# giech/usrp_nfc

Measured on NVIDIA B200. Metric: decoded_msamples_per_s, higher is better.
Workload: dtype f64

## Files before the change

usrp_nfc_b200/csrc/linecode.cu:

```cuda
#include "common.cuh"
#include "scan.cuh"

#include <algorithm>

namespace nfc {

#ifndef NFC_LC_CHUNK
#define NFC_LC_CHUNK 64
#endif
static const int CHUNK = NFC_LC_CHUNK;
static const int LOOKBACK_LIMIT = 4096;
static const int RSTATES = 32, GSTATES = 16;

struct __align__(16) ChunkMap {
    uint8_t r[RSTATES];
    uint8_t g[GSTATES];
};
struct ComposeMap {
    __device__ __forceinline__ ChunkMap operator()(const ChunkMap &a, const ChunkMap &b) const {
        ChunkMap c;
#pragma unroll
        for (int s = 0; s < RSTATES; s++) c.r[s] = b.r[a.r[s] & 31];
#pragma unroll
        for (int s = 0; s < GSTATES; s++) c.g[s] = b.g[a.g[s] & 15];
        return c;
    }
};

struct __align__(16) ChunkCnt {
    uint32_t nsym, nbit0, nbit1, nemit;
    uint32_t has0, tail0, has1, tail1;
};
struct CombineCnt {
    __device__ __forceinline__ ChunkCnt operator()(const ChunkCnt &a, const ChunkCnt &b) const {
        ChunkCnt c;
        c.nsym = a.nsym + b.nsym;
        c.nbit0 = a.nbit0 + b.nbit0;
        c.nbit1 = a.nbit1 + b.nbit1;
        c.nemit = a.nemit + b.nemit;
        if (a.has0 & 1) {
            if ((b.has0 & 2) && a.tail0 == 0) c.nemit--;
            c.has0 = a.has0;
        } else {
            c.has0 = (b.has0 & 1) | (((b.has0 & 2) && a.tail0 == 0) ? 2u : 0u);
        }
        if (a.has1 & 1) {
            if ((b.has1 & 2) && a.tail1 == 0) c.nemit--;
            c.has1 = a.has1;
        } else {
            c.has1 = (b.has1 & 1) | (((b.has1 & 2) && a.tail1 == 0) ? 2u : 0u);
        }
        c.tail0 = (b.has0 & 1) ? b.tail0 : a.tail0 + b.tail0;
        c.tail1 = (b.has1 & 1) ? b.tail1 : a.tail1 + b.tail1;
        return c;
    }
};
__device__ __forceinline__ uint32_t resolved_records(const ChunkCnt &pc, const uint32_t *pending) {
    return pc.nemit - (((pc.has0 & 2) && pending[0] == 0) ? 1u : 0u) - (((pc.has1 & 2) && pending[1] == 0) ? 1u : 0u);
}

struct EvCount {
    const uint32_t *d_M;
    uint32_t cap;
    __device__ __forceinline__ uint32_t n() const { return min(*d_M, cap); }
};

struct TabView {
    const uint8_t *dcm, *dcg;
    const TabEntry *tab;
    int goff;
    int use_reader, use_tag;
    uint32_t pitch, skip, len;
};

static const uint32_t NO_CAPTURE = 0xffffffffu;
__device__ __forceinline__ uint32_t batch_capture(const TabView &tv, uint32_t rel_pos, bool &inside) {
    const uint32_t cap = rel_pos / tv.pitch, off = rel_pos - cap * tv.pitch;
    inside = off >= tv.skip && off < tv.len;
    return cap;
}
__device__ __forceinline__ uint32_t batch_capture_before(const TabView &tv, const EventRec *__restrict__ ev, int64_t i) {
    return i > 0 ? ev[i - 1].rel_pos / tv.pitch : NO_CAPTURE;
}

template <class Sink>
__device__ __forceinline__ void framer_put(int &started, int o, int type, uint32_t pos, Sink &sink) {
    const int start_bit = type == 0 ? 1 : 0;
    sink.symbol(pos, type, o);
    if (o >= 2) {
        if (started) {
            sink.emission(pos, type);
            started = 0;
        }
    } else if (!started && o == start_bit) {
        started = 1;
    } else {
        sink.bit(type, o);
    }
}

template <class Sink>
__device__ __forceinline__ void step_event(const EventRec &ev, const TabView &tv, int &rs, int &gs, Sink &sink) {
    const bool is_r = ev.type == 1;
    if (!(is_r ? tv.use_reader != 0 : (ev.type == 0 && tv.use_tag != 0))) return;
    const uint8_t *dc = is_r ? tv.dcm : tv.dcg;
    const int nst = is_r ? MILLER_STATES : MANCH_STATES, sh = is_r ? 4 : 3;
    const int st = is_r ? rs : gs;
    const TabEntry e = tv.tab[(is_r ? 0 : tv.goff) + ((int)dc[ev.d] * 4 + (ev.v + 1)) * nst + (st & (nst - 1))];
    int started = st >> sh;
    const int n = tab_nout(e), type = is_r ? 1 : 0;
    if (n > 0) framer_put(started, tab_out0(e), type, ev.rel_pos, sink);
    if (n > 1 && is_r) framer_put(started, tab_out1(e), type, ev.rel_pos, sink);
    const int nx = (tab_next(e) & (nst - 1)) | (started << sh);
    rs = is_r ? nx : rs;
    gs = is_r ? gs : nx;
}

template <class Sink>
__device__ __forceinline__ void step_event_batch(const EventRec &ev, const TabView &tv, int &rs, int &gs, Sink &sink, uint32_t &cap_prev) {
    if (tv.pitch) {
        bool inside;
        const uint32_t cap = batch_capture(tv, ev.rel_pos, inside);
        if (cap != cap_prev) {
            cap_prev = cap;
            rs = 0;
            gs = 0;
            sink.new_capture();
        }
        if (!inside) return;
    }
    step_event(ev, tv, rs, gs, sink);
}

__device__ __forceinline__ void load8(const EventRec *__restrict__ ev, int64_t base, EventRec (&e)[8]) {
    const uint4 *p = reinterpret_cast<const uint4 *>(ev + base);
    const uint4 q[4] = {__ldg(p), __ldg(p + 1), __ldg(p + 2), __ldg(p + 3)};
#pragma unroll
    for (int k = 0; k < 4; k++) {
        const unsigned w[4] = {q[k].x, q[k].y, q[k].z, q[k].w};
#pragma unroll
        for (int h = 0; h < 2; h++) {
            EventRec r;
            r.rel_pos = w[2 * h];
            r.d = (uint16_t)(w[2 * h + 1] & 0xffffu);
            r.v = (int8_t)((w[2 * h + 1] >> 16) & 0xffu);
            r.type = (int8_t)(w[2 * h + 1] >> 24);
            e[2 * k + h] = r;
        }
    }
}

struct NullSink {
    __device__ __forceinline__ void symbol(uint32_t, int, int) {}
    __device__ __forceinline__ void emission(uint32_t, int) {}
    __device__ __forceinline__ void bit(int, int) {}
    __device__ __forceinline__ void new_capture() {}
};

__device__ __forceinline__ void load_tables(const LineTables &lt, TabEntry *sm, TabEntry *sg) {
    for (int i = threadIdx.x; i < lt.n_dclass_miller * 4 * MILLER_STATES; i += blockDim.x) sm[i] = lt.miller[i];
    for (int i = threadIdx.x; i < lt.n_dclass_manch * 4 * MANCH_STATES; i += blockDim.x) sg[i] = lt.manch[i];
    __syncthreads();
}

#define NFC_TABLE_SMEM                                              \
    __shared__ TabEntry s_tab[MAX_DCLASS * 4 * (MILLER_STATES + MANCH_STATES)]; \
    load_tables(lt, s_tab, s_tab + MAX_DCLASS * 4 * MILLER_STATES); \
    TabView tv;                                                     \
    tv.dcm = lt.dclass_miller; tv.dcg = lt.dclass_manch;            \
    tv.tab = s_tab; tv.goff = MAX_DCLASS * 4 * MILLER_STATES;        \
    tv.use_reader = lt.decode_reader; tv.use_tag = lt.decode_tag;   \
    tv.pitch = lt.batch_pitch; tv.skip = lt.batch_skip; tv.len = lt.batch_len;

__global__ void chunk_map_kernel(const EventRec *__restrict__ ev, EvCount evc, LineTables lt,
                                 ChunkMap *__restrict__ maps, uint32_t cap_chunks) {
    NFC_TABLE_SMEM
    const uint32_t c = blockIdx.x * blockDim.x + threadIdx.x;
    const uint32_t n_ev = evc.n();
    if (c >= cap_chunks) return;
    const uint32_t i0 = min(n_ev, c * CHUNK), i1 = min(n_ev, i0 + CHUNK);
    uint8_t r[RSTATES], g[GSTATES];
    for (int s = 0; s < RSTATES; s++) r[s] = (uint8_t)s;
    for (int s = 0; s < GSTATES; s++) g[s] = (uint8_t)s;
    bool r_flat = false, g_flat = false;
    NullSink sink;
    uint32_t cap_prev = tv.pitch ? batch_capture_before(tv, ev, (int64_t)i0) : 0u;
    for (uint32_t i = i0; i < i1; i++) {
        const EventRec e = ev[i];
        if (tv.pitch) {
            bool inside;
            const uint32_t cap = batch_capture(tv, e.rel_pos, inside);
            if (cap != cap_prev) {
                cap_prev = cap;
                r[0] = 0; g[0] = 0;
                r_flat = g_flat = true;
            }
            if (!inside) continue;
        }
        if (e.type == 1 && tv.use_reader) {
            if (r_flat) {
                int rs = r[0], gs = 0;
                step_event(e, tv, rs, gs, sink);
                r[0] = (uint8_t)rs;
            } else {
                bool same = true;
                int first = 0;
                for (int s = 0; s < RSTATES; s++) {
                    int rs = r[s], gs = 0;
                    step_event(e, tv, rs, gs, sink);
                    r[s] = (uint8_t)rs;
                    if (s == 0) first = rs;
                    same = same && (rs == first);
                }
                r_flat = same;
            }
        } else if (e.type == 0 && tv.use_tag) {
            if (g_flat) {
                int rs = 0, gs = g[0];
                step_event(e, tv, rs, gs, sink);
                g[0] = (uint8_t)gs;
            } else {
                bool same = true;
                int first = 0;
                for (int s = 0; s < GSTATES; s++) {
                    int rs = 0, gs = g[s];
                    step_event(e, tv, rs, gs, sink);
                    g[s] = (uint8_t)gs;
                    if (s == 0) first = gs;
                    same = same && (gs == first);
                }
                g_flat = same;
            }
        }
    }
    ChunkMap m;
    for (int s = 0; s < RSTATES; s++) m.r[s] = r_flat ? r[0] : r[s];
    for (int s = 0; s < GSTATES; s++) m.g[s] = g_flat ? g[0] : g[s];
    maps[c] = m;
}

struct CountSink {
    ChunkCnt c;
    __device__ __forceinline__ void symbol(uint32_t, int, int) { c.nsym++; }
    __device__ __forceinline__ void emission(uint32_t, int type) {
        uint32_t &has = type == 0 ? c.has0 : c.has1;
        uint32_t &tail = type == 0 ? c.tail0 : c.tail1;
        if (tail != 0) c.nemit++;
        else if (!(has & 1)) { c.nemit++; has |= 2; }
        has |= 1;
        tail = 0;
    }
    __device__ __forceinline__ void bit(int type, int) {
        if (type == 0) { c.nbit0++; c.tail0++; } else { c.nbit1++; c.tail1++; }
    }
    __device__ __forceinline__ void new_capture() {
        c.has0 |= 1; c.tail0 = 0;
        c.has1 |= 1; c.tail1 = 0;
    }
};

__global__ void chunk_summary_kernel(const EventRec *__restrict__ ev, EvCount evc, LineTables lt,
                                     uint16_t *__restrict__ summary) {
    NFC_TABLE_SMEM
    const uint32_t c = blockIdx.x * blockDim.x + threadIdx.x;
    const uint32_t n_ev = evc.n(), n_chunks = (n_ev + CHUNK - 1) / CHUNK;
    if (c >= n_chunks) return;
    int rs = 0, gs = 0;
    bool kR = false, kG = false;
    NullSink sink;
    const uint32_t i0 = c * CHUNK, i1 = min(n_ev, i0 + CHUNK);
    uint32_t cap_prev = tv.pitch ? batch_capture_before(tv, ev, (int64_t)i0) : 0u;
    for (uint32_t i = i0; i < i1; i += 8) {
        EventRec e8[8];
        load8(ev, i, e8);
#pragma unroll
        for (int k = 0; k < 8; k++) {
            if (i + k >= i1) continue;
            const EventRec e = e8[k];
            int dummy = 0;
            if (tv.pitch) {
                bool inside;
                const uint32_t cap = batch_capture(tv, e.rel_pos, inside);
                if (cap != cap_prev) {
                    cap_prev = cap;
                    rs = 0; kR = true;
                    gs = 0; kG = true;
                }
                if (!inside) continue;
            }
            if (e.type == 1 && tv.use_reader) {
                const uint8_t r = lt.reset_miller[(int)tv.dcm[e.d] * 4 + (e.v + 1)];
                if (r != 0xFF) { rs = r; kR = true; }
                else if (kR) step_event(e, tv, rs, dummy, sink);
            } else if (e.type == 0 && tv.use_tag) {
                const uint8_t r = lt.reset_manch[(int)tv.dcg[e.d] * 4 + (e.v + 1)];
                if (r != 0xFF) { gs = r; kG = true; }
                else if (kG) step_event(e, tv, dummy, gs, sink);
            }
        }
    }
    summary[c] = (uint16_t)((rs & 31) | (kR ? 32 : 0) | ((gs & 15) << 8) | (kG ? 4096 : 0));
}

__global__ void chunk_start_kernel(const EventRec *__restrict__ ev, EvCount evc, LineTables lt,
                                   const DecCarry *__restrict__ carry_in, const uint16_t *__restrict__ summary,
                                   uint16_t *__restrict__ start, uint32_t *__restrict__ flags) {
    NFC_TABLE_SMEM
    const uint32_t c = blockIdx.x * blockDim.x + threadIdx.x;
    const uint32_t n_ev = evc.n(), n_chunks = (n_ev + CHUNK - 1) / CHUNK;
    if (c >= n_chunks) return;
    const DecCarry carry = *carry_in;
    int rs = (carry.miller_state & 15) | ((carry.started[1] & 1) << 4);
    int gs = (carry.manch_state & 7) | ((carry.started[0] & 1) << 3);
    const int64_t i0 = (int64_t)c * CHUNK;
    bool foundR = !tv.use_reader, foundG = !tv.use_tag;
    int64_t iR = -1, iG = -1;
    int64_t cc = (int64_t)c - 1;
    const int64_t cmin = max((int64_t)0, (int64_t)c - LOOKBACK_LIMIT / CHUNK);
    for (; cc >= cmin && !(foundR && foundG); cc--) {
        const unsigned sm = summary[cc];
        if (!foundR && (sm & 32u)) { foundR = true; iR = (cc + 1) * CHUNK - 1; rs = (int)(sm & 31u); }
        if (!foundG && (sm & 4096u)) { foundG = true; iG = (cc + 1) * CHUNK - 1; gs = (int)((sm >> 8) & 15u); }
    }
    if (cc >= 0 && !(foundR && foundG)) {
        atomicOr(flags, (uint32_t)POST_UNRESOLVED);
        start[c] = 0;
        return;
    }
    NullSink sink;
    const int64_t fromR = tv.use_reader ? iR + 1 : i0, fromG = tv.use_tag ? iG + 1 : i0;
    const int64_t from = fromR < fromG ? fromR : fromG;
    uint32_t cap_prev = (tv.pitch && from < i0) ? batch_capture_before(tv, ev, from) : 0u;
    for (int64_t base = from & ~(int64_t)7; base < i0; base += 8) {
        EventRec e8[8];
        load8(ev, base, e8);
#pragma unroll
        for (int k = 0; k < 8; k++) {
            const int64_t kk = base + k;
            if (kk < from || kk >= i0) continue;
            const EventRec e = e8[k];
            int dummy_r = 0, dummy_g = 0;
            if (tv.pitch) {
                bool inside;
                const uint32_t cap = batch_capture(tv, e.rel_pos, inside);
                if (cap != cap_prev) {
                    cap_prev = cap;
                    if (kk > iR) rs = 0;
                    if (kk > iG) gs = 0;
                }
                if (!inside) continue;
            }
            if (e.type == 1) {
                if (kk > iR) step_event(e, tv, rs, dummy_g, sink);
            } else if (e.type == 0) {
                if (kk > iG) step_event(e, tv, dummy_r, gs, sink);
            }
        }
    }
    start[c] = (uint16_t)(rs | (gs << 8));
}

__global__ void chunk_start_from_maps_kernel(const ChunkMap *__restrict__ prefix, const DecCarry *__restrict__ carry_in,
                                             uint16_t *__restrict__ start, uint32_t n_chunks) {
    const uint32_t c = blockIdx.x * blockDim.x + threadIdx.x;
    if (c >= n_chunks) return;
    const DecCarry carry = *carry_in;
    const int rs0 = (carry.miller_state & 15) | ((carry.started[1] & 1) << 4);
    const int gs0 = (carry.manch_state & 7) | ((carry.started[0] & 1) << 3);
    start[c] = (uint16_t)(prefix[c].r[rs0] | (prefix[c].g[gs0] << 8));
}

__global__ void chunk_count_kernel(const EventRec *__restrict__ ev, EvCount evc, LineTables lt,
                                   const uint16_t *__restrict__ start, ChunkCnt *__restrict__ cnts, uint32_t cap_chunks) {
    NFC_TABLE_SMEM
    const uint32_t c = blockIdx.x * blockDim.x + threadIdx.x;
    const uint32_t n_ev = evc.n(), n_chunks = (n_ev + CHUNK - 1) / CHUNK;
    if (c >= cap_chunks) return;
    CountSink sink;
    sink.c = ChunkCnt{0, 0, 0, 0, 0, 0, 0, 0};
    if (c >= n_chunks) {
        cnts[c] = sink.c;
        return;
    }
    int rs = start[c] & 31, gs = (start[c] >> 8) & 15;
    const uint32_t i0 = c * CHUNK, i1 = min(n_ev, i0 + CHUNK);
    uint32_t cap_prev = tv.pitch ? batch_capture_before(tv, ev, (int64_t)i0) : 0u;
    for (uint32_t i = i0; i < i1; i += 8) {
        EventRec e[8];
        load8(ev, i, e);
#pragma unroll
        for (int k = 0; k < 8; k++)
            if (i + k < i1) step_event_batch(e[k], tv, rs, gs, sink, cap_prev);
    }
    cnts[c] = sink.c;
}

struct WriteSink {
    SymbolRec *sym;
    uint8_t *bits0, *bits1;
    FrameRec *fr;
    unsigned long long *fx;
    uint32_t *n_empty;
    int64_t a;
    unsigned long long base0, base1;
    uint32_t isym, ib0, ib1, iem;
    uint32_t pend0, pend1;
    uint32_t cap_sym, cap_b0, cap_b1, cap_em;
    __device__ __forceinline__ void symbol(uint32_t pos, int type, int o) {
        if (sym && isym < cap_sym) {
            SymbolRec s;
            s.rel_pos = pos; s.type = (int8_t)type; s.val = (int8_t)o; s.pad = 0;
            sym[isym] = s;
        }
        isym++;
    }
    __device__ __forceinline__ void emission(uint32_t pos, int type) {
        const uint32_t nbits = type == 0 ? pend0 : pend1;
        if (nbits == 0) {
            atomicAdd(n_empty, 1u);
            return;
        }
        if (iem < cap_em) {
            FrameRec f;
            f.pos = a + (int64_t)pos;
            f.bit_off = (int64_t)((type == 0 ? base0 + ib0 : base1 + ib1) - nbits);
            f.nbits = (int32_t)nbits;
            f.type = type;
            fr[iem] = f;
            fx[iem] = ((unsigned long long)f.pos << 24) | ((unsigned long long)nbits << 8) | (unsigned long long)type;
        }
        if ((((unsigned long long)(a + (int64_t)pos)) >> 40) || nbits >= 65536u) atomicOr(n_empty, 0x80000000u);
        iem++;
        if (type == 0) pend0 = 0; else pend1 = 0;
    }
    __device__ __forceinline__ void bit(int type, int o) {
        if (type == 0) { if (ib0 < cap_b0) bits0[ib0] = (uint8_t)o; ib0++; pend0++; }
        else { if (ib1 < cap_b1) bits1[ib1] = (uint8_t)o; ib1++; pend1++; }
    }
    __device__ __forceinline__ void new_capture() { pend0 = 0; pend1 = 0; }
};

struct LineOut {
    SymbolRec *sym;
    uint8_t *bits0, *bits1;
    FrameRec *fr;
    unsigned long long *fx;
    uint32_t cap_sym, cap_b0, cap_b1, cap_em;
    const uint32_t *pending_in;
    int64_t a;
    const unsigned long long *bits_in;
    unsigned long long *bits_out;
    uint32_t *n_empty;
    uint32_t *n_frames;
};

__global__ void chunk_write_kernel(const EventRec *__restrict__ ev, EvCount evc, LineTables lt,
                                   const uint16_t *__restrict__ start,
                                   const ChunkCnt *__restrict__ cnt_prefix, LineOut out, const DecCarry *__restrict__ carry_in,
                                   DecCarry *__restrict__ carry_out, uint32_t *__restrict__ pending_out) {
    NFC_TABLE_SMEM
    const uint32_t c = blockIdx.x * blockDim.x + threadIdx.x;
    const uint32_t n_ev = evc.n(), n_chunks = (n_ev + CHUNK - 1) / CHUNK;
    if (n_chunks == 0 && c == 0) {
        *carry_out = *carry_in;
        pending_out[0] = out.pending_in[0];
        pending_out[1] = out.pending_in[1];
        out.bits_out[0] = out.bits_in[0];
        out.bits_out[1] = out.bits_in[1];
    }
    if (c >= n_chunks) return;
    int rs = start[c] & 31, gs = (start[c] >> 8) & 15;
    const ChunkCnt pc = cnt_prefix[c];
    WriteSink sink;
    sink.sym = out.sym; sink.bits0 = out.bits0; sink.bits1 = out.bits1; sink.fr = out.fr; sink.fx = out.fx;
    sink.n_empty = out.n_empty; sink.a = out.a; sink.base0 = out.bits_in[0]; sink.base1 = out.bits_in[1];
    sink.cap_sym = out.cap_sym; sink.cap_b0 = out.cap_b0; sink.cap_b1 = out.cap_b1; sink.cap_em = out.cap_em;
    sink.isym = pc.nsym; sink.ib0 = pc.nbit0; sink.ib1 = pc.nbit1; sink.iem = resolved_records(pc, out.pending_in);
    sink.pend0 = (pc.has0 & 1) ? pc.tail0 : out.pending_in[0] + pc.tail0;
    sink.pend1 = (pc.has1 & 1) ? pc.tail1 : out.pending_in[1] + pc.tail1;
    const uint32_t i0 = c * CHUNK, i1 = min(n_ev, i0 + CHUNK);
    uint32_t cap_prev = tv.pitch ? batch_capture_before(tv, ev, (int64_t)i0) : 0u;
    for (uint32_t i = i0; i < i1; i += 8) {
        EventRec e[8];
        load8(ev, i, e);
#pragma unroll
        for (int k = 0; k < 8; k++)
            if (i + k < i1) step_event_batch(e[k], tv, rs, gs, sink, cap_prev);
    }
    if (c == n_chunks - 1) {
        DecCarry co;
        co.miller_state = rs & 15; co.started[1] = rs >> 4;
        co.manch_state = gs & 7; co.started[0] = gs >> 3;
        *carry_out = co;
        pending_out[0] = sink.pend0;
        pending_out[1] = sink.pend1;
        out.bits_out[0] = sink.base0 + sink.ib0;
        out.bits_out[1] = sink.base1 + sink.ib1;
        *out.n_frames = sink.iem;
    }
}

uint32_t linecode_chunks(uint32_t n_ev) { return (n_ev + CHUNK - 1) / CHUNK; }
size_t linecode_map_bytes() { return sizeof(ChunkMap); }
size_t linecode_cnt_bytes() { return sizeof(ChunkCnt); }
size_t linecode_emission_bytes() { return sizeof(FrameRec); }
size_t linecode_scratch_bytes(uint32_t n_chunks) {
    return scan_scratch_elems(n_chunks) * sizeof(ChunkMap) + scan_scratch_elems(n_chunks) * sizeof(ChunkCnt);
}

int launch_linecode_start(const EventRec *d_ev, const uint32_t *d_M, uint32_t cap_ev, const LineTables &lt, const DecCarry *d_carry_in,
                          uint16_t *d_summary, uint16_t *d_start, uint32_t *d_flags, cudaStream_t stream) {
    const uint32_t nc = std::max(1u, linecode_chunks(cap_ev));
    const EvCount evc{d_M, cap_ev};
    chunk_summary_kernel<<<(nc + 127) / 128, 128, 0, stream>>>(d_ev, evc, lt, d_summary);
    NFC_CUDA_CHECK(cudaGetLastError());
    chunk_start_kernel<<<(nc + 127) / 128, 128, 0, stream>>>(d_ev, evc, lt, d_carry_in, d_summary, d_start, d_flags);
    NFC_CUDA_CHECK(cudaGetLastError());
    return 0;
}

int launch_linecode_start_scan(const EventRec *d_ev, const uint32_t *d_M, uint32_t cap_ev, const LineTables &lt,
                               const DecCarry *d_carry_in, void *d_maps, void *d_prefix, void *d_scratch, uint16_t *d_start,
                               cudaStream_t stream) {
    const uint32_t nc = std::max(1u, linecode_chunks(cap_ev));
    ChunkMap *maps = (ChunkMap *)d_maps, *prefix = (ChunkMap *)d_prefix;
    const unsigned nb = (nc + 127) / 128;
    const EvCount evc{d_M, cap_ev};
    chunk_map_kernel<<<nb, 128, 0, stream>>>(d_ev, evc, lt, maps, nc);
    NFC_CUDA_CHECK(cudaGetLastError());
    ChunkMap ident;
    for (int s = 0; s < RSTATES; s++) ident.r[s] = (uint8_t)s;
    for (int s = 0; s < GSTATES; s++) ident.g[s] = (uint8_t)s;
    if (device_exclusive_scan<ChunkMap, ComposeMap>(maps, prefix, nc, ident, ComposeMap(), (ChunkMap *)d_scratch, nullptr, stream))
        return -1;
    chunk_start_from_maps_kernel<<<nb, 128, 0, stream>>>(prefix, d_carry_in, d_start, nc);
    NFC_CUDA_CHECK(cudaGetLastError());
    return 0;
}

int launch_linecode_count(const EventRec *d_ev, const uint32_t *d_M, uint32_t cap_ev, const LineTables &lt, const uint16_t *d_start,
                          void *d_cnts, void *d_cnt_prefix, void *d_scratch, void *d_total, cudaStream_t stream) {
    const uint32_t nc = std::max(1u, linecode_chunks(cap_ev));
    ChunkCnt *cnts = (ChunkCnt *)d_cnts, *cprefix = (ChunkCnt *)d_cnt_prefix;
    const EvCount evc{d_M, cap_ev};
    chunk_count_kernel<<<(nc + 127) / 128, 128, 0, stream>>>(d_ev, evc, lt, d_start, cnts, nc);
    NFC_CUDA_CHECK(cudaGetLastError());
    ChunkCnt zero = {0, 0, 0, 0, 0, 0, 0, 0};
    return device_exclusive_scan<ChunkCnt, CombineCnt>(cnts, cprefix, nc, zero, CombineCnt(), (ChunkCnt *)d_scratch,
                                                       (ChunkCnt *)d_total, stream);
}

int launch_linecode_write(const EventRec *d_ev, const uint32_t *d_M, uint32_t cap_ev, const LineTables &lt, const uint16_t *d_start,
                          const void *d_cnt_prefix, SymbolRec *d_sym, uint32_t cap_sym, uint8_t *d_bits0, uint32_t cap_b0,
                          uint8_t *d_bits1, uint32_t cap_b1, void *d_frames, void *d_findex, uint32_t cap_em, int64_t a,
                          const void *d_bits_in, void *d_bits_out, uint32_t *d_n_empty, uint32_t *d_n_frames, const uint32_t *d_pending_in,
                          const DecCarry *d_carry_in, DecCarry *d_carry_out, uint32_t *d_pending_out, cudaStream_t stream) {
    const uint32_t nc = std::max(1u, linecode_chunks(cap_ev));
    LineOut out;
    out.sym = d_sym; out.bits0 = d_bits0; out.bits1 = d_bits1; out.fr = (FrameRec *)d_frames; out.fx = (unsigned long long *)d_findex;
    out.cap_sym = cap_sym; out.cap_b0 = cap_b0; out.cap_b1 = cap_b1; out.cap_em = cap_em;
    out.pending_in = d_pending_in;
    out.a = a;
    out.bits_in = (const unsigned long long *)d_bits_in;
    out.bits_out = (unsigned long long *)d_bits_out;
    out.n_empty = d_n_empty;
    out.n_frames = d_n_frames;
    const EvCount evc{d_M, cap_ev};
    chunk_write_kernel<<<(nc + 127) / 128, 128, 0, stream>>>(d_ev, evc, lt, d_start, (const ChunkCnt *)d_cnt_prefix, out,
                                                             d_carry_in, d_carry_out, d_pending_out);
    NFC_CUDA_CHECK(cudaGetLastError());
    return 0;
}

}
```

usrp_nfc_b200/csrc/slicer.cu:

```cuda
#include <atomic>
#include <map>
#include <mutex>
#include <utility>
#include "common.cuh"
#include <cstdio>
#include <stdlib.h>

namespace nfc {

static const unsigned FULL = 0xffffffffu;
__device__ unsigned long long g_tile_stats[16];
#ifdef NFC_CYCLES
__device__ unsigned long long g_cyc[12];
#endif
__device__ int g_pipe_tune[4] = {6, 3, 2, 18};
enum { CLS_LOW = -1, CLS_MID = 0, CLS_HIGH = 1 };

template <int NT>
__device__ __forceinline__ void cta_sync() {
    asm volatile("bar.sync 1, %0;" ::"n"(NT) : "memory");
}
template <int NT>
__device__ __forceinline__ int cta_sync_or(int pred) {
    int r;
    asm volatile(
        "{\n\t"
        ".reg .pred p, q;\n\t"
        "setp.ne.s32 p, %1, 0;\n\t"
        "bar.red.or.pred q, 1, %2, p;\n\t"
        "selp.s32 %0, 1, 0, q;\n\t"
        "}"
        : "=r"(r)
        : "r"(pred), "n"(NT)
        : "memory");
    return r;
}

__device__ __forceinline__ float env_real(float s) { return __fmul_rn(s, s); }
__device__ __forceinline__ float env_iq(float re, float im) { return __fadd_rn(__fmul_rn(re, re), __fmul_rn(im, im)); }
__device__ __forceinline__ float env_sc16(short2 s, float scale) {
    return env_iq(__fdiv_rn((float)s.x, scale), __fdiv_rn((float)s.y, scale));
}
__device__ __forceinline__ float env_sc16_word(unsigned u, float scale) {
    return env_sc16(make_short2((short)(u & 0xffffu), (short)(u >> 16)), scale);
}
__device__ __forceinline__ float4 env_sc16x4(float4 v, float scale) {
    return make_float4(env_sc16_word(__float_as_uint(v.x), scale), env_sc16_word(__float_as_uint(v.y), scale),
                       env_sc16_word(__float_as_uint(v.z), scale), env_sc16_word(__float_as_uint(v.w), scale));
}

template <bool SC16 = true>
__device__ __forceinline__ float load_one(const void *in, int64_t idx, const SlicerParams &p) {
    if (SC16 && p.input_kind == IN_SC16) return env_sc16(__ldg(reinterpret_cast<const short2 *>(in) + idx), p.pcm_scale);
    switch (p.input_kind) {
        case IN_ENVELOPE_F32: return __ldg(reinterpret_cast<const float *>(in) + idx);
        case IN_REAL_F32: return env_real(__ldg(reinterpret_cast<const float *>(in) + idx));
        case IN_IQ_F32: {
            float2 c = __ldg(reinterpret_cast<const float2 *>(in) + idx);
            return env_iq(c.x, c.y);
        }
        default: {
            float s = __fdiv_rn((float)__ldg(reinterpret_cast<const short *>(in) + idx), p.pcm_scale);
            return env_real(s);
        }
    }
}

__device__ __forceinline__ float4 ldg_stream4(const float4 *ptr) {
    float4 r;
    asm volatile("ld.global.nc.L1::no_allocate.v4.f32 {%0,%1,%2,%3}, [%4];"
                 : "=f"(r.x), "=f"(r.y), "=f"(r.z), "=f"(r.w)
                 : "l"(ptr));
    return r;
}

template <int K, bool SC16 = true>
__device__ __forceinline__ void load_samples(const SegWork &w, const SlicerParams &p, int64_t p0, float (&x)[K]) {
    const int64_t i0 = p0 - w.in_pos0;
    if (K == 4 && p0 >= w.in_begin && p0 + 4 <= w.in_end) {
        if (p.input_kind == IN_ENVELOPE_F32 || p.input_kind == IN_REAL_F32) {
            float4 v = ldg_stream4(reinterpret_cast<const float4 *>(reinterpret_cast<const float *>(w.in) + i0));
            x[0] = v.x; x[1] = v.y; x[2] = v.z; x[3] = v.w;
            if (p.input_kind == IN_REAL_F32) {
#pragma unroll
                for (int j = 0; j < K; j++) x[j] = env_real(x[j]);
            }
            return;
        }
        if (p.input_kind == IN_IQ_F32) {
            const float4 *q = reinterpret_cast<const float4 *>(reinterpret_cast<const float2 *>(w.in) + i0);
            float4 a = ldg_stream4(q), b = ldg_stream4(q + 1);
            x[0] = env_iq(a.x, a.y); x[1] = env_iq(a.z, a.w); x[2] = env_iq(b.x, b.y); x[3] = env_iq(b.z, b.w);
            return;
        }
        if (p.input_kind == IN_PCM_S16) {
            short4 s = __ldg(reinterpret_cast<const short4 *>(reinterpret_cast<const short *>(w.in) + i0));
            x[0] = env_real(__fdiv_rn((float)s.x, p.pcm_scale));
            x[1] = env_real(__fdiv_rn((float)s.y, p.pcm_scale));
            x[2] = env_real(__fdiv_rn((float)s.z, p.pcm_scale));
            x[3] = env_real(__fdiv_rn((float)s.w, p.pcm_scale));
            return;
        }
        if (SC16 && p.input_kind == IN_SC16) {
            const float4 v = env_sc16x4(ldg_stream4(reinterpret_cast<const float4 *>(reinterpret_cast<const short2 *>(w.in) + i0)),
                                        p.pcm_scale);
            x[0] = v.x; x[1] = v.y; x[2] = v.z; x[3] = v.w;
            return;
        }
    }
#pragma unroll
    for (int j = 0; j < K; j++) {
        int64_t q = p0 + j;
        x[j] = (q >= w.in_begin && q < w.in_end) ? load_one<SC16>(w.in, q - w.in_pos0, p) : 0.0f;
    }
}

__device__ __noinline__ int classify_div(double pr, double ss, double lo, double hi) {
    double ratio = __ddiv_rn(pr, ss);
    if (lo > ratio) return CLS_LOW;
    if (ratio > hi) return CLS_HIGH;
    return CLS_MID;
}

__device__ __forceinline__ int classify(float x, double ss, const SlicerParams &p) {
    if (ss == 0.0) return x == 0.0f ? p.cls_ss0_x0 : p.cls_ss0_xn;
    const double pr = (double)x * p.Ld;
    if (!(ss > 0.0) || !(p.lo > 0.0) || !(p.hi > 0.0)) return classify_div(pr, ss, p.lo, p.hi);
    const double r = fma(-p.lo, ss, pr);
    if (r < 0.0) {
        if (r > -(p.lo * ss) * 0x1p-50) return classify_div(pr, ss, p.lo, p.hi);
        return CLS_LOW;
    }
    const double r2 = fma(-p.hi, ss, pr);
    if (r2 > 0.0) {
        if (r2 < (p.hi * ss) * 0x1p-50) return classify_div(pr, ss, p.lo, p.hi);
        return CLS_HIGH;
    }
    return CLS_MID;
}

__device__ __forceinline__ bool st2_forced(int64_t i, int64_t b, int64_t a, int mx) {
    if (b == NO_POS || i - b > (int64_t)mx + 1) return false;
    const int64_t j = b - a;
    const bool tmo = j >= mx && (j % mx) == 0;
    return !tmo;
}

template <int NT>
struct BlockShared {
    static const int NW = NT / 32;
    double wsum[2][NW];
    int wcnt[2][NW];
    int wlastcls[NW];
    int wmaxL[NW];
    int wmaxS[NW];
    unsigned flags[3];
    int emin, emax;
    double red[NW];
};

struct SegCarry {
    double ss0;
    int64_t lastL, lrun_start;
    int last_val;
    uint32_t seg_count;
    unsigned round_no;
    int scan_buf, cnt_buf;
};

template <int NT>
__device__ __forceinline__ double block_excl_scan(double v, double &total, double (*wsum)[NT / 32], int buf) {
    const int lane = threadIdx.x & 31, warp = threadIdx.x >> 5;
    double inc = v;
#pragma unroll
    for (int o = 1; o < 32; o <<= 1) {
        double n = __shfl_up_sync(FULL, inc, o);
        if (lane >= o) inc += n;
    }
    if (lane == 31) wsum[buf][warp] = inc;
    cta_sync<NT>();
    double wbase = 0.0, tot = 0.0;
#pragma unroll
    for (int w = 0; w < NT / 32; w++) {
        double s = wsum[buf][w];
        if (w < warp) wbase += s;
        tot += s;
    }
    total = tot;
    return wbase + (inc - v);
}

template <int NT>
__device__ __forceinline__ int block_excl_scan_int(int v, int &total, int (*wcnt)[NT / 32], int buf) {
    const int lane = threadIdx.x & 31, warp = threadIdx.x >> 5;
    int inc = v;
#pragma unroll
    for (int o = 1; o < 32; o <<= 1) {
        int n = __shfl_up_sync(FULL, inc, o);
        if (lane >= o) inc += n;
    }
    if (lane == 31) wcnt[buf][warp] = inc;
    cta_sync<NT>();
    int wbase = 0, tot = 0;
#pragma unroll
    for (int w = 0; w < NT / 32; w++) {
        int s = wcnt[buf][w];
        if (w < warp) wbase += s;
        tot += s;
    }
    total = tot;
    return wbase + (inc - v);
}

__device__ __forceinline__ void exp_track(float x, int &emin, int &emax) {
    const unsigned ub = __float_as_uint(x);
    if (ub != 0u) {
        const int e = (int)(ub >> 23);
        emin = min(emin, max(e, 1));
        emax = max(emax, e);
    }
}

template <int NT, int K, bool BM = false, bool SC16 = true>
__device__ __noinline__ void exact_tile(const SegWork *wp, const SlicerParams *pp, float *ring, BlockShared<NT> *shp,
                                        const int64_t P0, const int slot0, SegCarry *cs) {
    constexpr int NW = NT / 32;
    const SegWork &w = *wp;
    const SlicerParams &p = *pp;
    BlockShared<NT> &sh = *shp;
    const int L = p.L, mx = p.mx;
    const int tid = threadIdx.x, lane = tid & 31, warp = tid >> 5;
    const int64_t p0 = P0 + (int64_t)tid * K;
    SegCarry c = *cs;
    int emin = 1 << 30, emax = 0;
    const double ss0 = c.ss0;
    const int64_t lastL = c.lastL, lrun_start = c.lrun_start;
    const int last_val = c.last_val;

    float x[K], prev[K];
    bool act[K];
    load_samples<K, SC16>(w, p, p0, x);
#pragma unroll
    for (int j = 0; j < K; j++) act[j] = (p0 + j >= w.warm_begin) && (p0 + j < w.end);

    int slot[K];
#pragma unroll
    for (int j = 0; j < K; j++) {
        int s = slot0 + j;
        slot[j] = s >= L ? s - L : s;
    }
    if (K == 4 && (L & 3) == 0) {
        float4 v = *reinterpret_cast<const float4 *>(ring + slot0);
        prev[0] = v.x; prev[1] = v.y; prev[2] = v.z; prev[3] = v.w;
    } else {
#pragma unroll
        for (int j = 0; j < K; j++) prev[j] = ring[slot[j]];
    }

    int cls[K];
    bool forced[K];
#pragma unroll
    for (int j = 0; j < K; j++) {
        cls[j] = act[j] ? classify(x[j], ss0, p) : CLS_MID;
        forced[j] = false;
    }
    const bool carry_recent = lastL != NO_POS && (P0 - lastL) <= (int64_t)mx + 1;

    double total = 0.0;
    bool had_slow = false, anyL = false;
    for (;;) {
        const unsigned fb = c.round_no % 3u;
        if (tid == 0) sh.flags[(c.round_no + 1u) % 3u] = 0u;
        double pre[K];
        double run = 0.0;
#pragma unroll
        for (int j = 0; j < K; j++) {
            pre[j] = run;
            const bool admit = act[j] && (cls[j] == CLS_MID || (cls[j] == CLS_HIGH && forced[j]));
            if (admit) run += (double)x[j] - (double)prev[j];
        }
        const double base = block_excl_scan<NT>(run, total, sh.wsum, c.scan_buf);
        c.scan_buf ^= 1;

        unsigned f = 0u;
#pragma unroll
        for (int j = 0; j < K; j++) {
            if (act[j]) {
                const int cc = classify(x[j], ss0 + (base + pre[j]), p);
                if (cc != cls[j]) { f |= 1u; cls[j] = cc; }
                if (cc == CLS_HIGH) f |= 2u;
                if (cc == CLS_LOW) f |= 4u;
            }
        }
        f = __reduce_or_sync(FULL, f);
        if (lane == 0 && f) atomicOr(&sh.flags[fb], f);
        if (lane == 31) sh.wlastcls[warp] = act[K - 1] ? cls[K - 1] : 2;
        cta_sync<NT>();
        unsigned flags = sh.flags[fb];
        c.round_no++;

        if ((flags & 2u) && ((flags & 4u) || carry_recent)) {
            int pc = __shfl_up_sync(FULL, cls[K - 1], 1);
            const bool pact = __shfl_up_sync(FULL, (int)act[K - 1], 1) != 0;
            if (lane == 0) {
                pc = CLS_MID;
                bool found = false;
                for (int ww = warp - 1; ww >= 0 && !found; ww--) {
                    int cc = sh.wlastcls[ww];
                    if (cc != 2) { pc = cc; found = true; }
                }
                if (!found) pc = (last_val == -1) ? CLS_LOW : CLS_MID;
            } else if (!pact) {
                pc = (last_val == -1) ? CLS_LOW : CLS_MID;
            }
            int myL = -1, myS = -1;
            int preL[K], preS[K];
            {
                int c_prev = pc;
#pragma unroll
                for (int j = 0; j < K; j++) {
                    preL[j] = myL;
                    preS[j] = myS;
                    if (act[j]) {
                        if (cls[j] == CLS_LOW) {
                            if (c_prev != CLS_LOW) myS = tid * K + j;
                            myL = tid * K + j;
                        }
                        c_prev = cls[j];
                    }
                }
            }
            int incL = myL, incS = myS;
#pragma unroll
            for (int o = 1; o < 32; o <<= 1) {
                int a = __shfl_up_sync(FULL, incL, o), b = __shfl_up_sync(FULL, incS, o);
                if (lane >= o) { incL = max(incL, a); incS = max(incS, b); }
            }
            int exL = __shfl_up_sync(FULL, incL, 1), exS = __shfl_up_sync(FULL, incS, 1);
            if (lane == 0) { exL = -1; exS = -1; }
            if (lane == 31) { sh.wmaxL[warp] = incL; sh.wmaxS[warp] = incS; }
            cta_sync<NT>();
            for (int ww = 0; ww < warp; ww++) {
                exL = max(exL, sh.wmaxL[ww]);
                exS = max(exS, sh.wmaxS[ww]);
            }
            unsigned f2 = 0u;
#pragma unroll
            for (int j = 0; j < K; j++) {
                bool fo = false;
                if (act[j] && cls[j] == CLS_HIGH) {
                    const int bl = max(exL, preL[j]);
                    const int sl = max(exS, preS[j]);
                    const int64_t b = bl >= 0 ? P0 + bl : lastL;
                    const int64_t a = sl >= 0 ? P0 + sl : lrun_start;
                    fo = st2_forced(p0 + j, b, a, mx);
                }
                if (fo != forced[j]) { f2 = 1u; forced[j] = fo; }
            }
            const unsigned fb2 = c.round_no % 3u;
            if (tid == 0) sh.flags[(c.round_no + 1u) % 3u] = 0u;
            f2 = __reduce_or_sync(FULL, f2);
            if (lane == 0 && f2) atomicOr(&sh.flags[fb2], f2);
            cta_sync<NT>();
            flags |= sh.flags[fb2] & 1u;
            c.round_no++;
            had_slow = true;
        } else if (had_slow) {
            unsigned f2 = 0u;
#pragma unroll
            for (int j = 0; j < K; j++) {
                if (forced[j]) { f2 = 1u; forced[j] = false; }
            }
            if (cta_sync_or<NT>((int)f2)) flags |= 1u;
            had_slow = false;
        }
        if (!(flags & 1u)) {
            anyL = (flags & 4u) != 0u;
            break;
        }
    }

    float nv[K];
#pragma unroll
    for (int j = 0; j < K; j++) {
        const bool admit = act[j] && (cls[j] == CLS_MID || (cls[j] == CLS_HIGH && forced[j]));
        nv[j] = admit ? x[j] : prev[j];
        if (admit) exp_track(x[j], emin, emax);
    }
    if (K == 4 && (L & 3) == 0 && act[0] && act[K - 1]) {
        *reinterpret_cast<float4 *>(ring + slot0) = make_float4(nv[0], nv[1], nv[2], nv[3]);
    } else {
#pragma unroll
        for (int j = 0; j < K; j++)
            if (act[j]) ring[slot[j]] = nv[j];
    }

    int val[K];
#pragma unroll
    for (int j = 0; j < K; j++)
        val[j] = act[j] ? (cls[j] == CLS_LOW ? -1 : ((cls[j] == CLS_HIGH && !forced[j]) ? 1 : 0)) : 3;
    int mylast = 3;
#pragma unroll
    for (int j = 0; j < K; j++)
        if (val[j] != 3) mylast = val[j];
    int pv;
    {
        const unsigned has = __ballot_sync(FULL, mylast != 3);
        const unsigned lower = has & ((1u << lane) - 1u);
        const int src = lower ? 31 - __clz(lower) : 0;
        const int got = __shfl_sync(FULL, mylast, src);
        pv = lower ? got : 3;
        int wl = __shfl_sync(FULL, mylast, has ? 31 - __clz(has) : 0);
        if (!has) wl = 3;
        if (lane == 0) sh.wlastcls[warp] = wl;
    }
    cta_sync<NT>();
    if (pv == 3) {
        pv = last_val;
        for (int ww = warp - 1; ww >= 0; ww--) {
            const int cc = sh.wlastcls[ww];
            if (cc != 3) { pv = cc; break; }
        }
    }
    int ntr = 0;
    unsigned trmask = 0u;
    int maxS = -1, maxL = -1;
    {
        int c_prev = pv;
#pragma unroll
        for (int j = 0; j < K; j++) {
            if (val[j] != 3) {
                if (val[j] != c_prev) {
                    if (p0 + j >= w.begin) { trmask |= 1u << j; ntr++; }
                    if (val[j] == -1) maxS = tid * K + j;
                }
                if (val[j] == -1) maxL = tid * K + j;
                c_prev = val[j];
            }
        }
    }
    if (anyL) {
        int mL = __reduce_max_sync(FULL, maxL), mS = __reduce_max_sync(FULL, maxS);
        if (lane == 0) { sh.wmaxL[warp] = mL; sh.wmaxS[warp] = mS; }
    }
    int tot_tr = 0;
    const int tr_base = block_excl_scan_int<NT>(ntr, tot_tr, sh.wcnt, c.cnt_buf);
    c.cnt_buf ^= 1;
    if (BM) {
        if (K == 4 && w.bitmap) {
            unsigned wv = 0u;
#pragma unroll
            for (int j = 0; j < K; j++) {
                const bool on = val[j] != 3 && (p0 + j >= w.begin);
                const unsigned bn = __ballot_sync(FULL, !on || val[j] != -1), bh = __ballot_sync(FULL, on && val[j] == 1);
                if (lane == j) wv = bn;
                if (lane == 4 + j) wv = bh;
            }
            const int64_t cfirst = P0 + (int64_t)warp * 128;
            if (lane < 8 && cfirst + 127 >= w.begin && cfirst < w.end) w.bitmap[((cfirst - w.bm_pos0) >> 7) * 8 + lane] = wv;
        }
    } else if (tot_tr) {
        uint32_t idx = c.seg_count + (uint32_t)tr_base;
#pragma unroll
        for (int j = 0; j < K; j++) {
            if (trmask & (1u << j)) {
                if (idx < w.trans_cap) w.trans[idx] = pack_trans((uint32_t)(p0 + j - w.slab_pos0), val[j]);
                idx++;
            }
        }
        c.seg_count += (uint32_t)tot_tr;
    }
    c.ss0 = ss0 + total;
    if (anyL) {
        int mL = -1, mS = -1;
#pragma unroll
        for (int ww = 0; ww < NW; ww++) {
            mL = max(mL, sh.wmaxL[ww]);
            mS = max(mS, sh.wmaxS[ww]);
        }
        if (mL >= 0) {
            c.lastL = P0 + mL;
            if (mS >= 0) c.lrun_start = P0 + mS;
        }
    }
    {
        int lv = 3;
        for (int ww = NW - 1; ww >= 0; ww--) {
            const int cc = sh.wlastcls[ww];
            if (cc != 3) { lv = cc; break; }
        }
        if (lv != 3) c.last_val = lv;
    }
    emin = __reduce_min_sync(FULL, emin);
    emax = __reduce_max_sync(FULL, emax);
    if (lane == 0) {
        atomicMin(&sh.emin, emin);
        atomicMax(&sh.emax, emax);
    }
    if (tid == 0) *cs = c;
    cta_sync<NT>();
}

constexpr int SLICER_NT = 256;
__global__ void __launch_bounds__(SLICER_NT, 2) slicer_kernel(const SegWork *__restrict__ works,
                                                             const SlicerParams *__restrict__ params) {
    constexpr int NT = SLICER_NT, T = SLICER_NT;
    constexpr int NW = NT / 32;
    extern __shared__ __align__(16) float ring[];
    __shared__ BlockShared<NT> sh;

    __shared__ SegWork w_s;
    __shared__ SlicerParams p_s;
    __shared__ SegCarry c_s;
    if (threadIdx.x == 0) {
        w_s = works[blockIdx.x];
        p_s = params[w_s.param_idx];
    }
    __syncthreads();
    const SegWork &w = w_s;
    const SlicerParams &p = p_s;
    const int L = p.L;
    const int tid = threadIdx.x, lane = tid & 31, warp = tid >> 5;

    SegCarry c;
    int status = SEG_OK;
    int emin = 1 << 30, emax = 0;

    if (w.state_in) {
        const float *src = state_ring(w.state_in);
        for (int i = tid; i < L; i += NT) {
            float v = src[i];
            ring[i] = v;
            exp_track(v, emin, emax);
        }
        c.ss0 = w.state_in->ss;
        c.lastL = w.state_in->lastL;
        c.lrun_start = w.state_in->lrun_start;
        c.last_val = w.state_in->last_val;
    } else {
        double part = 0.0;
        for (int i = tid; i < L; i += NT) {
            const int64_t q = w.warm_begin - L + i;
            float v = load_one(w.in, q - w.in_pos0, p);
            ring[(int)(q % L)] = v;
            part += (double)v;
            exp_track(v, emin, emax);
        }
#pragma unroll
        for (int o = 16; o > 0; o >>= 1) part += __shfl_xor_sync(FULL, part, o);
        if (lane == 0) sh.red[warp] = part;
        __syncthreads();
        double s0 = 0.0;
        for (int i = 0; i < NW; i++) s0 += sh.red[i];
        c.ss0 = s0;
        c.lastL = NO_POS;
        c.lrun_start = NO_POS;
        c.last_val = 0;
    }
    if (tid == 0) {
        sh.flags[0] = sh.flags[1] = sh.flags[2] = 0u;
        sh.emin = 1 << 30;
        sh.emax = 0;
    }
    __syncthreads();
    c.seg_count = 0;
    c.scan_buf = 0;
    c.cnt_buf = 0;
    c.round_no = 0;
    unsigned n_exact = 0;

    const int64_t tile_first = w.warm_begin / T;
    const int64_t tile_last = (w.end > w.warm_begin) ? (w.end - 1) / T : tile_first - 1;
    int slot0 = (int)((tile_first * T + (int64_t)tid) % L);

    for (int64_t tile = tile_first; tile <= tile_last; tile++) {
        const int64_t P0 = tile * T;

        if (w.seam_in && P0 == w.begin && w.begin > w.warm_begin) {
            float *dst = state_ring(w.seam_in);
            for (int i = tid; i < L; i += NT) dst[i] = ring[i];
            if (tid == 0) {
                SlicerHdr h;
                h.ss = c.ss0; h.pos = w.begin; h.lastL = c.lastL; h.lrun_start = c.lrun_start;
                h.last_val = c.last_val; h.emin = 0; h.emax = 0; h.status = 0; h.count = 0; h.pad = 0;
                *w.seam_in = h;
            }
        }

#pragma unroll
        for (int j = 0; j < 3; j++) {
            if (w.ckpt_state[j] && P0 == w.ckpt_pos[j]) {
                float *dst = state_ring(w.ckpt_state[j]);
                for (int i = tid; i < L; i += NT) dst[i] = ring[i];
                if (tid == 0) {
                    SlicerHdr h;
                    h.ss = c.ss0; h.pos = P0; h.lastL = c.lastL; h.lrun_start = c.lrun_start;
                    h.last_val = c.last_val; h.emin = 0; h.emax = 0; h.status = 0; h.count = c.seg_count; h.pad = 0;
                    *w.ckpt_state[j] = h;
                }
            }
        }

        if (tid == 0) c_s = c;
        __syncthreads();
        exact_tile<NT, 1>(&w_s, &p_s, ring, &sh, P0, slot0, &c_s);
        c = c_s;
        n_exact++;
        slot0 += T % L;
        if (slot0 >= L) slot0 -= L;
    }

#pragma unroll
    for (int o = 16; o > 0; o >>= 1) {
        emin = min(emin, __shfl_xor_sync(FULL, emin, o));
        emax = max(emax, __shfl_xor_sync(FULL, emax, o));
    }
    __syncthreads();
    if (lane == 0) { atomicMin(&sh.emin, emin); atomicMax(&sh.emax, emax); }
    __syncthreads();
    emin = sh.emin; emax = sh.emax;
    if (emax >= 255) status |= SEG_NOT_SANE;
    if (emax > 0 && emax - emin > p.span_limit) status |= SEG_INEXACT;
    if (c.seg_count > w.trans_cap) status |= SEG_OVERFLOW;

    if (w.state_out) {
        float *dst = state_ring(w.state_out);
        for (int i = tid; i < L; i += NT) dst[i] = ring[i];
        if (tid == 0) {
            SlicerHdr h;
            h.ss = c.ss0; h.pos = w.end; h.lastL = c.lastL; h.lrun_start = c.lrun_start;
            h.last_val = c.last_val; h.emin = emin; h.emax = emax; h.status = status; h.count = c.seg_count; h.pad = 0;
            *w.state_out = h;
        }
    }
    if (tid == 0 && w.trans_count) *w.trans_count = c.seg_count;
    if (tid == 0 && w.status) *w.status = status;
    if (tid == 0) {
        atomicAdd(&g_tile_stats[1], (unsigned long long)n_exact);
        atomicAdd(&g_tile_stats[8], (unsigned long long)c.round_no);
    }
}

}
#include "slicer_fast.cuh"
namespace nfc {

__global__ void slicer_serial_kernel(const SegWork *__restrict__ works, const SlicerParams *__restrict__ params,
                                     float *__restrict__ ring_scratch, size_t ring_stride) {
    if (threadIdx.x != 0) return;
    const SegWork w = works[blockIdx.x];
    const SlicerParams p = params[w.param_idx];
    const int L = p.L, mx = p.mx;
    float *ring = ring_scratch + (size_t)blockIdx.x * ring_stride;

    double ss;
    int64_t lastL, lrun_start;
    int last_val;
    if (w.state_in) {
        const float *src = state_ring(w.state_in);
        for (int i = 0; i < L; i++) ring[i] = src[i];
        ss = w.state_in->ss;
        lastL = w.state_in->lastL;
        lrun_start = w.state_in->lrun_start;
        last_val = w.state_in->last_val;
    } else {
        ss = 0.0;
        for (int i = 0; i < L; i++) {
            const int64_t q = w.warm_begin - L + i;
            float v = load_one(w.in, q - w.in_pos0, p);
            ring[(int)(q % L)] = v;
            ss += (double)v;
        }
        lastL = NO_POS;
        lrun_start = NO_POS;
        last_val = 0;
    }
    uint32_t count = 0;
    int slot = (int)(w.warm_begin % L);
    for (int64_t q = w.warm_begin; q < w.end; q++) {
        if (w.seam_in && q == w.begin && w.begin > w.warm_begin) {
            float *dst = state_ring(w.seam_in);
            for (int i = 0; i < L; i++) dst[i] = ring[i];
            SlicerHdr h;
            h.ss = ss; h.pos = q; h.lastL = lastL; h.lrun_start = lrun_start;
            h.last_val = last_val; h.emin = 0; h.emax = 0; h.status = 0; h.count = 0; h.pad = 0;
            *w.seam_in = h;
        }
        const float x = load_one(w.in, q - w.in_pos0, p);
        const float prev = ring[slot];
        int c;
        if (ss == 0.0) c = x == 0.0f ? p.cls_ss0_x0 : p.cls_ss0_xn;
        else c = classify_div((double)x * p.Ld, ss, p.lo, p.hi);
        int val;
        if (c == CLS_LOW) {
            val = -1;
            if (last_val != -1) lrun_start = q;
            lastL = q;
        } else if (c == CLS_HIGH && !st2_forced(q, lastL, lrun_start, mx)) {
            val = 1;
        } else {
            val = 0;
            ring[slot] = x;
            ss += ((double)x - (double)prev);
        }
        if (val != last_val) {
            if (q >= w.begin) {
                if (count < w.trans_cap) w.trans[count] = pack_trans((uint32_t)(q - w.slab_pos0), val);
                count++;
            }
            last_val = val;
        }
        slot++;
        if (slot == L) slot = 0;
    }
    if (w.state_out) {
        float *dst = state_ring(w.state_out);
        for (int i = 0; i < L; i++) dst[i] = ring[i];
        SlicerHdr h;
        h.ss = ss; h.pos = w.end; h.lastL = lastL; h.lrun_start = lrun_start;
        h.last_val = last_val; h.emin = 0; h.emax = 0;
        h.status = count > w.trans_cap ? SEG_OVERFLOW : SEG_OK;
        h.count = count; h.pad = 0;
        *w.state_out = h;
    }
    if (w.trans_count) *w.trans_count = count;
    if (w.status) *w.status = count > w.trans_cap ? SEG_OVERFLOW : SEG_OK;
}

__device__ __forceinline__ void canon_st2(const SlicerHdr &h, int mx, int &kind, int64_t &val) {
    if (h.last_val == -1) { kind = 1; val = h.lrun_start; return; }
    if (h.lastL == NO_POS) { kind = 0; val = 0; return; }
    const int64_t j = h.lastL - h.lrun_start;
    const bool tmo = j >= mx && (j % mx) == 0;
    const int64_t until = tmo ? h.lastL : h.lastL + mx + 1;
    if (until < h.pos) { kind = 0; val = 0; } else { kind = 2; val = until; }
}

__global__ void seam_compare_kernel(const SlicerHdr *const *__restrict__ truth, const SlicerHdr *const *__restrict__ assumed,
                                    const int *__restrict__ param_idx, const SlicerParams *__restrict__ params,
                                    int *__restrict__ mismatch) {
    const SlicerHdr *a = truth[blockIdx.x], *b = assumed[blockIdx.x];
    if (!a || !b) return;
    const SlicerParams p = params[param_idx[blockIdx.x]];
    int bad = 0;
    const uint32_t *ra = reinterpret_cast<const uint32_t *>(state_ring(a));
    const uint32_t *rb = reinterpret_cast<const uint32_t *>(state_ring(b));
    if ((((uintptr_t)ra | (uintptr_t)rb) & 15) == 0 && (p.L & 3) == 0) {
        const uint4 *va = reinterpret_cast<const uint4 *>(ra), *vb = reinterpret_cast<const uint4 *>(rb);
        const int n4 = p.L >> 2;
        for (int i = threadIdx.x; i < n4; i += 2 * blockDim.x) {
            const int j = i + blockDim.x;
            const uint4 x0 = __ldg(va + i), y0 = __ldg(vb + i);
            uint4 x1 = x0, y1 = y0;
            if (j < n4) { x1 = __ldg(va + j); y1 = __ldg(vb + j); }
            bad |= (x0.x != y0.x) | (x0.y != y0.y) | (x0.z != y0.z) | (x0.w != y0.w) | (x1.x != y1.x) | (x1.y != y1.y) |
                   (x1.z != y1.z) | (x1.w != y1.w);
        }
    } else {
        for (int i = threadIdx.x; i < p.L; i += blockDim.x) bad |= (ra[i] != rb[i]);
    }
    if (threadIdx.x == 0) {
        if (__double_as_longlong(a->ss) != __double_as_longlong(b->ss)) bad = 1;
        if (a->last_val != b->last_val || a->pos != b->pos) bad = 1;
        int ka, kb;
        int64_t va, vb;
        canon_st2(*a, p.mx, ka, va);
        canon_st2(*b, p.mx, kb, vb);
        if (ka != kb || va != vb) bad = 1;
    }
    if (__syncthreads_or(bad) && threadIdx.x == 0) mismatch[blockIdx.x] = 1;
}

bool slicer_streaming_ok(int L, int kind);
int slicer_streaming_tile(int L, int kind);
int slicer_tile(int L, int kind) {
    if (slicer_streaming_ok(L, kind)) return slicer_streaming_tile(L, kind);
    return SLICER_NT;
}

static int raise_dynamic_smem(const void *fn, size_t smem);

struct FastVariant {
    const void *fn;
    int threads;
    size_t smem;
    int tile;
};
static int env_int(const char *name, int dflt) {
    const char *v = getenv(name);
    return (v && v[0]) ? atoi(v) : dflt;
}
static size_t smem_optin_limit() {
    int dev = 0, lim = 0;
    cudaGetDevice(&dev);
    cudaDeviceGetAttribute(&lim, cudaDevAttrMaxSharedMemoryPerBlockOptin, dev);
    return (size_t)lim;
}
static const size_t FAST_STATIC_SMEM = 10 * 1024;

static const int FAST_SMALL_MIN_L = 1024, FAST_BIG_MIN_L = 8192;
template <int KIND>
static FastVariant fast_variant(int L) {
    static const int pipe = env_int("NFC_SLICER_PIPE", 1), stages = env_int("NFC_SLICER_STAGES", 3);
    const size_t ring = ((size_t)L * 4 + 15) / 16 * 16;
    const size_t item = KIND == IN_IQ_F32 ? 8 : (KIND == IN_PCM_S16 ? 2 : 4);
    const size_t T = L >= FAST_BIG_MIN_L ? 4096 : 512;
    const size_t one = KIND == IN_IQ_F32 ? 0 : T * item;
    const size_t stg = KIND == IN_PCM_S16 ? T * 6 : T * 4;
    const size_t half = smem_optin_limit() / 2;
    FastVariant v;
    v.tile = (int)T;
    if (L < FAST_BIG_MIN_L) {
        if (pipe && KIND != IN_IQ_F32) {
            v.fn = (const void *)slicer_fast_kernel<128, 1, 5, KIND, 3>;
            v.threads = 192;
            v.smem = ring + 3 * stg;
        } else {
            v.fn = (const void *)slicer_fast_kernel<128, 1, 6, KIND, 0>;
            v.threads = 128;
            v.smem = ring + one;
        }
        return v;
    }
    if (pipe && KIND != IN_IQ_F32) {
        if (stages >= 3 && ring + 3 * stg + FAST_STATIC_SMEM <= half) {
            v.fn = (const void *)slicer_fast_kernel<256, 4, 2, KIND, 3>;
            v.threads = 320;
            v.smem = ring + 3 * stg;
        } else if (ring + 2 * stg + FAST_STATIC_SMEM <= half) {
            v.fn = (const void *)slicer_fast_kernel<256, 4, 2, KIND, 2>;
            v.threads = 320;
            v.smem = ring + 2 * stg;
        } else if (env_int("NFC_SLICER_HALF_TILE", 1) && ring + 3 * (stg / 2) + FAST_STATIC_SMEM <= half) {
            v.fn = (const void *)slicer_fast_kernel<256, 2, 2, KIND, 3>;
            v.threads = 320;
            v.smem = ring + 3 * (stg / 2);
            v.tile = 2048;
        } else if (ring + 3 * stg + FAST_STATIC_SMEM <= smem_optin_limit()) {
            v.fn = (const void *)slicer_fast_kernel<512, 2, 1, KIND, 3>;
            v.threads = 576;
            v.smem = ring + 3 * stg;
        } else {
            v.fn = (const void *)slicer_fast_kernel<256, 4, 3, KIND, 0>;
            v.threads = 256;
            v.smem = ring + one;
        }
    } else {
        v.fn = (const void *)slicer_fast_kernel<256, 4, 3, KIND, 0>;
        v.threads = 256;
        v.smem = ring + one;
    }
    return v;
}
static FastVariant fast_variant_of(int L, int kind) {
    switch (kind) {
        case IN_ENVELOPE_F32: return fast_variant<IN_ENVELOPE_F32>(L);
        case IN_REAL_F32: return fast_variant<IN_REAL_F32>(L);
        case IN_IQ_F32: return fast_variant<IN_IQ_F32>(L);
        case IN_SC16: return fast_variant<IN_SC16>(L);
        default: return fast_variant<IN_PCM_S16>(L);
    }
}

int slicer_streaming_tile(int L, int kind) { return fast_variant_of(L, kind).tile; }

static int raise_dynamic_smem(const void *fn, size_t smem) {
    static std::mutex mu;
    static std::map<std::pair<const void *, int>, size_t> have;
    int dev = 0;
    NFC_CUDA_CHECK(cudaGetDevice(&dev));
    std::lock_guard<std::mutex> lock(mu);
    size_t &cur = have[std::make_pair(fn, dev)];
    if (cur < smem) {
        NFC_CUDA_CHECK(cudaFuncSetAttribute(fn, cudaFuncAttributeMaxDynamicSharedMemorySize, (int)smem));
        cur = smem;
    }
    return 0;
}

bool slicer_streaming_ok(int L, int kind) {
    if (L % 4 != 0 || L < FAST_SMALL_MIN_L) return false;
    const FastVariant v = fast_variant_of(L, kind);
    cudaFuncAttributes fa;
    if (cudaFuncGetAttributes(&fa, v.fn) != cudaSuccess) return false;
    return v.smem + fa.sharedSizeBytes <= smem_optin_limit();
}

static int apply_pipe_tuning() {
    static std::mutex mu;
    static bool done[64] = {false};
    int dev = 0;
    NFC_CUDA_CHECK(cudaGetDevice(&dev));
    std::lock_guard<std::mutex> lock(mu);
    if (done[dev & 63]) return 0;
    done[dev & 63] = true;
    if (getenv("NFC_PIPE_MIN") || getenv("NFC_PIPE_COOL") || getenv("NFC_MEAS_MAX") || getenv("NFC_RESUM_BITS")) {
        int t[4] = {env_int("NFC_PIPE_MIN", 6), env_int("NFC_PIPE_COOL", 3), env_int("NFC_MEAS_MAX", 2), env_int("NFC_RESUM_BITS", 18)};
        if (t[0] < 3) t[0] = 3;
        if (t[1] < 0) t[1] = 0;
        if (t[2] < 1) t[2] = 1;
        NFC_CUDA_CHECK(cudaMemcpyToSymbol(g_pipe_tune, t, sizeof(t)));
    }
    return 0;
}

int launch_slicer_streaming(const SegWork *d_works, int n_works, const SlicerParams *d_params, int L, int kind, cudaStream_t stream) {
    if (n_works <= 0) return 0;
    if (apply_pipe_tuning()) return -1;
    const FastVariant v = fast_variant_of(L, kind);
    if (raise_dynamic_smem(v.fn, v.smem)) return -1;
    void *args[2] = {(void *)&d_works, (void *)&d_params};
    NFC_CUDA_CHECK(cudaLaunchKernel(v.fn, dim3((unsigned)n_works), dim3((unsigned)v.threads), args, v.smem, stream));
    return 0;
}

int launch_slicer(const SegWork *d_works, int n_works, const SlicerParams *d_params, int L, cudaStream_t stream) {
    if (n_works <= 0) return 0;
    const size_t smem = ((size_t)L * 4 + 15) / 16 * 16;
    if (raise_dynamic_smem((const void *)slicer_kernel, smem)) return -1;
    slicer_kernel<<<n_works, SLICER_NT, smem, stream>>>(d_works, d_params);
    NFC_CUDA_CHECK(cudaGetLastError());
    return 0;
}

int slicer_tile_stats(unsigned long long *out4, bool reset) {
    NFC_CUDA_CHECK(cudaMemcpyFromSymbol(out4, g_tile_stats, sizeof(unsigned long long) * 16));
#ifdef NFC_CYCLES
    {
        unsigned long long c[12];
        NFC_CUDA_CHECK(cudaMemcpyFromSymbol(c, g_cyc, sizeof(c)));
        fprintf(stderr, "cycles: tile passes %llu in %llu calls (%llu repeats), ring sums after refused tiles %llu, fix-point path %llu, exact path %llu, segment set-up %llu, snapshots %llu, after pipelined runs %llu (its last barrier %llu), loop top %llu, commits %llu\n",
                c[0], c[1], c[5], c[2], c[3], c[4], c[6], c[7], c[8], c[11], c[9], c[10]);
        if (reset) {
            unsigned long long z[12] = {0};
            NFC_CUDA_CHECK(cudaMemcpyToSymbol(g_cyc, z, sizeof(z)));
        }
    }
#endif
    if (reset) {
        unsigned long long z[16] = {0};
        NFC_CUDA_CHECK(cudaMemcpyToSymbol(g_tile_stats, z, sizeof(z)));
    }
    return 0;
}

int slicer_resident_ctas(int L, int kind) {
    int dev = 0, sms = 0, per = 0;
    cudaGetDevice(&dev);
    cudaDeviceGetAttribute(&sms, cudaDevAttrMultiProcessorCount, dev);
    cudaError_t e = cudaSuccess;
    const void *fn = (const void *)slicer_kernel;
    int threads = SLICER_NT;
    size_t dyn = ((size_t)L * 4 + 15) / 16 * 16;
    if (slicer_streaming_ok(L, kind)) {
        const FastVariant v = fast_variant_of(L, kind);
        fn = v.fn;
        threads = v.threads;
        dyn = v.smem;
    }
    if (raise_dynamic_smem(fn, dyn) == 0) e = cudaOccupancyMaxActiveBlocksPerMultiprocessor(&per, fn, threads, dyn);
    if (e != cudaSuccess || per < 1) per = 1;
    return sms * per;
}

__global__ void __launch_bounds__(256) batch_warm_kernel(const char *__restrict__ items, int64_t stride_bytes, int64_t pitch,
                                                         const SlicerParams *__restrict__ params, char *__restrict__ states,
                                                         size_t state_bytes) {
    extern __shared__ float warm_s[];
    const int64_t c = blockIdx.x;
    const SlicerParams p = params[c];
    const int L = p.L;
    SlicerHdr *h = reinterpret_cast<SlicerHdr *>(states + (size_t)c * state_bytes);
    float *ring = state_ring(h);
    const int64_t B = c * pitch;
    const void *in = items + c * stride_bytes;
    for (int i = threadIdx.x; i < L; i += blockDim.x) {
        const float v = load_one(in, i, p);
        warm_s[i] = v;
        ring[(int)((B + i) % L)] = v;
    }
    __syncthreads();
    if (threadIdx.x == 0) {
        double s = 0.0;
        for (int i = 0; i < L; i++) s += (double)warm_s[i];
        SlicerHdr hh;
        hh.ss = s;
        hh.pos = B + L;
        hh.lastL = NO_POS;
        hh.lrun_start = NO_POS;
        hh.last_val = 0;
        hh.emin = 0; hh.emax = 0; hh.status = 0; hh.count = 0; hh.pad = 0;
        *h = hh;
    }
}

__global__ void bitmap_fill_kernel(uint4 *__restrict__ bm, size_t n_chunks) {
    const size_t i = (size_t)blockIdx.x * blockDim.x + threadIdx.x;
    if (i >= n_chunks) return;
    bm[2 * i] = make_uint4(FULL, FULL, FULL, FULL);
    bm[2 * i + 1] = make_uint4(0u, 0u, 0u, 0u);
}

int launch_batch_warm(const void *d_items, int64_t stride_bytes, int64_t pitch, int n_cap, int L, const SlicerParams *d_params,
                      void *d_states, size_t state_bytes, cudaStream_t stream) {
    if (n_cap <= 0) return 0;
    const size_t smem = (size_t)L * 4;
    if (raise_dynamic_smem((const void *)batch_warm_kernel, smem)) return -1;
    batch_warm_kernel<<<n_cap, 256, smem, stream>>>((const char *)d_items, stride_bytes, pitch, d_params, (char *)d_states, state_bytes);
    NFC_CUDA_CHECK(cudaGetLastError());
    return 0;
}

int launch_bitmap_fill(uint32_t *d_bm, size_t n_chunks, cudaStream_t stream) {
    if (!n_chunks) return 0;
    bitmap_fill_kernel<<<(unsigned)((n_chunks + 255) / 256), 256, 0, stream>>>(reinterpret_cast<uint4 *>(d_bm), n_chunks);
    NFC_CUDA_CHECK(cudaGetLastError());
    return 0;
}

int launch_slicer_serial(const SegWork *d_works, int n_works, const SlicerParams *d_params, float *d_ring_scratch,
                         size_t ring_stride, cudaStream_t stream) {
    if (n_works <= 0) return 0;
    slicer_serial_kernel<<<n_works, 32, 0, stream>>>(d_works, d_params, d_ring_scratch, ring_stride);
    NFC_CUDA_CHECK(cudaGetLastError());
    return 0;
}

int launch_seam_compare(const SlicerHdr *const *d_truth, const SlicerHdr *const *d_assumed, const int *d_param_idx,
                        const SlicerParams *d_params, int *d_mismatch, int n, cudaStream_t stream) {
    if (n <= 0) return 0;
    seam_compare_kernel<<<n, 256, 0, stream>>>(d_truth, d_assumed, d_param_idx, d_params, d_mismatch);
    NFC_CUDA_CHECK(cudaGetLastError());
    return 0;
}

}
```

usrp_nfc_b200/csrc/stream.cu:

```cuda
#include <algorithm>
#include <atomic>
#include <chrono>
#include <cstdarg>
#include <cstdio>
#include <cstdlib>
#include <cstring>
#include <memory>
#include <string>
#include <thread>
#include <deque>
#include <vector>

#include "../../include/usrp_nfc_b200.h"
#include "common.cuh"
#include "tables.h"

namespace nfc {

int launch_slicer(const SegWork *d_works, int n_works, const SlicerParams *d_params, int L, cudaStream_t);
bool slicer_streaming_ok(int L, int kind);
int launch_slicer_streaming(const SegWork *d_works, int n_works, const SlicerParams *d_params, int L, int kind, cudaStream_t);
int launch_extract_count(const uint32_t *d_bm, int64_t bm_pos0, int64_t a, int64_t b, const RunCarry *d_rc_in, int carry_from_bm,
                         uint32_t *d_block_counts, uint32_t *d_block_offsets, uint32_t *d_scan_scratch, uint32_t *d_total,
                         cudaStream_t stream);
int launch_extract_write(const uint32_t *d_bm, int64_t bm_pos0, int64_t a, int64_t b, const RunCarry *d_rc_in, int carry_from_bm,
                         const uint32_t *d_block_offsets, TransRec *d_out, uint32_t out_cap, cudaStream_t stream);
size_t extract_blocks(int64_t bm_pos0, int64_t a, int64_t b);
int launch_slicer_serial(const SegWork *d_works, int n_works, const SlicerParams *d_params, float *d_ring_scratch,
                         size_t ring_stride, cudaStream_t);
int launch_seam_compare(const SlicerHdr *const *d_truth, const SlicerHdr *const *d_assumed, const int *d_param_idx,
                        const SlicerParams *d_params, int *d_mismatch, int n, cudaStream_t);
int launch_gather_transitions(const SegWork *d_works, const uint32_t *d_counts, uint32_t *d_offsets, int n_segs,
                              TransRec *d_dense, cudaStream_t);
int launch_gather_pieces(const TransRec *const *d_src, const uint32_t *d_n, const uint32_t *d_off, int n_pieces,
                         TransRec *d_dense, cudaStream_t);
int launch_run_count(const TransRec *d_tr, const uint32_t *d_R, uint32_t cap_R, int64_t w0, int64_t w1, const RunCarry *d_rc_in,
                     int mx, int keep_dropped, uint32_t *d_counts, uint32_t *d_offsets, uint32_t *d_scratch, uint32_t *d_total,
                     uint32_t *d_flags, cudaStream_t stream);
int launch_run_write(const TransRec *d_tr, const uint32_t *d_R, uint32_t cap_R, int64_t w0, int64_t w1, const RunCarry *d_rc_in,
                     int mx, int keep_dropped, const uint32_t *d_offsets, EventRec *d_events, uint32_t cap, const uint32_t *d_M,
                     RunCarry *d_carry_out, uint32_t *d_flags, cudaStream_t stream);
uint32_t linecode_chunks(uint32_t n_ev);
size_t linecode_map_bytes();
size_t linecode_cnt_bytes();
size_t linecode_emission_bytes();
size_t linecode_scratch_bytes(uint32_t n_chunks);
int launch_linecode_start(const EventRec *d_ev, const uint32_t *d_M, uint32_t cap_ev, const LineTables &lt, const DecCarry *d_carry_in,
                          uint16_t *d_summary, uint16_t *d_start, uint32_t *d_flags, cudaStream_t stream);
int launch_linecode_start_scan(const EventRec *d_ev, const uint32_t *d_M, uint32_t cap_ev, const LineTables &lt,
                               const DecCarry *d_carry_in, void *d_maps, void *d_prefix, void *d_scratch, uint16_t *d_start,
                               cudaStream_t stream);
int launch_linecode_count(const EventRec *d_ev, const uint32_t *d_M, uint32_t cap_ev, const LineTables &lt, const uint16_t *d_start,
                          void *d_cnts, void *d_cnt_prefix, void *d_scratch, void *d_total, cudaStream_t stream);
int launch_linecode_write(const EventRec *d_ev, const uint32_t *d_M, uint32_t cap_ev, const LineTables &lt, const uint16_t *d_start,
                          const void *d_cnt_prefix, SymbolRec *d_sym, uint32_t cap_sym, uint8_t *d_bits0, uint32_t cap_b0,
                          uint8_t *d_bits1, uint32_t cap_b1, void *d_frames, void *d_findex, uint32_t cap_em, int64_t a,
                          const void *d_bits_in, void *d_bits_out, uint32_t *d_n_empty, uint32_t *d_n_frames, const uint32_t *d_pending_in,
                          const DecCarry *d_carry_in, DecCarry *d_carry_out, uint32_t *d_pending_out, cudaStream_t stream);
int slicer_tile(int L, int kind);
int slicer_resident_ctas(int L, int kind);
int slicer_tile_stats(unsigned long long *out4, bool reset);
int launch_batch_warm(const void *d_items, int64_t stride_bytes, int64_t pitch, int n_cap, int L, const SlicerParams *d_params,
                      void *d_states, size_t state_bytes, cudaStream_t stream);
int launch_bitmap_fill(uint32_t *d_bm, size_t n_chunks, cudaStream_t stream);
int synth_render(void *dev_out, int64_t n, int64_t first_index, const int8_t *codes, const int64_t *lens, int64_t n_runs,
                 float carrier, float pause, float tag_high, float noise, float fade, double fade_period, uint64_t seed,
                 int as_envelope, cudaStream_t);

static thread_local char g_err[512] = "";
void set_error(const char *fmt, ...) {
    va_list ap;
    va_start(ap, fmt);
    vsnprintf(g_err, sizeof(g_err), fmt, ap);
    va_end(ap);
}

struct DevBuf {
    void *p = nullptr;
    size_t cap = 0;
    int ensure(size_t bytes) {
        if (bytes <= cap) return 0;
        if (p) cudaFree(p);
        p = nullptr;
        cap = 0;
        size_t want = bytes + bytes / 4 + 256;
        NFC_CUDA_CHECK(cudaMalloc(&p, want));
        cap = want;
        return 0;
    }
    void release() {
        if (p) cudaFree(p);
        p = nullptr;
        cap = 0;
    }
    template <class T>
    T *as() const { return reinterpret_cast<T *>(p); }
};

static size_t item_bytes(int kind) {
    switch (kind) {
        case IN_IQ_F32: return 8;
        case IN_PCM_S16: return 2;
        case IN_SC16: return 4;
        default: return 4;
    }
}

static int ceil_log2(int v) {
    int l = 0;
    while ((1LL << l) < v) l++;
    return l;
}

static int classify_ratio_host(double ratio, double lo, double hi) {
    if (lo > ratio) return -1;
    if (ratio > hi) return 1;
    return 0;
}

struct FrameArena {
    nfc_frame *p = nullptr;
    size_t n = 0, cap = 0;
    size_t size() const { return n; }
    bool empty() const { return n == 0; }
    nfc_frame *data() { return p; }
    const nfc_frame &operator[](size_t i) const { return p[i]; }
    void clear() { n = 0; }
    int reserve(size_t need) {
        if (need <= cap) return 0;
        const size_t ncap = std::max(need + need / 2 + 4096, cap * 2);
        nfc_frame *q = nullptr;
        if (cudaMallocHost((void **)&q, ncap * sizeof(nfc_frame)) != cudaSuccess) return -1;
        if (n) memcpy(q, p, n * sizeof(nfc_frame));
        if (p) cudaFreeHost(p);
        p = q;
        cap = ncap;
        return 0;
    }
    void release() {
        if (p) cudaFreeHost(p);
        p = nullptr;
        n = cap = 0;
    }
};
static_assert(sizeof(nfc_frame) == sizeof(FrameRec), "the device writes nfc_frame records");

struct BitArena {
    uint8_t *p = nullptr;
    size_t cap = 0, len = 0, closed = 0;
    int reserve(size_t need) {
        if (need <= cap) return 0;
        const size_t ncap = std::max(need + need / 2 + 65536, cap * 2);
        uint8_t *q = nullptr;
        if (cudaMallocHost((void **)&q, ncap) != cudaSuccess) return -1;
        if (len) memcpy(q, p, len);
        if (p) cudaFreeHost(p);
        p = q;
        cap = ncap;
        return 0;
    }
    void consume() {
        const size_t open = len - closed;
        if (open && closed) memmove(p, p + closed, open);
        len = open;
        closed = 0;
    }
    void clear() { len = closed = 0; }
    void release() {
        if (p) cudaFreeHost(p);
        p = nullptr;
        cap = len = closed = 0;
    }
};

struct Stream {
    nfc_params prm;
    SlicerParams sp;
    HostTables ht;
    LineTables lt;
    double factor;
    cudaStream_t cs = nullptr;
    cudaStream_t cs2 = nullptr;
    cudaStream_t cs3 = nullptr;
    cudaEvent_t ev_h[2] = {nullptr, nullptr};
    cudaEvent_t ev_k0 = nullptr, ev_k1 = nullptr;
    DevBuf staging2[2];
    static const int NCTX = 4;
    cudaEvent_t ev_a[NCTX] = {}, ev_b[NCTX] = {}, ev_c[NCTX] = {};
    cudaStream_t csR = nullptr, csL = nullptr;
    cudaEvent_t evE[NCTX] = {}, evR[NCTX] = {}, evL[NCTX] = {};
    long long chain_first_seq = 0;
    long long last_final_seq = -1;
    cudaEvent_t ev_ctx[NCTX] = {};
    cudaEvent_t ev_out[2] = {};
    bool ev_out_set[2] = {false, false};
    DevBuf ctx_d;
    char *ctx_h = nullptr;
    long long slab_seq = 0;
    struct Rates {
        bool have = false;
        double R = 0, M = 0, sym = 0, b0 = 0, b1 = 0, em = 0;
    } rates;

    int64_t pos = 0;
    bool stable = false;
    bool serial_mode = false;
    std::vector<float> warm;
    DevBuf state;
    RunCarry run_carry{0, 0, 0, 0};
    DecCarry dec_carry{0, 0, {0, 0}};
    uint32_t pending[2] = {0, 0};

    int64_t seg_len = 0, halo = 0, slab_len = 0;
    int force_serial = 0;

    DevBuf params_d, tab_d, staging, works_d, states_d, trans_seg, seg_counts, seg_status,
        seam_ptrs, mismatch_d, run_counts, run_offsets, scan_scr, maps_d, prefix_d, cnts_d, cprefix_d,
        line_scr, serial_ring, start_d, ckpt_d, redo_states, redo_trans,
        redo_counts, pieces_d, bitmap_d, ex_counts, ex_offsets, ex_scr, summ_d;
    DevBuf events_d[2], sym_d[2], bits0_d[2], bits1_d[2], em_d[2], fx_d[2];
    DevBuf trans_dense[2];
    std::vector<DevBuf> kept_bufs;
    static const int NPIN = 3;
    void *pinned[NPIN] = {nullptr, nullptr, nullptr};
    size_t pinned_cap[NPIN] = {0, 0, 0};
    long long slabs_enqueued = 0;
    std::atomic<long long> slabs_marshalled{0};
    std::thread marshal_thr;
    bool blocking_wait = false;
    cudaEvent_t ev_blk = nullptr;
    cudaError_t sync_cs() {
        if (!blocking_wait) return cudaStreamSynchronize(cs);
        const cudaError_t e = cudaEventRecord(ev_blk, cs);
        return e != cudaSuccess ? e : cudaEventSynchronize(ev_blk);
    }
    int set_wait_mode(bool blocking);
    std::atomic<int> marshal_err{0};
    struct SlabJob {
        long long seq = 0;
        int64_t a = 0, b = 0;
        uint32_t cap_R = 0, cap_M = 0, cap_sym = 0, cap_b0 = 0, cap_b1 = 0, cap_em = 0;
        bool exact = false;
        bool events_only = false;
        bool from_bitmap = false;
        bool want_ev = false, want_sym = false, want_fr = false, have_line = false;
        double t0 = 0, t1 = 0, t2 = 0;
    };
    std::deque<SlabJob> jobs;
    cudaEvent_t ev_d[NPIN] = {nullptr, nullptr, nullptr};
    int post_chain(int64_t a, int64_t b, bool from_bitmap, uint32_t R_host, bool force_exact, double t0, double t1,
                   const EventRec *host_events = nullptr, uint32_t n_host_events = 0);
    int64_t push_events(const nfc_event *ev, int64_t n);
    int finalize_front();
    int finalize_all() {
        while (!jobs.empty())
            if (finalize_front()) return -1;
        return 0;
    }
    int marshal(const SlabJob &j, int pi, char *hp, size_t off_ev, size_t off_sym, uint32_t M, uint32_t nsym);

    std::vector<nfc_event> out_events;
    std::vector<nfc_symbol> out_symbols;
    FrameArena out_frames;
    cudaEvent_t ev_last_records = nullptr;
    bool have_last_records = false;
    int settle_frames();
    uint64_t *findex = nullptr;
    size_t findex_n = 0, findex_cap = 0;
    bool findex_bad = false;
    bool findex_ext = false;
    bool findex_ext_locked = false;
    void findex_drop() {
        if (findex && findex_ext && findex_ext_locked) cudaHostUnregister(findex);
        if (findex && !findex_ext) cudaFreeHost(findex);
        findex = nullptr;
        findex_ext = findex_ext_locked = false;
        findex_cap = findex_n = 0;
    }
    int findex_reserve(size_t n) {
        if (n <= findex_cap) return 0;
        if (findex_ext) return -1;
        const size_t cap = std::max(n, findex_cap * 2 + 4096);
        uint64_t *p = nullptr;
        if (cudaMallocHost((void **)&p, cap * sizeof(uint64_t)) != cudaSuccess) return -1;
        if (findex_n) memcpy(p, findex, findex_n * sizeof(uint64_t));
        if (findex) cudaFreeHost(findex);
        findex = p;
        findex_cap = cap;
        return 0;
    }
    BitArena fb[2];
    int resident_ctas = 0;
    size_t ev_head = 0, sym_head = 0, fr_head = 0;

    nfc_stats stats;

    int tile() const { return slicer_tile(sp.L, sp.input_kind); }
    bool parallel_ok() const { return sp.L >= 256 && sp.L <= 52000 && !force_serial && !serial_mode; }

    int init(const nfc_params *p);
    void destroy();
    int ensure_pinned(int idx, size_t bytes);
    int join_marshal();
    int finish_pending() { return finalize_all(); }
    int settle() { return finalize_all() || join_marshal() || settle_frames() ? -1 : 0; }
    int64_t push(const void *items, int64_t n, int mem, int *called_back);
    int64_t push_batch(const void *items, int mem, int64_t n_cap, int64_t cap_len, int64_t stride_items, const double *lo_vals,
                       const double *hi_vals, int64_t *pitch_out);
    int64_t batch_fill_pitch = 0, batch_fill_caps = 0, batch_fill_len = 0;
    DevBuf batch_states, batch_stage;
    int finish_warmup();
    int process_slab(const void *d_in, int64_t in_pos0, int64_t in_begin, int64_t in_end, int64_t a, int64_t b, int64_t slicer_end);
    enum class Slicer { streaming, first_gen, sequential };
    int run_slicer(Slicer kind, const void *d_in, int64_t in_pos0, int64_t in_begin, int64_t in_end, int64_t a, int64_t b,
                   uint32_t *R_out, bool *fell_back);
    int launch_streaming(const SegWork *d_works, int n_works);
    void add_kernel_time();
    int compare_states(const std::vector<const SlicerHdr *> &truth, const std::vector<const SlicerHdr *> &assumed, int n,
                       std::vector<int> &mism);
    int64_t bm_lo = 0, bm_hi = 0, bm_origin = 0;
    int64_t super_slab = 5;
    bool super_balance = true;
    bool streaming_ok() const { return parallel_ok() && slicer_streaming_ok(sp.L, sp.input_kind); }
};

int Stream::ensure_pinned(int idx, size_t bytes) {
    if (bytes <= pinned_cap[idx]) return 0;
    if (pinned[idx]) cudaFreeHost(pinned[idx]);
    pinned[idx] = nullptr;
    pinned_cap[idx] = 0;
    NFC_CUDA_CHECK(cudaMallocHost(&pinned[idx], bytes + bytes / 4 + 4096));
    pinned_cap[idx] = bytes + bytes / 4 + 4096;
    return 0;
}

int Stream::join_marshal() {
    if (marshal_thr.joinable()) marshal_thr.join();
    if (const int err = marshal_err.exchange(0)) {
        set_error(err == 3 ? "more frames than the caller's frame index buffer holds (nfc_stream_set_frame_index_buffer)"
                           : (err == 2 ? "copying a slab's records to the host failed" : "internal: frame longer than the retained bits"));
        return -1;
    }
    return 0;
}

int Stream::init(const nfc_params *p) {
    prm = *p;
    memset(&stats, 0, sizeof(stats));
    if (!(p->samp_rate > 0) || p->av_window < 1 || p->max_len < 1 || p->max_len > 65535) {
        set_error("bad parameters: samp_rate=%g av_window=%d max_len=%d", p->samp_rate, p->av_window, p->max_len);
        return -1;
    }
    if (p->av_window >= (1 << 28)) {
        set_error("av_window too large");
        return -1;
    }
    NFC_CUDA_CHECK(cudaSetDevice(p->device));
    NFC_CUDA_CHECK(cudaStreamCreateWithFlags(&cs, cudaStreamNonBlocking));
    NFC_CUDA_CHECK(cudaStreamCreateWithFlags(&cs2, cudaStreamNonBlocking));
    NFC_CUDA_CHECK(cudaStreamCreateWithFlags(&cs3, cudaStreamNonBlocking));
    NFC_CUDA_CHECK(cudaStreamCreateWithFlags(&csR, cudaStreamNonBlocking));
    NFC_CUDA_CHECK(cudaStreamCreateWithFlags(&csL, cudaStreamNonBlocking));
    for (int i = 0; i < 2; i++) NFC_CUDA_CHECK(cudaEventCreateWithFlags(&ev_h[i], cudaEventDisableTiming));
    NFC_CUDA_CHECK(cudaEventCreate(&ev_k0));
    NFC_CUDA_CHECK(cudaEventCreate(&ev_k1));
    for (int i = 0; i < NCTX; i++) {
        NFC_CUDA_CHECK(cudaEventCreate(&ev_a[i]));
        NFC_CUDA_CHECK(cudaEventCreate(&ev_b[i]));
        NFC_CUDA_CHECK(cudaEventCreate(&ev_c[i]));
        NFC_CUDA_CHECK(cudaEventCreateWithFlags(&ev_ctx[i], cudaEventDisableTiming));
        NFC_CUDA_CHECK(cudaEventCreateWithFlags(&evE[i], cudaEventDisableTiming));
        NFC_CUDA_CHECK(cudaEventCreateWithFlags(&evR[i], cudaEventDisableTiming));
        NFC_CUDA_CHECK(cudaEventCreateWithFlags(&evL[i], cudaEventDisableTiming));
    }
    for (int i = 0; i < 2; i++) NFC_CUDA_CHECK(cudaEventCreateWithFlags(&ev_out[i], cudaEventDisableTiming));
    for (int i = 0; i < NPIN; i++) NFC_CUDA_CHECK(cudaEventCreateWithFlags(&ev_d[i], cudaEventDisableTiming | cudaEventBlockingSync));
    NFC_CUDA_CHECK(cudaMallocHost((void **)&ctx_h, (size_t)NCTX * 256));
    if (ctx_d.ensure((size_t)NCTX * 256)) return -1;
    NFC_CUDA_CHECK(cudaMemset(ctx_d.p, 0, (size_t)NCTX * 256));
    factor = 1e6 / p->samp_rate;
    sp.lo = p->lo_val;
    sp.hi = p->hi_val;
    sp.L = p->av_window;
    sp.Ld = (double)p->av_window;
    sp.mx = p->max_len;
    sp.loL = sp.lo / sp.Ld;
    sp.hiL = sp.hi / sp.Ld;
    sp.cls_ss0_x0 = classify_ratio_host(1.0, sp.lo, sp.hi);
    sp.cls_ss0_xn = classify_ratio_host(sp.hi + 0.1, sp.lo, sp.hi);
    sp.span_limit = std::max(0, 28 - ceil_log2(sp.L) - 1);
    sp.input_kind = p->input_kind;
    sp.pcm_scale = p->pcm_scale > 0 ? p->pcm_scale : 32767.0f;
    if (params_d.ensure(sizeof(SlicerParams))) return -1;
    NFC_CUDA_CHECK(cudaMemcpy(params_d.p, &sp, sizeof(sp), cudaMemcpyHostToDevice));

    if (!build_tables(sp.mx, factor, ht)) {
        set_error("line-code tables need more than %d duration classes", MAX_DCLASS);
        return -1;
    }
    const size_t dcm = ht.dclass_miller.size(), dcg = ht.dclass_manch.size();
    const size_t tm = ht.miller.size() * sizeof(TabEntry), tg = ht.manch.size() * sizeof(TabEntry);
    auto up = [](size_t v) { return (v + 255) / 256 * 256; };
    const size_t o1 = up(dcm), o2 = o1 + up(dcg), o3 = o2 + up(tm), o4 = o3 + up(tg), o5 = o4 + up(ht.reset_miller.size());
    if (tab_d.ensure(o5 + up(ht.reset_manch.size()))) return -1;
    char *base = tab_d.as<char>();
    NFC_CUDA_CHECK(cudaMemcpy(base, ht.dclass_miller.data(), dcm, cudaMemcpyHostToDevice));
    NFC_CUDA_CHECK(cudaMemcpy(base + o1, ht.dclass_manch.data(), dcg, cudaMemcpyHostToDevice));
    NFC_CUDA_CHECK(cudaMemcpy(base + o2, ht.miller.data(), tm, cudaMemcpyHostToDevice));
    NFC_CUDA_CHECK(cudaMemcpy(base + o3, ht.manch.data(), tg, cudaMemcpyHostToDevice));
    NFC_CUDA_CHECK(cudaMemcpy(base + o4, ht.reset_miller.data(), ht.reset_miller.size(), cudaMemcpyHostToDevice));
    NFC_CUDA_CHECK(cudaMemcpy(base + o5, ht.reset_manch.data(), ht.reset_manch.size(), cudaMemcpyHostToDevice));
    lt.dclass_miller = (const uint8_t *)base;
    lt.dclass_manch = (const uint8_t *)(base + o1);
    lt.miller = (const TabEntry *)(base + o2);
    lt.manch = (const TabEntry *)(base + o3);
    lt.reset_miller = (const uint8_t *)(base + o4);
    lt.reset_manch = (const uint8_t *)(base + o5);
    lt.n_dclass_miller = ht.n_dclass_miller;
    lt.n_dclass_manch = ht.n_dclass_manch;
    lt.decode_reader = p->decode_reader;
    lt.decode_tag = p->decode_tag;
    lt.batch_pitch = 0;
    lt.batch_skip = 0;
    lt.batch_len = 0;

    warm.reserve((size_t)sp.L);
    if (state.ensure(state_block_bytes(sp.L))) return -1;
    resident_ctas = parallel_ok() ? slicer_resident_ctas(sp.L, sp.input_kind) : 1;
    if (const char *e = getenv("NFC_SUPER_SLAB")) super_slab = std::max(1, std::min(8, atoi(e)));
    if (const char *e = getenv("NFC_SUPER_BALANCE")) super_balance = atoi(e) != 0;
    return 0;
}

void Stream::destroy() {
    DevBuf *all[] = {&batch_states, &batch_stage, &params_d, &tab_d, &staging, &works_d, &states_d, &trans_seg, &trans_dense[0], &trans_dense[1], &seg_counts,
                     &seg_status, &seam_ptrs, &mismatch_d, &run_counts, &run_offsets, &scan_scr, &maps_d,
                     &prefix_d, &cnts_d, &cprefix_d, &line_scr, &ctx_d, &events_d[0], &events_d[1], &sym_d[0], &sym_d[1], &bits0_d[0],
                     &bits0_d[1], &bits1_d[0], &bits1_d[1], &em_d[0], &em_d[1], &fx_d[0], &fx_d[1],
                     &serial_ring, &start_d, &ckpt_d, &redo_states, &redo_trans, &redo_counts, &pieces_d, &state, &bitmap_d,
                     &ex_counts, &ex_offsets, &ex_scr, &summ_d};
    finalize_all();
    if (marshal_thr.joinable()) marshal_thr.join();
    if (cs) cudaStreamSynchronize(cs);
    if (csR) cudaStreamSynchronize(csR);
    if (csL) cudaStreamSynchronize(csL);
    if (cs2) cudaStreamSynchronize(cs2);
    for (DevBuf *b : all) b->release();
    if (ctx_h) cudaFreeHost(ctx_h);
    ctx_h = nullptr;
    fb[0].release();
    fb[1].release();
    out_frames.release();
    findex_drop();
    for (int i = 0; i < NPIN; i++)
        if (pinned[i]) cudaFreeHost(pinned[i]);
    for (int i = 0; i < NCTX; i++) {
        if (ev_a[i]) cudaEventDestroy(ev_a[i]);
        if (ev_b[i]) cudaEventDestroy(ev_b[i]);
        if (ev_c[i]) cudaEventDestroy(ev_c[i]);
        if (ev_ctx[i]) cudaEventDestroy(ev_ctx[i]);
        if (evE[i]) cudaEventDestroy(evE[i]);
        if (evR[i]) cudaEventDestroy(evR[i]);
        if (evL[i]) cudaEventDestroy(evL[i]);
    }
    for (int i = 0; i < 2; i++)
        if (ev_out[i]) cudaEventDestroy(ev_out[i]);
    if (csR) cudaStreamDestroy(csR);
    if (csL) cudaStreamDestroy(csL);
    if (cs2) cudaStreamDestroy(cs2);
    if (cs3) cudaStreamDestroy(cs3);
    if (ev_k0) cudaEventDestroy(ev_k0);
    if (ev_k1) cudaEventDestroy(ev_k1);
    for (int i = 0; i < 2; i++) {
        if (ev_h[i]) cudaEventDestroy(ev_h[i]);
        staging2[i].release();
    }
    for (int i = 0; i < NPIN; i++)
        if (ev_d[i]) cudaEventDestroy(ev_d[i]);
    if (ev_blk) cudaEventDestroy(ev_blk);
    if (cs) cudaStreamDestroy(cs);
}

static float host_env(const void *items, int64_t i, int kind, float pcm_scale) {
    switch (kind) {
        case IN_ENVELOPE_F32: return ((const float *)items)[i];
        case IN_REAL_F32: {
            volatile float s = ((const float *)items)[i];
            volatile float r = s * s;
            return r;
        }
        case IN_IQ_F32: {
            volatile float re = ((const float *)items)[2 * i], im = ((const float *)items)[2 * i + 1];
            volatile float a = re * re, b = im * im;
            volatile float r = a + b;
            return r;
        }
        case IN_SC16: {
            const int16_t *iq = (const int16_t *)items + 2 * i;
            volatile float re = (float)iq[0] / pcm_scale, im = (float)iq[1] / pcm_scale;
            volatile float a = re * re, b = im * im;
            volatile float r = a + b;
            return r;
        }
        default: {
            volatile float s = (float)((const int16_t *)items)[i] / pcm_scale;
            volatile float r = s * s;
            return r;
        }
    }
}

int Stream::set_wait_mode(bool blocking) {
    if (settle()) return -1;
    NFC_CUDA_CHECK(cudaSetDevice(prm.device));
    const unsigned flags = cudaEventDisableTiming | (blocking ? cudaEventBlockingSync : 0);
    for (int i = 0; i < NCTX; i++) {
        if (ev_ctx[i]) cudaEventDestroy(ev_ctx[i]);
        ev_ctx[i] = nullptr;
        NFC_CUDA_CHECK(cudaEventCreateWithFlags(&ev_ctx[i], flags));
    }
    if (blocking && !ev_blk) NFC_CUDA_CHECK(cudaEventCreateWithFlags(&ev_blk, cudaEventDisableTiming | cudaEventBlockingSync));
    blocking_wait = blocking;
    return 0;
}

int Stream::finish_warmup() {
    double s = 0;
    for (int i = 0; i < sp.L; i++) s += (double)warm[(size_t)i];
    std::vector<char> blk(state_block_bytes(sp.L), 0);
    SlicerHdr *h = reinterpret_cast<SlicerHdr *>(blk.data());
    h->ss = s;
    h->pos = sp.L;
    h->lastL = NO_POS;
    h->lrun_start = NO_POS;
    h->last_val = 0;
    memcpy(state_ring(h), warm.data(), (size_t)sp.L * 4);
    NFC_CUDA_CHECK(cudaMemcpyAsync(state.p, blk.data(), blk.size(), cudaMemcpyHostToDevice, cs));
    NFC_CUDA_CHECK(sync_cs());
    run_carry.st = 0;
    run_carry.last_bit = 0;
    run_carry.dur = sp.L % sp.mx;
    stable = true;
    return 0;
}

int64_t Stream::push(const void *items, int64_t n, int mem, int *called_back) {
    if (called_back) *called_back = 0;
    if (n < 0) {
        set_error("negative item count");
        return -1;
    }
    NFC_CUDA_CHECK(cudaSetDevice(prm.device));
    const size_t ib = item_bytes(sp.input_kind);
    if (!stable) {
        const int64_t need = sp.L - (int64_t)warm.size();
        const int64_t can = std::min(n, need);
        if (can > 0) {
            std::vector<char> tmp;
            const void *src = items;
            if (mem == NFC_MEM_DEVICE) {
                tmp.resize((size_t)can * ib);
                NFC_CUDA_CHECK(cudaMemcpyAsync(tmp.data(), items, (size_t)can * ib, cudaMemcpyDeviceToHost, cs));
                NFC_CUDA_CHECK(sync_cs());
                src = tmp.data();
            }
            for (int64_t i = 0; i < can; i++) warm.push_back(host_env(src, i, sp.input_kind, sp.pcm_scale));
        }
        pos += can;
        if (can == need && finish_warmup()) return -1;
        return can;
    }
    if (called_back) *called_back = 1;
    int64_t done = 0;
    const int64_t slab = slab_len > 0 ? std::min<int64_t>(slab_len, (int64_t)1 << 30) : (int64_t)1 << 28;
    const bool host_in = mem == NFC_MEM_HOST;
    auto stage_host = [&](int64_t off, int64_t m, int64_t a, int buf) -> int {
        const size_t padb = (size_t)(a - (a - (a & 3))) * ib;
        if (staging2[buf].ensure(padb + (size_t)m * ib + 64)) return -1;
        NFC_CUDA_CHECK(cudaMemcpyAsync(staging2[buf].as<char>() + padb, (const char *)items + (size_t)off * ib, (size_t)m * ib,
                                       cudaMemcpyHostToDevice, cs3));
        NFC_CUDA_CHECK(cudaEventRecord(ev_h[buf], cs3));
        stats.h2d_bytes += (int64_t)((size_t)m * ib);
        return 0;
    };
    int hbuf = 0;
    if (host_in && n > 0) {
        NFC_CUDA_CHECK(sync_cs());
        if (stage_host(0, std::min(slab, n), pos, hbuf)) return -1;
    }
    while (done < n) {
        const int64_t m = std::min(slab, n - done);
        const int64_t a = pos, b = pos + m;
        const int64_t in_pos0 = a - (a & 3);
        const void *d_in = nullptr;
        int64_t in_begin = in_pos0;
        int64_t slicer_end = b;
        const char *src = (const char *)items + (size_t)done * ib;
        const size_t padb = (size_t)(a - in_pos0) * ib;
        if (host_in) {
            const int64_t m_next = std::min(slab, n - (done + m));
            if (m_next > 0 && stage_host(done + m, m_next, b, hbuf ^ 1)) return -1;
            NFC_CUDA_CHECK(cudaStreamWaitEvent(cs, ev_h[hbuf], 0));
            d_in = staging2[hbuf].p;
            hbuf ^= 1;
        } else if ((((uintptr_t)src - padb) & 15) == 0) {
            d_in = src - padb;
            in_begin = a;
            int64_t take = super_slab;
            if (super_balance) {
                const int64_t left = (n - done + slab - 1) / slab, launches = (left + super_slab - 1) / super_slab;
                take = (left + launches - 1) / launches;
            }
            slicer_end = std::min(pos + (n - done), a + take * slab);
        } else {
            if (staging.ensure(padb + (size_t)m * ib + 64)) return -1;
            NFC_CUDA_CHECK(cudaMemcpyAsync(staging.as<char>() + padb, src, (size_t)m * ib, cudaMemcpyDeviceToDevice, cs));
            d_in = staging.p;
        }
        if (process_slab(d_in, in_pos0, in_begin, std::max(b, slicer_end), a, b, slicer_end)) return -1;
        pos = b;
        done += m;
        stats.samples += m;
    }
    return n;
}

int64_t Stream::push_batch(const void *items, int mem, int64_t n_cap, int64_t cap_len, int64_t stride_items, const double *lo_vals,
                           const double *hi_vals, int64_t *pitch_out) {
    NFC_CUDA_CHECK(cudaSetDevice(prm.device));
    const int L = sp.L;
    const int T = tile();
    const size_t ib = item_bytes(sp.input_kind);
    if (pos != 0 || stable || !warm.empty()) {
        set_error("push_batch: the stream has consumed samples; reset it first");
        return -1;
    }
    if (!streaming_ok()) {
        set_error("push_batch: needs the streaming slicer (av_window in [1024, 52000], a multiple of 4)");
        return -1;
    }
    if (n_cap <= 0 || cap_len <= (int64_t)L + 2 * sp.mx || stride_items < cap_len || L <= sp.mx + 1) {
        set_error("push_batch: bad shape (captures %lld, items %lld, stride %lld, av_window %d)", (long long)n_cap, (long long)cap_len,
                  (long long)stride_items, L);
        return -1;
    }
    if (prm.outputs & NFC_OUT_DROPPED_EVENTS) {
        set_error("push_batch: type -1 events are not reproduced across capture boundaries (NFC_OUT_DROPPED_EVENTS)");
        return -1;
    }
    if (((size_t)stride_items * ib) % 16 != 0 || ((uintptr_t)items % 16) != 0) {
        set_error("push_batch: captures must start 16-byte aligned");
        return -1;
    }
    const int64_t pitch = (cap_len + T - 1) / T * T;
    if (pitch >= ((int64_t)1 << 30)) {
        set_error("push_batch: capture too long for one slab");
        return -1;
    }
    if (pitch_out) *pitch_out = pitch;
    const void *d_items = items;
    if (mem == NFC_MEM_HOST) {
        const size_t bytes = ((size_t)(n_cap - 1) * (size_t)stride_items + (size_t)cap_len) * ib;
        if (batch_stage.ensure(bytes + 64)) return -1;
        NFC_CUDA_CHECK(cudaMemcpyAsync(batch_stage.p, items, bytes, cudaMemcpyHostToDevice, cs));
        stats.h2d_bytes += (int64_t)bytes;
        d_items = batch_stage.p;
    }
    std::vector<SlicerParams> ps((size_t)n_cap, sp);
    for (int64_t c = 0; c < n_cap; c++) {
        SlicerParams &q = ps[(size_t)c];
        if (lo_vals) q.lo = lo_vals[c];
        if (hi_vals) q.hi = hi_vals[c];
        q.loL = q.lo / q.Ld;
        q.hiL = q.hi / q.Ld;
        q.cls_ss0_x0 = classify_ratio_host(1.0, q.lo, q.hi);
        q.cls_ss0_xn = classify_ratio_host(q.hi + 0.1, q.lo, q.hi);
        if (!(q.lo > 0.0) || !(q.hi > q.lo)) {
            set_error("push_batch: capture %lld: thresholds must satisfy 0 < lo_val < hi_val", (long long)c);
            return -1;
        }
    }
    if (params_d.ensure(sizeof(SlicerParams) * (size_t)n_cap)) return -1;
    NFC_CUDA_CHECK(cudaMemcpyAsync(params_d.p, ps.data(), sizeof(SlicerParams) * (size_t)n_cap, cudaMemcpyHostToDevice, cs));
    const size_t sblk = state_block_bytes(L);
    if (batch_states.ensure(sblk * (size_t)n_cap) || seg_status.ensure(sizeof(int32_t) * (size_t)n_cap) ||
        works_d.ensure(sizeof(SegWork) * (size_t)n_cap))
        return -1;
    const int64_t total = n_cap * pitch;
    const size_t n_chunks = (size_t)(total / 128);
    const size_t bm_cap_before = bitmap_d.cap;
    if (bitmap_d.ensure((n_chunks + 64) * 32)) return -1;
    if (bitmap_d.cap != bm_cap_before || batch_fill_pitch != pitch || batch_fill_caps < n_cap || batch_fill_len != cap_len) {
        if (launch_bitmap_fill(bitmap_d.as<uint32_t>(), n_chunks, cs)) return -1;
        batch_fill_pitch = pitch;
        batch_fill_caps = n_cap;
        batch_fill_len = cap_len;
        stats.launches++;
    }
    if (launch_batch_warm(d_items, (int64_t)((size_t)stride_items * ib), pitch, (int)n_cap, L, params_d.as<SlicerParams>(), batch_states.p,
                          sblk, cs))
        return -1;
    stats.launches++;
    std::vector<int64_t> order((size_t)n_cap);
    for (int64_t c = 0; c < n_cap; c++) order[(size_t)c] = c;
    if (hi_vals) std::stable_sort(order.begin(), order.end(), [&](int64_t a, int64_t b) { return hi_vals[a] > hi_vals[b]; });
    std::vector<SegWork> works((size_t)n_cap);
    for (int64_t k = 0; k < n_cap; k++) {
        const int64_t c = order[(size_t)k];
        SegWork &w = works[(size_t)k];
        memset(&w, 0, sizeof(w));
        const int64_t B = c * pitch;
        w.in = (const char *)d_items + (size_t)c * (size_t)stride_items * ib;
        w.in_pos0 = B;
        w.in_begin = B;
        w.in_end = B + cap_len;
        w.warm_begin = B + L;
        w.begin = B + L;
        w.end = B + cap_len;
        w.slab_pos0 = 0;
        w.state_in = reinterpret_cast<const SlicerHdr *>(batch_states.as<char>() + sblk * (size_t)c);
        for (int j = 0; j < 3; j++) w.ckpt_pos[j] = INT64_MAX;
        w.status = seg_status.as<int32_t>() + c;
        w.param_idx = (int32_t)c;
        w.bitmap = bitmap_d.as<uint32_t>();
        w.bm_pos0 = 0;
    }
    NFC_CUDA_CHECK(cudaMemcpyAsync(works_d.p, works.data(), sizeof(SegWork) * (size_t)n_cap, cudaMemcpyHostToDevice, cs));
    if (launch_streaming(works_d.as<SegWork>(), (int)n_cap)) return -1;
    stats.launches++;
    stats.slicer_launches++;
    stats.segments += n_cap;
    std::vector<int32_t> status((size_t)n_cap);
    NFC_CUDA_CHECK(cudaMemcpyAsync(status.data(), seg_status.p, sizeof(int32_t) * (size_t)n_cap, cudaMemcpyDeviceToHost, cs));
    NFC_CUDA_CHECK(sync_cs());
    add_kernel_time();
    for (int64_t c = 0; c < n_cap; c++)
        if (status[(size_t)c] & (SEG_INEXACT | SEG_NOT_SANE)) {
            set_error("push_batch: capture %lld is outside the exactly-summable regime: decode the captures one by one", (long long)c);
            return -3;
        }
    stable = true;
    bm_lo = 0;
    bm_hi = total;
    bm_origin = 0;
    lt.batch_pitch = (uint32_t)pitch;
    lt.batch_skip = (uint32_t)L;
    lt.batch_len = (uint32_t)cap_len;
    const int64_t slab_max = slab_len > 0 ? std::min<int64_t>(slab_len, (int64_t)1 << 30) : (int64_t)1 << 30;
    const int64_t per_slab = std::max<int64_t>(1, slab_max / pitch);
    int rc = 0;
    if (finish_pending()) return -1;
    run_carry = RunCarry{0, 0, L % sp.mx, 0};
    for (int64_t c0 = 0; c0 < n_cap && !rc; c0 += per_slab) {
        const int64_t c1 = std::min(n_cap, c0 + per_slab);
        if (process_slab(nullptr, c0 * pitch, c0 * pitch, c1 * pitch, c0 * pitch, c1 * pitch, c1 * pitch)) rc = -1;
        pos = c1 * pitch;
        stats.samples += (c1 - c0) * cap_len;
    }
    if (!rc && finish_pending()) rc = -1;
    lt.batch_pitch = 0;
    bm_lo = bm_hi = 0;
    cudaMemcpyAsync(params_d.p, &sp, sizeof(sp), cudaMemcpyHostToDevice, cs);
    if (sync_cs() != cudaSuccess && !rc) rc = -1;
    return rc ? rc : n_cap;
}

int Stream::launch_streaming(const SegWork *d_works, int n_works) {
    NFC_CUDA_CHECK(cudaEventRecord(ev_k0, cs));
    if (launch_slicer_streaming(d_works, n_works, params_d.as<SlicerParams>(), sp.L, sp.input_kind, cs)) return -1;
    NFC_CUDA_CHECK(cudaEventRecord(ev_k1, cs));
    return 0;
}

void Stream::add_kernel_time() {
    float ms = 0;
    if (cudaEventElapsedTime(&ms, ev_k0, ev_k1) == cudaSuccess) {
        stats.slicer_kernel_ms += ms;
        stats.slicer_kernel_launches++;
    }
}

int Stream::compare_states(const std::vector<const SlicerHdr *> &truth, const std::vector<const SlicerHdr *> &assumed, int n,
                           std::vector<int> &mism) {
    const size_t room = truth.size();
    char *base = seam_ptrs.as<char>();
    NFC_CUDA_CHECK(cudaMemcpyAsync(base, truth.data(), sizeof(void *) * (size_t)n, cudaMemcpyHostToDevice, cs));
    NFC_CUDA_CHECK(cudaMemcpyAsync(base + sizeof(void *) * room, assumed.data(), sizeof(void *) * (size_t)n, cudaMemcpyHostToDevice, cs));
    NFC_CUDA_CHECK(cudaMemsetAsync(base + 2 * sizeof(void *) * room, 0, sizeof(int) * (size_t)n, cs));
    NFC_CUDA_CHECK(cudaMemsetAsync(mismatch_d.p, 0, sizeof(int) * (size_t)n, cs));
    if (launch_seam_compare((const SlicerHdr *const *)base, (const SlicerHdr *const *)(base + sizeof(void *) * room),
                            (const int *)(base + 2 * sizeof(void *) * room), params_d.as<SlicerParams>(), mismatch_d.as<int>(), n, cs))
        return -1;
    stats.launches++;
    NFC_CUDA_CHECK(cudaMemcpyAsync(mism.data(), mismatch_d.p, sizeof(int) * (size_t)n, cudaMemcpyDeviceToHost, cs));
    return 0;
}

static int print_segment_cycles(const std::vector<SegWork> &works) {
    const int nseg = (int)works.size();
    double sum = 0;
    uint32_t mn = ~0u, mx = 0;
    std::vector<uint32_t> kc((size_t)nseg), rs((size_t)nseg);
    for (int k = 0; k < nseg; k++) {
        SlicerHdr h;
        NFC_CUDA_CHECK(cudaMemcpy(&h, works[(size_t)k].state_out, sizeof(SlicerHdr), cudaMemcpyDeviceToHost));
        kc[(size_t)k] = h.count; rs[(size_t)k] = h.pad;
        sum += h.count; mn = std::min(mn, h.count); mx = std::max(mx, h.count);
    }
    fprintf(stderr, "segments %d kcycles min %u avg %.0f max %u\n", nseg, mn, sum / nseg, mx);
    for (int k = 0; k < nseg; k += std::max(1, nseg / 24))
        fprintf(stderr, "  seg %d: %u kcyc, redo %u slow %u\n", k, kc[(size_t)k], rs[(size_t)k] >> 16, rs[(size_t)k] & 0xffff);
    for (int q = 0; q < 6; q++) {
        int best = 0;
        for (int k = 1; k < nseg; k++) if (kc[(size_t)k] > kc[(size_t)best]) best = k;
        fprintf(stderr, "  slowest seg %d: %u kcyc, redo %u slow %u\n", best, kc[(size_t)best], rs[(size_t)best] >> 16, rs[(size_t)best] & 0xffff);
        kc[(size_t)best] = 0;
    }
    return 0;
}

int Stream::run_slicer(Slicer kind, const void *d_in, int64_t in_pos0, int64_t in_begin, int64_t in_end, int64_t a, int64_t b,
                       uint32_t *R_out, bool *fell_back) {
    if (finalize_all()) return -1;
    bm_hi = bm_lo = 0;
    const bool bitmap = kind == Slicer::streaming;
    const int L = sp.L;
    const int T = tile();
    *fell_back = false;
    std::vector<int64_t> begins;
    begins.push_back(a);
    int64_t H = 0;
    if (kind != Slicer::sequential) {
        const int64_t Hs = halo > 0 ? halo : (int64_t)16 * L;
        H = (Hs + T - 1) / T * T;
        int64_t S = seg_len;
        if (S <= 0) {
            const int64_t n = b - a, res = std::max(1, resident_ctas);
            const int64_t s_min = 6 * H;
            int64_t s_max, k = 1;
            if (bitmap) {
                s_max = std::max<int64_t>((int64_t)4096 * L, s_min);
                k = std::max<int64_t>(1, (n + res * s_max - 1) / (res * s_max));
            } else {
                s_max = std::max<int64_t>((int64_t)256 * L, s_min);
                while (n / (res * (k + 1)) >= s_min) k++;
            }
            S = std::clamp(n / (res * k), s_min, s_max);
        }
        S = (S + T - 1) / T * T;
        int64_t b1 = a + std::max<int64_t>(S, (int64_t)L + H);
        b1 = (b1 + T - 1) / T * T;
        while (b1 + S / 2 <= b && b1 < b) {
            begins.push_back(b1);
            b1 += S;
        }
    }
    const int nseg = (int)begins.size();
    const size_t sblk = state_block_bytes(L);
    const int NCK = 3;
    const int64_t ck_off[NCK] = {H, 3 * H, 7 * H};
    if (states_d.ensure(sblk * 2 * (size_t)nseg) || (nseg > 1 && ckpt_d.ensure(sblk * NCK * (size_t)nseg))) return -1;
    if (seg_status.ensure(sizeof(int32_t) * (size_t)nseg) || works_d.ensure(sizeof(SegWork) * (size_t)nseg * 2) ||
        mismatch_d.ensure(sizeof(int) * (size_t)nseg) || seam_ptrs.ensure((sizeof(void *) * 2 + sizeof(int)) * (size_t)nseg))
        return -1;
    if (!bitmap && seg_counts.ensure(sizeof(uint32_t) * (size_t)nseg)) return -1;
    if (kind == Slicer::sequential && serial_ring.ensure((size_t)L * 4 + 64)) return -1;
    const int64_t bm_pos0 = a / T * T;
    if (bitmap && bitmap_d.ensure(((size_t)((b - bm_pos0 + 127) / 128) + 64) * 32)) return -1;
    auto seam_in = [&](int k) { return reinterpret_cast<SlicerHdr *>(states_d.as<char>() + sblk * (2 * (size_t)k)); };
    auto st_out = [&](int k) { return reinterpret_cast<SlicerHdr *>(states_d.as<char>() + sblk * (2 * (size_t)k + 1)); };
    auto ckpt = [&](int k, int j) { return reinterpret_cast<SlicerHdr *>(ckpt_d.as<char>() + sblk * ((size_t)k * NCK + (size_t)j)); };
    auto tmp_state = [&](int i) { return reinterpret_cast<SlicerHdr *>(redo_states.as<char>() + sblk * (size_t)i); };
    auto launch = [&](const SegWork *d_works, int n_works) -> int {
        if (kind == Slicer::streaming) {
            if (launch_streaming(d_works, n_works)) return -1;
        } else if (kind == Slicer::first_gen) {
            if (launch_slicer(d_works, n_works, params_d.as<SlicerParams>(), L, cs)) return -1;
        } else {
            if (launch_slicer_serial(d_works, n_works, params_d.as<SlicerParams>(), serial_ring.as<float>(), (size_t)L + 16, cs))
                return -1;
            stats.serial_segments += n_works;
        }
        stats.launches++;
        stats.slicer_launches++;
        return 0;
    };

    std::vector<uint32_t> caps((size_t)nseg);
    for (int k = 0; k < nseg; k++) {
        const int64_t e = k + 1 < nseg ? begins[(size_t)k + 1] : b;
        caps[(size_t)k] = (uint32_t)std::min<int64_t>((e - begins[(size_t)k]) / 8 + 1024, (e - begins[(size_t)k]) + 16);
    }
    std::vector<SegWork> works((size_t)nseg);
    std::vector<uint32_t> counts((size_t)nseg);
    std::vector<int32_t> status((size_t)nseg);
    struct Piece {
        const TransRec *src;
        uint32_t n;
    };

    for (int attempt = 0; attempt < 4; attempt++) {
        std::vector<size_t> toff((size_t)nseg);
        if (!bitmap) {
            size_t total_cap = 0;
            for (int k = 0; k < nseg; k++) {
                toff[(size_t)k] = total_cap;
                total_cap += caps[(size_t)k];
            }
            if (trans_seg.ensure(total_cap * sizeof(TransRec) + 16)) return -1;
        }
        for (int k = 0; k < nseg; k++) {
            SegWork &w = works[(size_t)k];
            memset(&w, 0, sizeof(w));
            w.in = d_in;
            w.in_pos0 = in_pos0;
            w.in_begin = in_begin;
            w.in_end = in_end;
            w.begin = begins[(size_t)k];
            w.end = k + 1 < nseg ? begins[(size_t)k + 1] : b;
            w.warm_begin = k == 0 ? a : w.begin - H;
            w.slab_pos0 = a;
            w.state_in = k == 0 ? state.as<SlicerHdr>() : nullptr;
            w.seam_in = k == 0 ? nullptr : seam_in(k);
            for (int j = 0; j < NCK; j++) {
                const bool use = k > 0 && w.begin + ck_off[j] < w.end;
                w.ckpt_pos[j] = use ? w.begin + ck_off[j] : INT64_MAX;
                w.ckpt_state[j] = use ? ckpt(k, j) : nullptr;
            }
            w.state_out = st_out(k);
            w.status = seg_status.as<int32_t>() + k;
            if (bitmap) {
                w.bitmap = bitmap_d.as<uint32_t>();
                w.bm_pos0 = bm_pos0;
            } else {
                w.trans = trans_seg.as<TransRec>() + toff[(size_t)k];
                w.trans_cap = caps[(size_t)k];
                w.trans_count = seg_counts.as<uint32_t>() + k;
            }
        }
        NFC_CUDA_CHECK(cudaMemcpyAsync(works_d.p, works.data(), sizeof(SegWork) * (size_t)nseg, cudaMemcpyHostToDevice, cs));
        if (launch(works_d.as<SegWork>(), nseg)) return -1;
        stats.segments += nseg;

        std::vector<int> mism((size_t)nseg, 0);
        std::vector<const SlicerHdr *> truth((size_t)nseg, nullptr), assumed((size_t)nseg, nullptr);
        if (nseg > 1) {
            for (int k = 1; k < nseg; k++) {
                truth[(size_t)k] = st_out(k - 1);
                assumed[(size_t)k] = seam_in(k);
            }
            if (compare_states(truth, assumed, nseg, mism)) return -1;
        }
        if (!bitmap)
            NFC_CUDA_CHECK(cudaMemcpyAsync(counts.data(), seg_counts.p, sizeof(uint32_t) * (size_t)nseg, cudaMemcpyDeviceToHost, cs));
        NFC_CUDA_CHECK(cudaMemcpyAsync(status.data(), seg_status.p, sizeof(int32_t) * (size_t)nseg, cudaMemcpyDeviceToHost, cs));
        NFC_CUDA_CHECK(sync_cs());
        if (bitmap) add_kernel_time();
        int st_all = 0;
        bool over = false;
        for (int k = 0; k < nseg; k++) {
            st_all |= status[(size_t)k];
            if (counts[(size_t)k] > caps[(size_t)k]) {
                over = true;
                caps[(size_t)k] = counts[(size_t)k] + 16;
            }
        }
        if (kind != Slicer::sequential && (st_all & (SEG_INEXACT | SEG_NOT_SANE))) {
            *fell_back = true;
            return 0;
        }
        if (over) {
            stats.overflow_retries++;
            continue;
        }

        std::vector<std::vector<Piece>> pieces((size_t)nseg);
        for (int k = 0; k < nseg && !bitmap; k++) pieces[(size_t)k].push_back(Piece{works[(size_t)k].trans, counts[(size_t)k]});
        std::vector<char> bad((size_t)nseg, 0);
        int nbad = 0;
        for (int k = 1; k < nseg; k++) {
            bad[(size_t)k] = mism[(size_t)k] ? 1 : 0;
            nbad += bad[(size_t)k];
        }
        for (int guard = 0; nbad > 0 && guard < nseg + 2; guard++) {
            std::vector<int> ks;
            for (int k = 1; k < nseg; k++)
                if (bad[(size_t)k] && !bad[(size_t)k - 1]) ks.push_back(k);
            const int nr = (int)ks.size();
            stats.seam_mismatches += nr;
            size_t rcap_total = 0;
            std::vector<size_t> roff((size_t)nr);
            for (int i = 0; i < nr; i++) {
                roff[(size_t)i] = rcap_total;
                rcap_total += caps[(size_t)ks[(size_t)i]];
            }
            if (redo_states.ensure(sblk * (size_t)nr) || redo_counts.ensure(sizeof(uint32_t) * 2 * (size_t)nr) ||
                (!bitmap && redo_trans.ensure(rcap_total * sizeof(TransRec) + 16)))
                return -1;
            std::vector<uint32_t> used((size_t)nr, 0);
            std::vector<int64_t> at((size_t)nr);
            std::vector<char> active((size_t)nr, 1);
            for (int i = 0; i < nr; i++) at[(size_t)i] = works[(size_t)ks[(size_t)i]].begin;
            for (int stage = 0; stage <= NCK; stage++) {
                std::vector<SegWork> redo;
                std::vector<int> who;
                for (int i = 0; i < nr; i++) {
                    if (!active[(size_t)i]) continue;
                    const int k = ks[(size_t)i];
                    const SegWork &ws = works[(size_t)k];
                    if (stage < NCK && !ws.ckpt_state[stage]) continue;
                    SegWork w = ws;
                    w.warm_begin = w.begin = at[(size_t)i];
                    w.end = stage < NCK ? ws.ckpt_pos[stage] : ws.end;
                    w.state_in = at[(size_t)i] == ws.begin ? st_out(k - 1) : tmp_state(i);
                    w.seam_in = nullptr;
                    for (int j = 0; j < NCK; j++) { w.ckpt_pos[j] = INT64_MAX; w.ckpt_state[j] = nullptr; }
                    w.state_out = tmp_state(i);
                    w.status = reinterpret_cast<int32_t *>(redo_counts.as<uint32_t>() + nr + i);
                    if (!bitmap) {
                        w.trans = redo_trans.as<TransRec>() + roff[(size_t)i] + used[(size_t)i];
                        w.trans_cap = caps[(size_t)k] - std::min(caps[(size_t)k], used[(size_t)i]);
                        w.trans_count = redo_counts.as<uint32_t>() + i;
                    }
                    redo.push_back(w);
                    who.push_back(i);
                }
                if (redo.empty()) continue;
                SegWork *d_redo = works_d.as<SegWork>() + nseg;
                NFC_CUDA_CHECK(cudaMemcpyAsync(d_redo, redo.data(), sizeof(SegWork) * redo.size(), cudaMemcpyHostToDevice, cs));
                if (launch(d_redo, (int)redo.size())) return -1;
                const int nw = (int)who.size();
                std::vector<SlicerHdr> ck_hdr((size_t)nw);
                for (int q = 0; q < nw; q++) {
                    const int i = who[(size_t)q], k = ks[(size_t)i];
                    truth[(size_t)q] = tmp_state(i);
                    assumed[(size_t)q] = stage < NCK ? works[(size_t)k].ckpt_state[stage] : tmp_state(i);
                    if (!bitmap && stage < NCK)
                        NFC_CUDA_CHECK(cudaMemcpyAsync(&ck_hdr[(size_t)q], works[(size_t)k].ckpt_state[stage], sizeof(SlicerHdr),
                                                       cudaMemcpyDeviceToHost, cs));
                }
                if (compare_states(truth, assumed, nw, mism)) return -1;
                std::vector<uint32_t> rc((size_t)nr * 2);
                NFC_CUDA_CHECK(cudaMemcpyAsync(rc.data(), redo_counts.p, sizeof(uint32_t) * 2 * (size_t)nr, cudaMemcpyDeviceToHost, cs));
                NFC_CUDA_CHECK(sync_cs());
                if (bitmap) add_kernel_time();
                for (int q = 0; q < nw; q++) {
                    const int i = who[(size_t)q], k = ks[(size_t)i];
                    if ((int32_t)rc[(size_t)nr + i] & (SEG_INEXACT | SEG_NOT_SANE)) {
                        *fell_back = true;
                        return 0;
                    }
                    if (!bitmap) {
                        const uint32_t got = rc[(size_t)i];
                        if (got > redo[(size_t)q].trans_cap) {
                            over = true;
                            caps[(size_t)k] = caps[(size_t)k] * 2 + got;
                        }
                        used[(size_t)i] += std::min(got, redo[(size_t)q].trans_cap);
                    }
                    at[(size_t)i] = redo[(size_t)q].end;
                    if (stage < NCK && !mism[(size_t)q]) {
                        const uint32_t cc = ck_hdr[(size_t)q].count;
                        if (!bitmap)
                            pieces[(size_t)k] = {Piece{redo_trans.as<TransRec>() + roff[(size_t)i], used[(size_t)i]},
                                                 Piece{works[(size_t)k].trans + cc, counts[(size_t)k] - std::min(counts[(size_t)k], cc)}};
                        active[(size_t)i] = 0;
                        bad[(size_t)k] = 0;
                    } else if (stage == NCK || at[(size_t)i] >= works[(size_t)k].end) {
                        if (!bitmap) pieces[(size_t)k] = {Piece{redo_trans.as<TransRec>() + roff[(size_t)i], used[(size_t)i]}};
                        NFC_CUDA_CHECK(cudaMemcpyAsync(st_out(k), tmp_state(i), sblk, cudaMemcpyDeviceToDevice, cs));
                        active[(size_t)i] = 0;
                        bad[(size_t)k] = 0;
                        if (k + 1 < nseg) bad[(size_t)k + 1] = 2;
                    }
                }
                if (over) break;
            }
            if (over) break;
            std::vector<int> unk;
            for (int k = 1; k < nseg; k++)
                if (bad[(size_t)k] == 2) unk.push_back(k);
            if (!unk.empty()) {
                for (size_t q = 0; q < unk.size(); q++) {
                    truth[q] = st_out(unk[q] - 1);
                    assumed[q] = seam_in(unk[q]);
                }
                if (compare_states(truth, assumed, (int)unk.size(), mism)) return -1;
                NFC_CUDA_CHECK(sync_cs());
                for (size_t q = 0; q < unk.size(); q++) bad[(size_t)unk[q]] = mism[q] ? 1 : 0;
            }
            nbad = 0;
            for (int k = 1; k < nseg; k++) nbad += bad[(size_t)k] ? 1 : 0;
            if (nbad > 0 && !bitmap) {
                kept_bufs.push_back(redo_trans);
                redo_trans = DevBuf();
            }
        }
        if (over) {
            stats.overflow_retries++;
            for (DevBuf &kb : kept_bufs) kb.release();
            kept_bufs.clear();
            continue;
        }
        if (nbad > 0) {
            set_error("seam repair did not settle");
            return -1;
        }
        if (bitmap && getenv("NFC_SEGDEBUG") && print_segment_cycles(works)) return -1;
        NFC_CUDA_CHECK(cudaMemcpyAsync(state.p, st_out(nseg - 1), sblk, cudaMemcpyDeviceToDevice, cs));
        if (bitmap) {
            bm_lo = a;
            bm_hi = b;
            bm_origin = bm_pos0;
            return 0;
        }
        std::vector<const TransRec *> psrc;
        std::vector<uint32_t> pn, poff;
        size_t R = 0;
        for (int k = 0; k < nseg; k++)
            for (const Piece &pc : pieces[(size_t)k]) {
                psrc.push_back(pc.src);
                pn.push_back(pc.n);
                poff.push_back((uint32_t)R);
                R += pc.n;
            }
        const size_t np = psrc.size();
        DevBuf &td = trans_dense[slab_seq & 1];
        if (td.ensure((R + 16) * sizeof(TransRec)) || pieces_d.ensure(np * (sizeof(void *) + 8) + 64)) return -1;
        char *pb = pieces_d.as<char>();
        NFC_CUDA_CHECK(cudaMemcpyAsync(pb, psrc.data(), np * sizeof(void *), cudaMemcpyHostToDevice, cs));
        NFC_CUDA_CHECK(cudaMemcpyAsync(pb + np * sizeof(void *), pn.data(), np * 4, cudaMemcpyHostToDevice, cs));
        NFC_CUDA_CHECK(cudaMemcpyAsync(pb + np * (sizeof(void *) + 4), poff.data(), np * 4, cudaMemcpyHostToDevice, cs));
        if (launch_gather_pieces((const TransRec *const *)pb, (const uint32_t *)(pb + np * sizeof(void *)),
                                 (const uint32_t *)(pb + np * (sizeof(void *) + 4)), (int)np, td.as<TransRec>(), cs))
            return -1;
        stats.launches++;
        NFC_CUDA_CHECK(sync_cs());
        for (DevBuf &kb : kept_bufs) kb.release();
        kept_bufs.clear();
        *R_out = (uint32_t)R;
        return 0;
    }
    set_error("transition buffers kept overflowing");
    return -1;
}

static double now_ms() {
    return std::chrono::duration<double, std::milli>(std::chrono::steady_clock::now().time_since_epoch()).count();
}

struct PostCtx {
    uint32_t M, R, flags, n_empty, n_frames, pad0[3];
    uint32_t tot[8];
    RunCarry rc_out;
    DecCarry dc_out;
    uint32_t pend_out[2];
    uint32_t pad1[2];
    unsigned long long bits_out[2];
    uint32_t pad2[32];
};
static_assert(sizeof(PostCtx) == 256, "context blocks are 256 bytes apart");

int64_t Stream::push_events(const nfc_event *ev, int64_t n) {
    if (n < 0 || (n > 0 && !ev) || n >= ((int64_t)1 << 31)) {
        set_error("push_events: bad arguments");
        return -1;
    }
    NFC_CUDA_CHECK(cudaSetDevice(prm.device));
    if (finalize_all()) return -1;
    if (n == 0) return 0;
    const int64_t a = ev[0].pos;
    std::vector<EventRec> recs((size_t)n);
    int64_t prev = a;
    for (int64_t i = 0; i < n; i++) {
        const int64_t rel = ev[i].pos - a;
        if (ev[i].pos < prev || rel >= ((int64_t)1 << 32) || ev[i].d < 1 || ev[i].d > sp.mx || ev[i].v < -1 || ev[i].v > 2 ||
            ev[i].type < -1 || ev[i].type > 1) {
            set_error("push_events: event %lld out of range (positions ascend within 2^32, d in 1..max_len, v in -1..2, type in -1..1)",
                      (long long)i);
            return -1;
        }
        prev = ev[i].pos;
        EventRec r;
        r.rel_pos = (uint32_t)rel;
        r.d = (uint16_t)ev[i].d;
        r.v = ev[i].v;
        r.type = ev[i].type;
        recs[(size_t)i] = r;
    }
    const double t0 = now_ms();
    const int ci = (int)(slab_seq % NCTX);
    NFC_CUDA_CHECK(cudaEventRecord(ev_a[ci], cs));
    if (post_chain(a, a + 1, false, 0, false, t0, t0, recs.data(), (uint32_t)n)) return -1;
    if (finalize_all()) return -1;
    return n;
}

int Stream::process_slab(const void *d_in, int64_t in_pos0, int64_t in_begin, int64_t in_end, int64_t a, int64_t b,
                         int64_t slicer_end) {
    const double t0 = now_ms();
    const int ci = (int)(slab_seq % NCTX);
    NFC_CUDA_CHECK(cudaEventRecord(ev_a[ci], cs));
    uint32_t R = 0;
    bool fell_back = false, from_bitmap = false;
    if (streaming_ok() && a >= bm_lo && b <= bm_hi) {
        from_bitmap = true;
    } else if (streaming_ok()) {
        if (run_slicer(Slicer::streaming, d_in, in_pos0, in_begin, in_end, a, std::max(b, slicer_end), &R, &fell_back)) return -1;
        from_bitmap = !fell_back;
    } else {
        const Slicer kind = parallel_ok() ? Slicer::first_gen : Slicer::sequential;
        if (run_slicer(kind, d_in, in_pos0, in_begin, in_end, a, b, &R, &fell_back)) return -1;
    }
    if (fell_back) {
        serial_mode = true;
        if (run_slicer(Slicer::sequential, d_in, in_pos0, in_begin, in_end, a, b, &R, &fell_back)) return -1;
    }
    return post_chain(a, b, from_bitmap, R, false, t0, now_ms());
}

int Stream::post_chain(int64_t a, int64_t b, bool from_bitmap, uint32_t R_host, bool force_exact, double t0, double t1,
                       const EventRec *host_events, uint32_t n_host_events) {
    static const bool no_async = getenv("NFC_POST_SYNC") != nullptr;
    const int64_t n = b - a;
    SlabJob j;
    j.seq = slab_seq++;
    j.a = a; j.b = b;
    j.from_bitmap = from_bitmap;
    j.t0 = t0; j.t1 = t1;
    const int ci = (int)(j.seq % NCTX), pv = (int)((j.seq + NCTX - 1) % NCTX), oi = (int)(j.seq & 1);
    PostCtx *cx = ctx_d.as<PostCtx>() + ci, *cp = ctx_d.as<PostCtx>() + pv;
    if (force_exact) NFC_CUDA_CHECK(cudaEventRecord(ev_a[ci], cs));
    const bool fresh = jobs.empty();
    if (fresh) {
        PostCtx up;
        memset(&up, 0, sizeof(up));
        up.rc_out = run_carry;
        up.dc_out = dec_carry;
        up.pend_out[0] = pending[0];
        up.pend_out[1] = pending[1];
        up.bits_out[0] = fb[0].len;
        up.bits_out[1] = fb[1].len;
        NFC_CUDA_CHECK(cudaMemcpyAsync(cp, &up, sizeof(up), cudaMemcpyHostToDevice, cs));
        chain_first_seq = j.seq;
    }
    auto queued = [&](long long seq) { return seq >= chain_first_seq && seq >= 0; };
    NFC_CUDA_CHECK(cudaMemsetAsync(cx, 0, 64, cs));
    const bool want_line = (prm.outputs & (NFC_OUT_SYMBOLS | NFC_OUT_FRAMES)) != 0;
    const bool want_sym = (prm.outputs & NFC_OUT_SYMBOLS) != 0;
    const int keep_dropped = (prm.outputs & NFC_OUT_DROPPED_EVENTS) ? 1 : 0;
    j.exact = force_exact || no_async || !rates.have || !from_bitmap || host_events != nullptr;
    j.events_only = host_events != nullptr;
    auto cap_of = [&](double rate) -> uint32_t {
        const double c = rate * (double)n * 1.5 + 65536.0;
        return (uint32_t)std::min(c, 4.0e9);
    };
    auto sync_on = [&](cudaStream_t st) -> cudaError_t {
        if (!blocking_wait) return cudaStreamSynchronize(st);
        const cudaError_t e = cudaEventRecord(ev_blk, st);
        return e != cudaSuccess ? e : cudaEventSynchronize(ev_blk);
    };
    DevBuf &td = trans_dense[oi];

    if (from_bitmap) {
        if (queued(j.seq - 2)) NFC_CUDA_CHECK(cudaStreamWaitEvent(cs, evR[(j.seq - 2) % NCTX], 0));
        const size_t nblk = extract_blocks(bm_origin, a, b);
        if (ex_counts.ensure((nblk + 16) * 4) || ex_offsets.ensure((nblk + 16) * 4) || ex_scr.ensure((nblk / 256 + 1024) * 4 * 4)) return -1;
        const int carry_from_bm = (!fresh && a > bm_lo) ? 1 : 0;
        if (!fresh && !carry_from_bm) NFC_CUDA_CHECK(cudaStreamWaitEvent(cs, evR[pv], 0));
        if (launch_extract_count(bitmap_d.as<uint32_t>(), bm_origin, a, b, &cp->rc_out, carry_from_bm, ex_counts.as<uint32_t>(),
                                 ex_offsets.as<uint32_t>(), ex_scr.as<uint32_t>(), &cx->R, cs))
            return -1;
        stats.launches += 4;
        if (j.exact) {
            uint32_t R = 0;
            NFC_CUDA_CHECK(cudaMemcpyAsync(&R, &cx->R, 4, cudaMemcpyDeviceToHost, cs));
            NFC_CUDA_CHECK(sync_on(cs));
            j.cap_R = R;
        } else {
            j.cap_R = cap_of(rates.R);
        }
        if (td.ensure(((size_t)j.cap_R + 16) * sizeof(TransRec))) return -1;
        if (launch_extract_write(bitmap_d.as<uint32_t>(), bm_origin, a, b, &cp->rc_out, carry_from_bm, ex_offsets.as<uint32_t>(),
                                 td.as<TransRec>(), j.cap_R, cs))
            return -1;
        stats.launches++;
    } else {
        j.cap_R = R_host;
        NFC_CUDA_CHECK(cudaMemcpyAsync(&cx->R, &R_host, 4, cudaMemcpyHostToDevice, cs));
    }
    NFC_CUDA_CHECK(cudaEventRecord(ev_b[ci], cs));
    NFC_CUDA_CHECK(cudaEventRecord(evE[ci], cs));

    NFC_CUDA_CHECK(cudaStreamWaitEvent(csR, evE[ci], 0));
    if (queued(j.seq - 2)) NFC_CUDA_CHECK(cudaStreamWaitEvent(csR, evL[(j.seq - 2) % NCTX], 0));
    if (ev_out_set[oi]) NFC_CUDA_CHECK(cudaStreamWaitEvent(csR, ev_out[oi], 0));
    if (host_events) {
        j.cap_M = n_host_events;
        if (events_d[oi].ensure(((size_t)j.cap_M + 16) * sizeof(EventRec))) return -1;
        if (n_host_events)
            NFC_CUDA_CHECK(cudaMemcpyAsync(events_d[oi].p, host_events, (size_t)n_host_events * sizeof(EventRec), cudaMemcpyHostToDevice, csR));
        NFC_CUDA_CHECK(cudaMemcpyAsync(&cx->M, &n_host_events, 4, cudaMemcpyHostToDevice, csR));
        NFC_CUDA_CHECK(cudaMemcpyAsync(&cx->rc_out, &cp->rc_out, sizeof(RunCarry), cudaMemcpyDeviceToDevice, csR));
        NFC_CUDA_CHECK(cudaStreamSynchronize(csR));
    } else {
    const size_t nrun = (size_t)j.cap_R + 1;
    if (run_counts.ensure(nrun * 4) || run_offsets.ensure(nrun * 4) || scan_scr.ensure((nrun / 256 + 1024) * 4 * 4)) return -1;
    if (launch_run_count(td.as<TransRec>(), &cx->R, j.cap_R, 0, n, &cp->rc_out, sp.mx, keep_dropped, run_counts.as<uint32_t>(),
                         run_offsets.as<uint32_t>(), scan_scr.as<uint32_t>(), &cx->M, &cx->flags, csR))
        return -1;
    stats.launches += 3;
    if (j.exact) {
        uint32_t M = 0;
        NFC_CUDA_CHECK(cudaMemcpyAsync(&M, &cx->M, 4, cudaMemcpyDeviceToHost, csR));
        NFC_CUDA_CHECK(sync_on(csR));
        j.cap_M = M;
    } else {
        j.cap_M = cap_of(rates.M);
    }
    if (events_d[oi].ensure(((size_t)j.cap_M + 16) * sizeof(EventRec))) return -1;
    if (launch_run_write(td.as<TransRec>(), &cx->R, j.cap_R, 0, n, &cp->rc_out, sp.mx, keep_dropped, run_offsets.as<uint32_t>(),
                         events_d[oi].as<EventRec>(), j.cap_M, &cx->M, &cx->rc_out, &cx->flags, csR))
        return -1;
    stats.launches++;
    }
    NFC_CUDA_CHECK(cudaEventRecord(evR[ci], csR));

    NFC_CUDA_CHECK(cudaStreamWaitEvent(csL, evR[ci], 0));
    if (ev_out_set[oi]) NFC_CUDA_CHECK(cudaStreamWaitEvent(csL, ev_out[oi], 0));
    j.have_line = want_line;
    if (want_line) {
        const uint32_t nc = std::max(1u, linecode_chunks(j.cap_M));
        if (start_d.ensure((size_t)nc * 2 + 64) || summ_d.ensure((size_t)nc * 2 + 64) || cnts_d.ensure((size_t)nc * linecode_cnt_bytes()) ||
            cprefix_d.ensure((size_t)nc * linecode_cnt_bytes()) || line_scr.ensure(linecode_scratch_bytes(nc) + 256))
            return -1;
        const EventRec *ev = events_d[oi].as<EventRec>();
        if (launch_linecode_start(ev, &cx->M, j.cap_M, lt, &cp->dc_out, summ_d.as<uint16_t>(), start_d.as<uint16_t>(), &cx->flags, csL)) return -1;
        if (launch_linecode_count(ev, &cx->M, j.cap_M, lt, start_d.as<uint16_t>(), cnts_d.p, cprefix_d.p, line_scr.p, cx->tot, csL)) return -1;
        stats.launches += 6;
        if (j.exact) {
            PostCtx hx;
            NFC_CUDA_CHECK(cudaMemcpyAsync(&hx, cx, 64, cudaMemcpyDeviceToHost, csL));
            NFC_CUDA_CHECK(sync_on(csL));
            if (hx.flags & POST_UNRESOLVED) {
                stats.linecode_scan_fallbacks++;
                if (maps_d.ensure((size_t)nc * linecode_map_bytes()) || prefix_d.ensure((size_t)nc * linecode_map_bytes())) return -1;
                if (launch_linecode_start_scan(ev, &cx->M, j.cap_M, lt, &cp->dc_out, maps_d.p, prefix_d.p, line_scr.p, start_d.as<uint16_t>(), csL))
                    return -1;
                if (launch_linecode_count(ev, &cx->M, j.cap_M, lt, start_d.as<uint16_t>(), cnts_d.p, cprefix_d.p, line_scr.p, cx->tot, csL)) return -1;
                stats.launches += 9;
                NFC_CUDA_CHECK(cudaMemsetAsync(&cx->flags, 0, 4, csL));
                NFC_CUDA_CHECK(cudaMemcpyAsync(&hx, cx, 64, cudaMemcpyDeviceToHost, csL));
                NFC_CUDA_CHECK(sync_on(csL));
            }
            j.cap_sym = hx.tot[0]; j.cap_b0 = hx.tot[1]; j.cap_b1 = hx.tot[2]; j.cap_em = hx.tot[3];
        } else {
            j.cap_sym = cap_of(rates.sym); j.cap_b0 = cap_of(rates.b0); j.cap_b1 = cap_of(rates.b1); j.cap_em = cap_of(rates.em);
        }
        if ((want_sym && sym_d[oi].ensure(((size_t)j.cap_sym + 16) * sizeof(SymbolRec))) || bits0_d[oi].ensure((size_t)j.cap_b0 + 16) ||
            bits1_d[oi].ensure((size_t)j.cap_b1 + 16) || em_d[oi].ensure(((size_t)j.cap_em + 16) * linecode_emission_bytes()) ||
            fx_d[oi].ensure(((size_t)j.cap_em + 16) * 8))
            return -1;
        if (launch_linecode_write(ev, &cx->M, j.cap_M, lt, start_d.as<uint16_t>(), cprefix_d.p, want_sym ? sym_d[oi].as<SymbolRec>() : nullptr,
                                  want_sym ? j.cap_sym : 0, bits0_d[oi].as<uint8_t>(), j.cap_b0, bits1_d[oi].as<uint8_t>(), j.cap_b1, em_d[oi].p,
                                  fx_d[oi].p, j.cap_em, a, cp->bits_out, cx->bits_out, &cx->n_empty, &cx->n_frames, cp->pend_out, &cp->dc_out, &cx->dc_out,
                                  cx->pend_out, csL))
            return -1;
        stats.launches++;
    } else {
        NFC_CUDA_CHECK(cudaMemcpyAsync(&cx->dc_out, &cp->dc_out, sizeof(DecCarry) + 8 + 8 + 16, cudaMemcpyDeviceToDevice, csL));
    }
    NFC_CUDA_CHECK(cudaEventRecord(ev_c[ci], csL));
    NFC_CUDA_CHECK(cudaMemcpyAsync(ctx_h + (size_t)ci * 256, cx, 256, cudaMemcpyDeviceToHost, csL));
    NFC_CUDA_CHECK(cudaEventRecord(ev_ctx[ci], csL));
    NFC_CUDA_CHECK(cudaEventRecord(evL[ci], csL));
    j.want_ev = (prm.outputs & NFC_OUT_EVENTS) != 0;
    j.want_sym = want_sym && want_line;
    j.want_fr = (prm.outputs & NFC_OUT_FRAMES) != 0 && want_line;
    j.t2 = now_ms();
    jobs.push_back(j);
    while (jobs.size() > 1)
        if (finalize_front()) return -1;
    return 0;
}

int Stream::settle_frames() {
    if (have_last_records) {
        cudaError_t e;
        if (blocking_wait) e = cudaEventSynchronize(ev_last_records);
        else
            while ((e = cudaEventQuery(ev_last_records)) == cudaErrorNotReady) {}
        NFC_CUDA_CHECK(e);
        have_last_records = false;
    }
    return 0;
}

int Stream::finalize_front() {
    if (jobs.empty()) return 0;
    static const bool timing = getenv("NFC_TIMING") != nullptr;
    const SlabJob j = jobs.front();
    const int ci = (int)(j.seq % NCTX), oi = (int)(j.seq & 1);
    NFC_CUDA_CHECK(cudaEventSynchronize(ev_ctx[ci]));
    const double t3 = now_ms();
    PostCtx hx;
    memcpy(&hx, ctx_h + (size_t)ci * 256, sizeof(hx));
    bool bad = false;
    if (!j.exact) {
        bad = (hx.flags & (POST_OVF_TRANS | POST_OVF_EVENTS | POST_UNRESOLVED)) != 0 || hx.R > j.cap_R || hx.M > j.cap_M;
        if (j.have_line)
            bad = bad || (j.want_sym && hx.tot[0] > j.cap_sym) || hx.tot[1] > j.cap_b0 || hx.tot[2] > j.cap_b1 || hx.tot[3] > j.cap_em;
    } else if (hx.flags & (POST_OVF_TRANS | POST_OVF_EVENTS | POST_UNRESOLVED)) {
        set_error("internal: a slab sized exactly reports flags %u", hx.flags);
        return -1;
    }
    if (bad) {
        std::vector<SlabJob> again(jobs.begin(), jobs.end());
        jobs.clear();
        NFC_CUDA_CHECK(cudaStreamSynchronize(cs));
        NFC_CUDA_CHECK(cudaStreamSynchronize(csR));
        NFC_CUDA_CHECK(cudaStreamSynchronize(csL));
        stats.overflow_retries++;
        slab_seq = j.seq;
        for (const SlabJob &r : again) {
            if (!r.from_bitmap) {
                set_error("internal: a slab without bitmap cannot be done again");
                return -1;
            }
            if (post_chain(r.a, r.b, true, 0, true, r.t0, r.t1)) return -1;
        }
        return 0;
    }
    jobs.pop_front();
    const uint32_t M = hx.M, nsym = hx.tot[0], nbit0 = hx.tot[1], nbit1 = hx.tot[2];
    const uint32_t nemit = hx.n_frames;
    run_carry = hx.rc_out;
    dec_carry = hx.dc_out;
    pending[0] = hx.pend_out[0];
    pending[1] = hx.pend_out[1];
    if (!j.events_only) {
        const double n = (double)std::max<int64_t>(1, j.b - j.a);
        auto upd = [&](double &r, uint32_t v) { r = std::max(r * 0.98, (double)v / n); };
        upd(rates.R, hx.R); upd(rates.M, M); upd(rates.sym, nsym); upd(rates.b0, nbit0); upd(rates.b1, nbit1); upd(rates.em, nemit);
        rates.have = true;
    }
    float ms_ab = 0, ms_ac = 0, ms_cc = 0;
    cudaEventElapsedTime(&ms_ab, ev_a[ci], ev_b[ci]);
    cudaEventElapsedTime(&ms_ac, ev_a[ci], ev_c[ci]);
    if (last_final_seq == j.seq - 1 && j.seq > chain_first_seq &&
        cudaEventElapsedTime(&ms_cc, ev_c[(j.seq + NCTX - 1) % NCTX], ev_c[ci]) == cudaSuccess && ms_cc > 0 && ms_cc < ms_ac)
        ms_ac = ms_cc;
    last_final_seq = j.seq;
    stats.slicer_ms += ms_ab;
    stats.kernel_ms += ms_ac;

    const bool want_ev = j.want_ev, want_sym = j.want_sym, want_fr = j.want_fr;
    size_t off_ev = 0, off_sym = 0, total = 0;
    auto place = [&](size_t bytes) {
        size_t o = total;
        total += (bytes + 63) / 64 * 64;
        return o;
    };
    place(64);
    if (want_ev) off_ev = place((size_t)M * sizeof(EventRec));
    if (want_sym) off_sym = place((size_t)nsym * sizeof(SymbolRec));
    const int pi = (int)(slabs_enqueued % NPIN);
    while (slabs_marshalled.load(std::memory_order_acquire) < slabs_enqueued - (NPIN - 1)) std::this_thread::yield();
    if (ensure_pinned(pi, total)) return -1;
    char *hp = (char *)pinned[pi];
    if (want_fr) {
        const uint32_t nb[2] = {nbit0, nbit1};
        const size_t f0 = out_frames.size();
        const bool grow_any = fb[0].len + nb[0] > fb[0].cap || fb[1].len + nb[1] > fb[1].cap || f0 + nemit > out_frames.cap ||
                              f0 + nemit > findex_cap;
        if (grow_any) {
            if (join_marshal()) return -1;
            NFC_CUDA_CHECK(cudaStreamSynchronize(cs2));
            if (findex_n != f0) {
                set_error("internal: frame index out of step");
                return -1;
            }
            if (fb[0].reserve(fb[0].len + nb[0]) || fb[1].reserve(fb[1].len + nb[1]) || out_frames.reserve(f0 + nemit)) {
                set_error("out of page-locked memory for the frames of a slab");
                return -1;
            }
            if (findex_reserve(f0 + nemit)) {
                set_error(findex_ext ? "more frames than the caller's frame index buffer holds (nfc_stream_set_frame_index_buffer)"
                                     : "out of page-locked memory for the frame index");
                return -1;
            }
        }
        if (nemit) {
            NFC_CUDA_CHECK(cudaMemcpyAsync(out_frames.p + f0, em_d[oi].p, (size_t)nemit * sizeof(nfc_frame), cudaMemcpyDeviceToHost, cs2));
            NFC_CUDA_CHECK(cudaMemcpyAsync(findex + f0, fx_d[oi].p, (size_t)nemit * 8, cudaMemcpyDeviceToHost, cs2));
        }
        if (nbit0) NFC_CUDA_CHECK(cudaMemcpyAsync(fb[0].p + fb[0].len, bits0_d[oi].p, nbit0, cudaMemcpyDeviceToHost, cs2));
        if (nbit1) NFC_CUDA_CHECK(cudaMemcpyAsync(fb[1].p + fb[1].len, bits1_d[oi].p, nbit1, cudaMemcpyDeviceToHost, cs2));
        if (hx.tot[4] & 1) fb[0].closed = fb[0].len + nbit0 - hx.tot[5];
        if (hx.tot[6] & 1) fb[1].closed = fb[1].len + nbit1 - hx.tot[7];
        fb[0].len += nbit0;
        fb[1].len += nbit1;
        out_frames.n = f0 + nemit;
        findex_n = f0 + nemit;
        stats.empty_frames += hx.n_empty & 0x7fffffffu;
        if (hx.n_empty >> 31) findex_bad = true;
        total += (size_t)nbit0 + nbit1 + (size_t)nemit * (sizeof(nfc_frame) + 8);
    }
    if (want_ev && M) NFC_CUDA_CHECK(cudaMemcpyAsync(hp + off_ev, events_d[oi].p, (size_t)M * sizeof(EventRec), cudaMemcpyDeviceToHost, cs2));
    if (want_sym && nsym)
        NFC_CUDA_CHECK(cudaMemcpyAsync(hp + off_sym, sym_d[oi].p, (size_t)nsym * sizeof(SymbolRec), cudaMemcpyDeviceToHost, cs2));
    NFC_CUDA_CHECK(cudaEventRecord(ev_d[pi], cs2));
    NFC_CUDA_CHECK(cudaEventRecord(ev_out[oi], cs2));
    ev_out_set[oi] = true;
    slabs_enqueued++;
    stats.d2h_bytes += (int64_t)total + 256;
    if (timing)
        fprintf(stderr, "slab %lld..%lld%s: slicer %.2f ms (dev %.2f), chain queued in %.2f (dev %.2f), context seen %.2f ms after queuing\n",
                (long long)j.a, (long long)j.b, j.exact ? " (exact sizes)" : "", j.t1 - j.t0, ms_ab, j.t2 - j.t1, ms_ac - ms_ab, t3 - j.t2);
    if (!want_ev && !want_sym) {
        ev_last_records = ev_d[pi];
        have_last_records = true;
        slabs_marshalled.fetch_add(1, std::memory_order_release);
        return 0;
    }
    return marshal(j, pi, hp, off_ev, off_sym, M, nsym);
}

int Stream::marshal(const SlabJob &j, int pi, char *hp, size_t off_ev, size_t off_sym, uint32_t M, uint32_t nsym) {
    const int64_t a = j.a;
    const bool want_ev = j.want_ev, want_sym = j.want_sym;
    if (marshal_err.load()) return join_marshal();
    auto prev = std::make_shared<std::thread>(std::move(marshal_thr));
    const cudaEvent_t evd = ev_d[pi];
    const int dev = prm.device;
    marshal_thr = std::thread([this, prev, evd, dev, hp, off_ev, off_sym, M, nsym, a, want_ev, want_sym]() {
      if (prev->joinable()) prev->join();
      cudaSetDevice(dev);
      static const bool timing = getenv("NFC_TIMING") != nullptr;
      const double tm0 = timing ? now_ms() : 0.0;
      double tm1 = tm0;
      if (cudaEventSynchronize(evd) != cudaSuccess) marshal_err = 2;
      else [&]() {
        if (timing) tm1 = now_ms();
        auto grow = [](auto &v, size_t more) {
            if (v.capacity() < v.size() + more) v.reserve(std::max(v.size() + more, v.capacity() * 2));
        };
        if (want_ev) {
            const EventRec *e = reinterpret_cast<const EventRec *>(hp + off_ev);
            grow(out_events, M);
            for (uint32_t i = 0; i < M; i++) {
                nfc_event o;
                o.pos = a + (int64_t)e[i].rel_pos;
                o.d = e[i].d;
                o.v = e[i].v;
                o.type = e[i].type;
                o.pad = 0;
                out_events.push_back(o);
            }
        }
        if (want_sym) {
            const SymbolRec *s = reinterpret_cast<const SymbolRec *>(hp + off_sym);
            grow(out_symbols, nsym);
            for (uint32_t i = 0; i < nsym; i++) {
                nfc_symbol o;
                o.pos = a + (int64_t)s[i].rel_pos;
                o.type = s[i].type;
                o.val = s[i].val;
                o.pad = 0;
                o.pad2 = 0;
                out_symbols.push_back(o);
            }
        }
      }();
      if (timing) fprintf(stderr, "  records of slab at %lld: waited %.2f ms for them, into the output vectors in %.2f ms\n", (long long)a, tm1 - tm0, now_ms() - tm1);
      slabs_marshalled.fetch_add(1, std::memory_order_release);
    });
    return 0;
}

}

using nfc::Stream;
struct nfc_stream {
    Stream s;
};

template <class T>
static int64_t drain_vec(std::vector<T> &v, size_t &head, T *out, int64_t cap) {
    const int64_t avail = (int64_t)(v.size() - head);
    if (cap <= 0 || !out) return avail;
    const int64_t n = std::min(avail, cap);
    memcpy(out, v.data() + head, (size_t)n * sizeof(T));
    head += (size_t)n;
    if (head == v.size()) {
        v.clear();
        head = 0;
    }
    return n;
}

extern "C" {

void nfc_default_params(nfc_params *p) {
    memset(p, 0, sizeof(*p));
    p->samp_rate = 2e6;
    p->lo_val = 0.1;
    p->hi_val = 1.1;
    p->av_window = 2000;
    p->max_len = 50;
    p->decode_reader = 1;
    p->decode_tag = 1;
    p->input_kind = NFC_IN_ENVELOPE_F32;
    p->outputs = NFC_OUT_EVENTS | NFC_OUT_SYMBOLS | NFC_OUT_FRAMES | NFC_OUT_DROPPED_EVENTS;
    p->device = 0;
    p->pcm_scale = 32767.0f;
}

int nfc_stream_create(const nfc_params *p, nfc_stream **out) {
    if (!p || !out) {
        nfc::set_error("null argument");
        return -1;
    }
    if (p->input_kind < NFC_IN_ENVELOPE_F32 || p->input_kind > NFC_IN_SC16) {
        nfc::set_error("unknown input_kind %d (NFC_IN_ENVELOPE_F32 .. NFC_IN_SC16: 0 .. 4)", (int)p->input_kind);
        return -1;
    }
    int ndev = 0;
    if (cudaGetDeviceCount(&ndev) != cudaSuccess || ndev <= 0) {
        nfc::set_error("no CUDA device: this library has no CPU path");
        return -1;
    }
    nfc_stream *h = new (std::nothrow) nfc_stream();
    if (!h) {
        nfc::set_error("out of memory");
        return -1;
    }
    if (h->s.init(p)) {
        h->s.destroy();
        delete h;
        return -1;
    }
    *out = h;
    return 0;
}

int nfc_stream_destroy(nfc_stream *h) {
    if (!h) return 0;
    cudaSetDevice(h->s.prm.device);
    h->s.destroy();
    delete h;
    return 0;
}

int nfc_stream_reset(nfc_stream *h) {
    if (!h) return -1;
    Stream &s = h->s;
    s.settle();
    s.pos = 0;
    s.stable = false;
    s.serial_mode = false;
    s.bm_lo = s.bm_hi = 0;
    s.warm.clear();
    s.run_carry = nfc::RunCarry{0, 0, 0, 0};
    s.dec_carry = nfc::DecCarry{0, 0, {0, 0}};
    s.pending[0] = s.pending[1] = 0;
    s.fb[0].clear();
    s.fb[1].clear();
    s.out_events.clear();
    s.out_symbols.clear();
    s.out_frames.clear();
    s.findex_n = 0;
    s.findex_bad = false;
    s.ev_head = s.sym_head = s.fr_head = 0;
    return 0;
}

int nfc_stream_set_thresholds(nfc_stream *h, double lo_val, double hi_val) {
    if (!h) return -1;
    Stream &s = h->s;
    if (s.settle()) return -1;
    if (s.pos != 0 || s.stable || !s.warm.empty()) {
        nfc::set_error("set_thresholds: the stream has consumed samples; reset it first");
        return -1;
    }
    cudaSetDevice(s.prm.device);
    s.prm.lo_val = lo_val;
    s.prm.hi_val = hi_val;
    s.sp.lo = lo_val;
    s.sp.hi = hi_val;
    s.sp.loL = s.sp.lo / s.sp.Ld;
    s.sp.hiL = s.sp.hi / s.sp.Ld;
    s.sp.cls_ss0_x0 = nfc::classify_ratio_host(1.0, s.sp.lo, s.sp.hi);
    s.sp.cls_ss0_xn = nfc::classify_ratio_host(s.sp.hi + 0.1, s.sp.lo, s.sp.hi);
    NFC_CUDA_CHECK(cudaMemcpyAsync(s.params_d.p, &s.sp, sizeof(s.sp), cudaMemcpyHostToDevice, s.cs));
    NFC_CUDA_CHECK(s.sync_cs());
    return 0;
}

int64_t nfc_stream_push(nfc_stream *h, const void *items, int64_t n, int mem, int *called_back) {
    if (!h || (n > 0 && !items)) {
        nfc::set_error("null argument");
        return -1;
    }
    return h->s.push(items, n, mem, called_back);
}

int64_t nfc_stream_push_batch(nfc_stream *h, const void *items, int mem, int64_t n_captures, int64_t items_per_capture,
                              int64_t stride_items, const double *lo_vals, const double *hi_vals, int64_t *pitch) {
    if (!h || !items) {
        nfc::set_error("null argument");
        return -1;
    }
    if (h->s.settle()) return -1;
    return h->s.push_batch(items, mem, n_captures, items_per_capture, stride_items, lo_vals, hi_vals, pitch);
}

int64_t nfc_stream_push_events(nfc_stream *h, const nfc_event *ev, int64_t n) {
    if (!h) {
        nfc::set_error("null argument");
        return -1;
    }
    return h->s.push_events(ev, n);
}

int64_t nfc_stream_drain_events(nfc_stream *h, nfc_event *out, int64_t cap) {
    if (!h || h->s.settle()) return -1;
    return drain_vec(h->s.out_events, h->s.ev_head, out, cap);
}

int64_t nfc_stream_drain_symbols(nfc_stream *h, nfc_symbol *out, int64_t cap) {
    if (!h || h->s.settle()) return -1;
    return drain_vec(h->s.out_symbols, h->s.sym_head, out, cap);
}

int64_t nfc_stream_pending_frame_bits(nfc_stream *h) {
    if (!h || h->s.settle()) return -1;
    return (int64_t)(h->s.fb[0].closed + h->s.fb[1].closed);
}

int64_t nfc_stream_drain_frames(nfc_stream *h, nfc_frame *out, int64_t cap, uint8_t *bits, int64_t bits_cap) {
    if (!h || h->s.settle()) return -1;
    Stream &s = h->s;
    const int64_t avail = (int64_t)s.out_frames.size();
    if (cap <= 0 || !out) return avail;
    const int64_t nb0 = (int64_t)s.fb[0].closed, nb1 = (int64_t)s.fb[1].closed;
    if (cap < avail || bits_cap < nb0 + nb1 || (!bits && nb0 + nb1 > 0)) {
        nfc::set_error("drain_frames: buffers too small (%lld frames, %lld bits pending)", (long long)avail,
                       (long long)(nb0 + nb1));
        return -2;
    }
    auto copy_frames = [&](int64_t i0, int64_t i1) {
        for (int64_t i = i0; i < i1; i++) {
            out[i] = s.out_frames[(size_t)i];
            if (out[i].type == 1) out[i].bit_off += nb0;
        }
    };
    if (nb0 + nb1 > (4 << 20)) {
        std::thread t0([&] { if (nb0) memcpy(bits, s.fb[0].p, (size_t)nb0); });
        std::thread t1([&] { if (nb1) memcpy(bits + nb0, s.fb[1].p, (size_t)nb1); });
        std::thread t2([&] { copy_frames(0, avail / 2); });
        copy_frames(avail / 2, avail);
        t0.join();
        t1.join();
        t2.join();
    } else {
        if (nb0) memcpy(bits, s.fb[0].p, (size_t)nb0);
        if (nb1) memcpy(bits + nb0, s.fb[1].p, (size_t)nb1);
        copy_frames(0, avail);
    }
    s.out_frames.clear();
    s.findex_n = 0;
    s.findex_bad = false;
    s.fb[0].consume();
    s.fb[1].consume();
    s.fr_head = 0;
    return avail;
}

int64_t nfc_stream_view_frames(nfc_stream *h, const nfc_frame **frames, const uint8_t **bits_tag, int64_t *n_bits_tag,
                               const uint8_t **bits_reader, int64_t *n_bits_reader) {
    if (!h || !frames || !bits_tag || !n_bits_tag || !bits_reader || !n_bits_reader) {
        nfc::set_error("null argument");
        return -1;
    }
    if (getenv("NFC_TIMING")) {
        const double t0 = nfc::now_ms();
        if (h->s.finish_pending()) return -1;
        const double t1 = nfc::now_ms();
        if (h->s.join_marshal()) return -1;
        fprintf(stderr, "view_frames: last slab's records %.2f ms, its marshalling %.2f ms\n", t1 - t0, nfc::now_ms() - t1);
    }
    if (h->s.settle()) return -1;
    Stream &s = h->s;
    *frames = s.out_frames.data();
    *bits_tag = s.fb[0].p;
    *n_bits_tag = (int64_t)s.fb[0].closed;
    *bits_reader = s.fb[1].p;
    *n_bits_reader = (int64_t)s.fb[1].closed;
    return (int64_t)s.out_frames.size();
}

int64_t nfc_stream_view_frame_index(nfc_stream *h, const uint64_t **index) {
    if (!h || !index) {
        nfc::set_error("null argument");
        return -1;
    }
    if (h->s.settle()) return -1;
    Stream &s = h->s;
    if (s.findex_bad || s.findex_n != s.out_frames.size()) {
        nfc::set_error("view_frame_index: a frame does not fit the packing (position >= 2^40 or more than 65535 bits)");
        return -1;
    }
    *index = s.findex;
    return (int64_t)s.findex_n;
}

int nfc_stream_set_frame_index_buffer(nfc_stream *h, uint64_t *buf, int64_t cap) {
    if (!h || (buf && cap <= 0)) {
        nfc::set_error("bad argument");
        return -1;
    }
    if (h->s.settle()) return -1;
    Stream &s = h->s;
    if (!s.out_frames.empty()) {
        nfc::set_error("set_frame_index_buffer: the stream holds frames; release them first");
        return -1;
    }
    cudaSetDevice(s.prm.device);
    s.findex_drop();
    s.findex = buf;
    s.findex_ext = buf != nullptr;
    s.findex_cap = buf ? (size_t)cap : 0;
    if (buf) {
        s.findex_ext_locked = cudaHostRegister(buf, (size_t)cap * 8, cudaHostRegisterPortable) == cudaSuccess;
        if (!s.findex_ext_locked) cudaGetLastError();
    }
    s.findex_n = 0;
    s.findex_bad = false;
    return 0;
}

int nfc_stream_release_frames(nfc_stream *h) {
    if (!h || h->s.settle()) return -1;
    Stream &s = h->s;
    s.out_frames.clear();
    s.findex_n = 0;
    s.findex_bad = false;
    s.fb[0].consume();
    s.fb[1].consume();
    s.fr_head = 0;
    return 0;
}

int nfc_stream_get_state(nfc_stream *h, nfc_state *st, float *ring, uint8_t *pending_bits) {
    if (!h || !st) {
        nfc::set_error("null argument");
        return -1;
    }
    if (h->s.settle()) return -1;
    Stream &s = h->s;
    memset(st, 0, sizeof(*st));
    st->pos = s.pos;
    st->stable = s.stable ? 1 : 0;
    st->serial_mode = s.serial_mode ? 1 : 0;
    st->lastL = nfc::NO_POS;
    st->lrun_start = nfc::NO_POS;
    if (s.stable) {
        cudaSetDevice(s.prm.device);
        std::vector<char> blk(nfc::state_block_bytes(s.sp.L));
        NFC_CUDA_CHECK(cudaMemcpy(blk.data(), s.state.p, blk.size(), cudaMemcpyDeviceToHost));
        const nfc::SlicerHdr *hd = reinterpret_cast<const nfc::SlicerHdr *>(blk.data());
        st->ss = hd->ss;
        st->lastL = hd->lastL;
        st->lrun_start = hd->lrun_start;
        st->index = (int32_t)(s.pos % s.sp.L);
        if (ring) memcpy(ring, nfc::state_ring(hd), (size_t)s.sp.L * 4);
        st->cur_state = s.run_carry.st;
        st->last_bit = s.run_carry.last_bit;
        st->dur = s.run_carry.dur;
    } else {
        st->dur = 1;
        if (ring) {
            memset(ring, 0, (size_t)s.sp.L * 4);
            if (!s.warm.empty()) memcpy(ring, s.warm.data(), s.warm.size() * 4);
        }
    }
    st->miller_state = s.dec_carry.miller_state;
    st->manch_state = s.dec_carry.manch_state;
    for (int t = 0; t < 2; t++) {
        st->started[t] = s.dec_carry.started[t];
        st->pending[t] = (int32_t)s.pending[t];
    }
    if (pending_bits) {
        size_t o = 0;
        for (int t = 0; t < 2; t++) {
            const size_t open = s.fb[t].len - s.fb[t].closed;
            if (open) memcpy(pending_bits + o, s.fb[t].p + s.fb[t].closed, open);
            o += open;
        }
    }
    return 0;
}

int nfc_stream_set_state(nfc_stream *h, const nfc_state *st, const float *ring, const uint8_t *pending_bits) {
    if (!h || !st) {
        nfc::set_error("null argument");
        return -1;
    }
    Stream &s = h->s;
    s.bm_lo = s.bm_hi = 0;
    if (s.settle()) return -1;
    if (!st->stable || !ring) {
        nfc::set_error("set_state needs a stable state with its ring");
        return -1;
    }
    cudaSetDevice(s.prm.device);
    std::vector<char> blk(nfc::state_block_bytes(s.sp.L), 0);
    nfc::SlicerHdr *hd = reinterpret_cast<nfc::SlicerHdr *>(blk.data());
    hd->ss = st->ss;
    hd->pos = st->pos;
    if (st->lastL == INT64_MIN) {
        const int64_t P = st->pos;
        if (st->cur_state == 2 && st->last_bit == -1) {
            hd->lastL = P - 1;
            hd->lrun_start = P - st->dur;
        } else if (st->cur_state == 2) {
            hd->lastL = P - st->dur - 1;
            hd->lrun_start = hd->lastL;
        } else if (st->last_bit == -1) {
            hd->lastL = P - 1;
            hd->lrun_start = P - 1 - s.sp.mx;
        } else {
            hd->lastL = nfc::NO_POS;
            hd->lrun_start = nfc::NO_POS;
        }
    } else {
        hd->lastL = st->lastL;
        hd->lrun_start = st->lrun_start;
    }
    hd->last_val = st->last_bit;
    memcpy(nfc::state_ring(hd), ring, (size_t)s.sp.L * 4);
    NFC_CUDA_CHECK(cudaMemcpy(s.state.p, blk.data(), blk.size(), cudaMemcpyHostToDevice));
    s.pos = st->pos;
    s.stable = true;
    s.serial_mode = st->serial_mode != 0;
    s.run_carry.st = st->cur_state;
    s.run_carry.last_bit = st->last_bit;
    s.run_carry.dur = st->dur;
    s.dec_carry.miller_state = st->miller_state;
    s.dec_carry.manch_state = st->manch_state;
    size_t o = 0;
    for (int t = 0; t < 2; t++) {
        s.dec_carry.started[t] = st->started[t];
        s.pending[t] = (uint32_t)st->pending[t];
        s.fb[t].len = s.fb[t].closed;
        if (s.fb[t].reserve(s.fb[t].len + (size_t)st->pending[t] + 64)) {
            nfc::set_error("out of page-locked memory");
            return -1;
        }
        if (pending_bits) memcpy(s.fb[t].p + s.fb[t].len, pending_bits + o, (size_t)st->pending[t]);
        else memset(s.fb[t].p + s.fb[t].len, 0, (size_t)st->pending[t]);
        s.fb[t].len += (size_t)st->pending[t];
        o += (size_t)st->pending[t];
    }
    return 0;
}

int nfc_stream_set_wait_mode(nfc_stream *h, int blocking) {
    if (!h) return -1;
    return h->s.set_wait_mode(blocking != 0);
}

int nfc_stream_set_tuning(nfc_stream *h, int64_t seg_len, int64_t halo, int64_t slab_len, int force_serial) {
    if (!h) return -1;
    h->s.seg_len = seg_len;
    h->s.halo = halo;
    h->s.slab_len = slab_len;
    h->s.force_serial = force_serial;
    return 0;
}

int nfc_stream_get_stats(nfc_stream *h, nfc_stats *st) {
    if (!h || !st) return -1;
    h->s.finish_pending();
    cudaSetDevice(h->s.prm.device);
    unsigned long long ts[16] = {0};
    if (nfc::slicer_tile_stats(ts, false) == 0) {
        h->s.stats.fast_tiles = (int64_t)ts[0];
        h->s.stats.exact_tiles = (int64_t)ts[1];
        h->s.stats.repeated_passes = (int64_t)ts[5];
        h->s.stats.fixpoint_tiles = (int64_t)ts[3];
        h->s.stats.st2_tiles = (int64_t)ts[6];
        h->s.stats.unproven_tiles = (int64_t)(ts[2] + ts[7]);
        h->s.stats.ring_resums = (int64_t)ts[4];
        h->s.stats.exact_rounds = (int64_t)ts[8];
        h->s.stats.pipe_tiles = (int64_t)ts[11];
        h->s.stats.pipe_runs = (int64_t)ts[12];
        h->s.stats.pipe_aborts = (int64_t)ts[13];
        if (getenv("NFC_TIMING"))
            fprintf(stderr, "slicer segments: %llu cycles in all, %llu of them inside pipelined runs (%llu tiles of %llu)\n", ts[15], ts[14], ts[11], ts[0]);
    }
    *st = h->s.stats;
    return 0;
}

int nfc_stream_reset_stats(nfc_stream *h) {
    if (!h) return -1;
    memset(&h->s.stats, 0, sizeof(h->s.stats));
    unsigned long long ts[16];
    cudaSetDevice(h->s.prm.device);
    nfc::slicer_tile_stats(ts, true);
    return 0;
}

void *nfc_stream_cuda_stream(nfc_stream *h) { return h ? (void *)h->s.cs : nullptr; }

int nfc_build_tables(double samp_rate, int32_t max_len, int which, uint8_t *dclass, int32_t dclass_cap, uint16_t *table,
                     int32_t table_cap, int32_t *n_dclass) {
    nfc::HostTables t;
    if (!(samp_rate > 0) || max_len < 1 || !nfc::build_tables(max_len, 1e6 / samp_rate, t)) {
        nfc::set_error("cannot build line-code tables for samp_rate=%g max_len=%d", samp_rate, max_len);
        return -1;
    }
    const std::vector<uint8_t> &dc = which ? t.dclass_miller : t.dclass_manch;
    const std::vector<nfc::TabEntry> &tb = which ? t.miller : t.manch;
    if (n_dclass) *n_dclass = which ? t.n_dclass_miller : t.n_dclass_manch;
    if (dclass && dclass_cap >= (int32_t)dc.size()) memcpy(dclass, dc.data(), dc.size());
    if (table && table_cap >= (int32_t)tb.size()) memcpy(table, tb.data(), tb.size() * sizeof(uint16_t));
    return (int)tb.size();
}

int nfc_synth_render(void *dev_out, int64_t n, int64_t first_index, const int8_t *codes, const int64_t *lens,
                     int64_t n_runs, float carrier, float pause, float tag_high, float noise, float fade,
                     double fade_period, uint64_t seed, int as_envelope, int device) {
    if (cudaSetDevice(device) != cudaSuccess) {
        nfc::set_error("cudaSetDevice(%d) failed", device);
        return -1;
    }
    return nfc::synth_render(dev_out, n, first_index, codes, lens, n_runs, carrier, pause, tag_high, noise, fade, fade_period, seed,
                             as_envelope, nullptr);
}

const char *nfc_last_error(void) { return nfc::g_err; }
int nfc_abi_version(void) { return NFC_ABI_VERSION; }

int nfc_abi_sizeof(int which) {
    switch (which) {
        case 0: return (int)sizeof(nfc_params);
        case 1: return (int)sizeof(nfc_event);
        case 2: return (int)sizeof(nfc_symbol);
        case 3: return (int)sizeof(nfc_frame);
        case 4: return (int)sizeof(nfc_frame_tail);
        case 5: return (int)sizeof(nfc_state);
        case 6: return (int)sizeof(nfc_stats);
        default: return -1;
    }
}
int nfc_device_count(void) {
    int n = 0;
    if (cudaGetDeviceCount(&n) != cudaSuccess) return 0;
    return n;
}

}
```

Measured before the change: 474,100.

## Fuse linecode summary, start, count and write into one decoupled-lookback pass kernel

Replaces the separate chunk summary, chunk start, count, prefix-scan and write kernels with a single line_pass kernel. Each block stages its events into shared memory, computes chunk summaries and starts with a tag-based cross-block lookback, and counts with an in-block warp scan plus a decoupled-lookback prefix across blocks, then writes. The aim is fewer launches and fewer global passes over the event array. The cost is spin-waiting on global tags, reliance on ticket-ordered blocks, and a count-only pass that is reused in exact mode.

```diff
diff --git a/usrp_nfc_b200/csrc/linecode.cu b/usrp_nfc_b200/csrc/linecode.cu
--- a/usrp_nfc_b200/csrc/linecode.cu
+++ b/usrp_nfc_b200/csrc/linecode.cu
@@ -259,105 +259,77 @@
     }
 };
 
-__global__ void chunk_summary_kernel(const EventRec *__restrict__ ev, EvCount evc, LineTables lt,
-                                     uint16_t *__restrict__ summary) {
-    NFC_TABLE_SMEM
-    const uint32_t c = blockIdx.x * blockDim.x + threadIdx.x;
-    const uint32_t n_ev = evc.n(), n_chunks = (n_ev + CHUNK - 1) / CHUNK;
-    if (c >= n_chunks) return;
+
+struct PassEvents {
+    const EventRec *g, *s;
+    int64_t e0;
+    __device__ __forceinline__ EventRec operator()(int64_t i) const {
+        if (i < e0) return g[i];
+        const int64_t l = i - e0;
+        return s[l + l / CHUNK];
+    }
+};
+struct ChunkEvents {
+    const EventRec *s;
+    uint32_t i0;
+    __device__ __forceinline__ EventRec operator()(uint32_t i) const { return s[i - i0]; }
+};
+
+__device__ __forceinline__ uint16_t chunk_summary(const ChunkEvents &ev, uint32_t i0, uint32_t i1, uint32_t cap_prev,
+                                                  const LineTables &lt, const TabView &tv) {
     int rs = 0, gs = 0;
     bool kR = false, kG = false;
     NullSink sink;
-    const uint32_t i0 = c * CHUNK, i1 = min(n_ev, i0 + CHUNK);
-    uint32_t cap_prev = tv.pitch ? batch_capture_before(tv, ev, (int64_t)i0) : 0u;
-    for (uint32_t i = i0; i < i1; i += 8) {
-        EventRec e8[8];
-        load8(ev, i, e8);
-#pragma unroll
-        for (int k = 0; k < 8; k++) {
-            if (i + k >= i1) continue;
-            const EventRec e = e8[k];
-            int dummy = 0;
-            if (tv.pitch) {
-                bool inside;
-                const uint32_t cap = batch_capture(tv, e.rel_pos, inside);
-                if (cap != cap_prev) {
-                    cap_prev = cap;
-                    rs = 0; kR = true;
-                    gs = 0; kG = true;
-                }
-                if (!inside) continue;
+#pragma unroll 8
+    for (uint32_t i = i0; i < i1; i++) {
+        const EventRec e = ev(i);
+        int dummy = 0;
+        if (tv.pitch) {
+            bool inside;
+            const uint32_t cap = batch_capture(tv, e.rel_pos, inside);
+            if (cap != cap_prev) {
+                cap_prev = cap;
+                rs = 0; kR = true;
+                gs = 0; kG = true;
             }
-            if (e.type == 1 && tv.use_reader) {
-                const uint8_t r = lt.reset_miller[(int)tv.dcm[e.d] * 4 + (e.v + 1)];
-                if (r != 0xFF) { rs = r; kR = true; }
-                else if (kR) step_event(e, tv, rs, dummy, sink);
-            } else if (e.type == 0 && tv.use_tag) {
-                const uint8_t r = lt.reset_manch[(int)tv.dcg[e.d] * 4 + (e.v + 1)];
-                if (r != 0xFF) { gs = r; kG = true; }
-                else if (kG) step_event(e, tv, dummy, gs, sink);
+            if (!inside) continue;
+        }
+        if (e.type == 1 && tv.use_reader) {
+            const uint8_t r = lt.reset_miller[(int)tv.dcm[e.d] * 4 + (e.v + 1)];
+            if (r != 0xFF) { rs = r; kR = true; }
+            else if (kR) step_event(e, tv, rs, dummy, sink);
+        } else if (e.type == 0 && tv.use_tag) {
+            const uint8_t r = lt.reset_manch[(int)tv.dcg[e.d] * 4 + (e.v + 1)];
+            if (r != 0xFF) { gs = r; kG = true; }
+            else if (kG) step_event(e, tv, dummy, gs, sink);
+        }
+    }
+    return (uint16_t)((rs & 31) | (kR ? 32 : 0) | ((gs & 15) << 8) | (kG ? 4096 : 0));
+}
+
+__device__ __forceinline__ void lookback_replay(const PassEvents &ev, int64_t from, int64_t i0, int64_t iR, int64_t iG,
+                                                const TabView &tv, int &rs, int &gs) {
+    NullSink sink;
+    uint32_t cap_prev = (tv.pitch && from < i0) ? (from > 0 ? ev(from - 1).rel_pos / tv.pitch : NO_CAPTURE) : 0u;
+    for (int64_t kk = from; kk < i0; kk++) {
+        const EventRec e = ev(kk);
+        int dummy_r = 0, dummy_g = 0;
+        if (tv.pitch) {
+            bool inside;
+            const uint32_t cap = batch_capture(tv, e.rel_pos, inside);
+            if (cap != cap_prev) {
+                cap_prev = cap;
+                if (kk > iR) rs = 0;
+                if (kk > iG) gs = 0;
             }
-        }
-    }
-    summary[c] = (uint16_t)((rs & 31) | (kR ? 32 : 0) | ((gs & 15) << 8) | (kG ? 4096 : 0));
-}
-
-__global__ void chunk_start_kernel(const EventRec *__restrict__ ev, EvCount evc, LineTables lt,
-                                   const DecCarry *__restrict__ carry_in, const uint16_t *__restrict__ summary,
-                                   uint16_t *__restrict__ start, uint32_t *__restrict__ flags) {
-    NFC_TABLE_SMEM
-    const uint32_t c = blockIdx.x * blockDim.x + threadIdx.x;
-    const uint32_t n_ev = evc.n(), n_chunks = (n_ev + CHUNK - 1) / CHUNK;
-    if (c >= n_chunks) return;
-    const DecCarry carry = *carry_in;
-    int rs = (carry.miller_state & 15) | ((carry.started[1] & 1) << 4);
-    int gs = (carry.manch_state & 7) | ((carry.started[0] & 1) << 3);
-    const int64_t i0 = (int64_t)c * CHUNK;
-    bool foundR = !tv.use_reader, foundG = !tv.use_tag;
-    int64_t iR = -1, iG = -1;
-    int64_t cc = (int64_t)c - 1;
-    const int64_t cmin = max((int64_t)0, (int64_t)c - LOOKBACK_LIMIT / CHUNK);
-    for (; cc >= cmin && !(foundR && foundG); cc--) {
-        const unsigned sm = summary[cc];
-        if (!foundR && (sm & 32u)) { foundR = true; iR = (cc + 1) * CHUNK - 1; rs = (int)(sm & 31u); }
-        if (!foundG && (sm & 4096u)) { foundG = true; iG = (cc + 1) * CHUNK - 1; gs = (int)((sm >> 8) & 15u); }
-    }
-    if (cc >= 0 && !(foundR && foundG)) {
-        atomicOr(flags, (uint32_t)POST_UNRESOLVED);
-        start[c] = 0;
-        return;
-    }
-    NullSink sink;
-    const int64_t fromR = tv.use_reader ? iR + 1 : i0, fromG = tv.use_tag ? iG + 1 : i0;
-    const int64_t from = fromR < fromG ? fromR : fromG;
-    uint32_t cap_prev = (tv.pitch && from < i0) ? batch_capture_before(tv, ev, from) : 0u;
-    for (int64_t base = from & ~(int64_t)7; base < i0; base += 8) {
-        EventRec e8[8];
-        load8(ev, base, e8);
-#pragma unroll
-        for (int k = 0; k < 8; k++) {
-            const int64_t kk = base + k;
-            if (kk < from || kk >= i0) continue;
-            const EventRec e = e8[k];
-            int dummy_r = 0, dummy_g = 0;
-            if (tv.pitch) {
-                bool inside;
-                const uint32_t cap = batch_capture(tv, e.rel_pos, inside);
-                if (cap != cap_prev) {
-                    cap_prev = cap;
-                    if (kk > iR) rs = 0;
-                    if (kk > iG) gs = 0;
-                }
-                if (!inside) continue;
-            }
-            if (e.type == 1) {
-                if (kk > iR) step_event(e, tv, rs, dummy_g, sink);
-            } else if (e.type == 0) {
-                if (kk > iG) step_event(e, tv, dummy_r, gs, sink);
-            }
-        }
-    }
-    start[c] = (uint16_t)(rs | (gs << 8));
+            if (!inside) continue;
+        }
+        if (e.type == 1) {
+            if (kk > iR) step_event(e, tv, rs, dummy_g, sink);
+        } else if (e.type == 0) {
+            if (kk > iG) step_event(e, tv, dummy_r, gs, sink);
+        }
+    }
 }
 
 __global__ void chunk_start_from_maps_kernel(const ChunkMap *__restrict__ prefix, const DecCarry *__restrict__ carry_in,
@@ -368,31 +340,6 @@
     const int rs0 = (carry.miller_state & 15) | ((carry.started[1] & 1) << 4);
     const int gs0 = (carry.manch_state & 7) | ((carry.started[0] & 1) << 3);
     start[c] = (uint16_t)(prefix[c].r[rs0] | (prefix[c].g[gs0] << 8));
-}
-
-__global__ void chunk_count_kernel(const EventRec *__restrict__ ev, EvCount evc, LineTables lt,
-                                   const uint16_t *__restrict__ start, ChunkCnt *__restrict__ cnts, uint32_t cap_chunks) {
-    NFC_TABLE_SMEM
-    const uint32_t c = blockIdx.x * blockDim.x + threadIdx.x;
-    const uint32_t n_ev = evc.n(), n_chunks = (n_ev + CHUNK - 1) / CHUNK;
-    if (c >= cap_chunks) return;
-    CountSink sink;
-    sink.c = ChunkCnt{0, 0, 0, 0, 0, 0, 0, 0};
-    if (c >= n_chunks) {
-        cnts[c] = sink.c;
-        return;
-    }
-    int rs = start[c] & 31, gs = (start[c] >> 8) & 15;
-    const uint32_t i0 = c * CHUNK, i1 = min(n_ev, i0 + CHUNK);
-    uint32_t cap_prev = tv.pitch ? batch_capture_before(tv, ev, (int64_t)i0) : 0u;
-    for (uint32_t i = i0; i < i1; i += 8) {
-        EventRec e[8];
-        load8(ev, i, e);
-#pragma unroll
-        for (int k = 0; k < 8; k++)
-            if (i + k < i1) step_event_batch(e[k], tv, rs, gs, sink, cap_prev);
-    }
-    cnts[c] = sink.c;
 }
 
 struct WriteSink {
@@ -417,7 +364,7 @@
     __device__ __forceinline__ void emission(uint32_t pos, int type) {
         const uint32_t nbits = type == 0 ? pend0 : pend1;
         if (nbits == 0) {
-            atomicAdd(n_empty, 1u);
+            if (n_empty) atomicAdd(n_empty, 1u);
             return;
         }
         if (iem < cap_em) {
@@ -429,7 +376,8 @@
             fr[iem] = f;
             fx[iem] = ((unsigned long long)f.pos << 24) | ((unsigned long long)nbits << 8) | (unsigned long long)type;
         }
-        if ((((unsigned long long)(a + (int64_t)pos)) >> 40) || nbits >= 65536u) atomicOr(n_empty, 0x80000000u);
+        if (n_empty && ((((unsigned long long)(a + (int64_t)pos)) >> 40) || nbits >= 65536u))
+            atomicOr(n_empty, 0x80000000u);
         iem++;
         if (type == 0) pend0 = 0; else pend1 = 0;
     }
@@ -452,25 +400,186 @@
     unsigned long long *bits_out;
     uint32_t *n_empty;
     uint32_t *n_frames;
-};
-
-__global__ void chunk_write_kernel(const EventRec *__restrict__ ev, EvCount evc, LineTables lt,
-                                   const uint16_t *__restrict__ start,
-                                   const ChunkCnt *__restrict__ cnt_prefix, LineOut out, const DecCarry *__restrict__ carry_in,
-                                   DecCarry *__restrict__ carry_out, uint32_t *__restrict__ pending_out) {
+    uint32_t *tot;
+};
+
+static const int LP_THREADS = 128;
+static const int LP_STRIDE = CHUNK + 1;
+static const size_t LP_SMEM = (size_t)LP_THREADS * LP_STRIDE * sizeof(EventRec);
+static_assert(LP_THREADS % 32 == 0 && LP_THREADS * CHUNK >= LOOKBACK_LIMIT, "a lookback reaches into the block before at most");
+
+struct LinePass {
+    uint32_t *ticket;
+    volatile uint32_t *sum_tag;
+    volatile uint32_t *agg_tag, *inc_tag;
+    ChunkCnt *agg, *inc;
+    uint16_t *summary;
+    uint32_t tag;
+};
+
+__device__ __forceinline__ void wait_tag(volatile uint32_t *f, uint32_t tag) {
+    while (*f != tag) __nanosleep(32);
+    __threadfence();
+}
+__device__ __forceinline__ ChunkCnt load_cnt_l2(const ChunkCnt *p) {
+    const uint4 u = __ldcg(reinterpret_cast<const uint4 *>(p)), v = __ldcg(reinterpret_cast<const uint4 *>(p) + 1);
+    return ChunkCnt{u.x, u.y, u.z, u.w, v.x, v.y, v.z, v.w};
+}
+
+__global__ void __launch_bounds__(LP_THREADS) line_pass_kernel(const EventRec *__restrict__ ev, EvCount evc, LineTables lt,
+                                                               const DecCarry *__restrict__ carry_in, uint16_t *__restrict__ start,
+                                                               int starts_given, LinePass lp, uint32_t *__restrict__ flags,
+                                                               LineOut out, DecCarry *__restrict__ carry_out,
+                                                               uint32_t *__restrict__ pending_out) {
+    extern __shared__ EventRec s_ev[];
+    __shared__ uint16_t s_sum[LP_THREADS];
+    __shared__ ChunkCnt s_warp[LP_THREADS / 32];
+    __shared__ ChunkCnt s_pre;
+    __shared__ uint32_t s_blk;
+    const int tid = threadIdx.x;
+    if (tid == 0) {
+        s_blk = atomicAdd(lp.ticket, 1u);
+        __threadfence();
+        if (atomicAdd(lp.ticket + 1, 1u) == gridDim.x - 1) {
+            atomicExch(lp.ticket, 0u);
+            atomicExch(lp.ticket + 1, 0u);
+        }
+    }
     NFC_TABLE_SMEM
-    const uint32_t c = blockIdx.x * blockDim.x + threadIdx.x;
+    const uint32_t b = s_blk;
     const uint32_t n_ev = evc.n(), n_chunks = (n_ev + CHUNK - 1) / CHUNK;
-    if (n_chunks == 0 && c == 0) {
-        *carry_out = *carry_in;
-        pending_out[0] = out.pending_in[0];
-        pending_out[1] = out.pending_in[1];
-        out.bits_out[0] = out.bits_in[0];
-        out.bits_out[1] = out.bits_in[1];
-    }
-    if (c >= n_chunks) return;
-    int rs = start[c] & 31, gs = (start[c] >> 8) & 15;
-    const ChunkCnt pc = cnt_prefix[c];
+    if (n_chunks == 0) {
+        if (b == 0 && tid == 0) {
+            *carry_out = *carry_in;
+            pending_out[0] = out.pending_in[0];
+            pending_out[1] = out.pending_in[1];
+            out.bits_out[0] = out.bits_in[0];
+            out.bits_out[1] = out.bits_in[1];
+        }
+        return;
+    }
+    const uint32_t c0 = b * LP_THREADS;
+    if (c0 >= n_chunks) return;
+
+    const int64_t e0 = (int64_t)c0 * CHUNK;
+    const uint32_t ne = min(n_ev - (uint32_t)e0, (uint32_t)(LP_THREADS * CHUNK));
+    {
+        const uint4 *src = reinterpret_cast<const uint4 *>(ev + e0);
+        uint2 *dst = reinterpret_cast<uint2 *>(s_ev);
+#pragma unroll 4
+        for (uint32_t p = tid; p < (ne + 1) / 2; p += LP_THREADS) {
+            const uint4 q = __ldg(src + p);
+            const uint32_t l = 2 * p, s = l + l / CHUNK;
+            dst[s] = make_uint2(q.x, q.y);
+            dst[s + 1] = make_uint2(q.z, q.w);
+        }
+    }
+    __syncthreads();
+
+    const uint32_t c = c0 + tid;
+    const bool has = c < n_chunks;
+    const uint32_t i0 = c * CHUNK, i1 = has ? min(n_ev, i0 + CHUNK) : i0;
+    const PassEvents all{ev, s_ev, e0};
+    const ChunkEvents own{s_ev + tid * LP_STRIDE, i0};
+    const uint32_t cap0 = (has && tv.pitch) ? (i0 > 0 ? all((int64_t)i0 - 1).rel_pos / tv.pitch : NO_CAPTURE) : 0u;
+    int rs = 0, gs = 0;
+    if (starts_given) {
+        if (has) {
+            rs = start[c] & 31;
+            gs = (start[c] >> 8) & 15;
+        }
+    } else {
+        const uint16_t sm = has ? chunk_summary(own, i0, i1, cap0, lt, tv) : 0;
+        s_sum[tid] = sm;
+        if (has) lp.summary[c] = sm;
+        __threadfence();
+        __syncthreads();
+        if (tid == 0) lp.sum_tag[b] = lp.tag;
+
+        const DecCarry carry = *carry_in;
+        rs = (carry.miller_state & 15) | ((carry.started[1] & 1) << 4);
+        gs = (carry.manch_state & 7) | ((carry.started[0] & 1) << 3);
+        bool foundR = !tv.use_reader, foundG = !tv.use_tag;
+        int64_t iR = -1, iG = -1;
+        int64_t cc = (int64_t)c - 1;
+        const int64_t cmin = max((int64_t)0, (int64_t)c - LOOKBACK_LIMIT / CHUNK);
+        auto look = [&](unsigned sm) {
+            if (!foundR && (sm & 32u)) { foundR = true; iR = (cc + 1) * CHUNK - 1; rs = (int)(sm & 31u); }
+            if (!foundG && (sm & 4096u)) { foundG = true; iG = (cc + 1) * CHUNK - 1; gs = (int)((sm >> 8) & 15u); }
+        };
+        for (; cc >= max(cmin, (int64_t)c0) && !(foundR && foundG); cc--) look(s_sum[cc - c0]);
+        const bool need = has && !(foundR && foundG) && cc >= cmin;
+        if (__syncthreads_or(need)) {
+            if (tid == 0)
+                for (int64_t p = (int64_t)b - 1; p >= 0 && (p + 1) * LP_THREADS > (int64_t)c0 - LOOKBACK_LIMIT / CHUNK; p--)
+                    wait_tag(lp.sum_tag + p, lp.tag);
+            __syncthreads();
+        }
+        if (need)
+            for (; cc >= cmin && !(foundR && foundG); cc--) look(__ldcg(lp.summary + cc));
+        if (has) {
+            if (cc >= 0 && !(foundR && foundG)) {
+                atomicOr(flags, (uint32_t)POST_UNRESOLVED);
+                rs = 0;
+                gs = 0;
+            } else {
+                const int64_t fromR = tv.use_reader ? iR + 1 : i0, fromG = tv.use_tag ? iG + 1 : i0;
+                lookback_replay(all, fromR < fromG ? fromR : fromG, i0, iR, iG, tv, rs, gs);
+            }
+            start[c] = (uint16_t)(rs | (gs << 8));
+        }
+    }
+
+    CountSink cnt;
+    cnt.c = ChunkCnt{0, 0, 0, 0, 0, 0, 0, 0};
+    if (has) {
+        int r = rs, g = gs;
+        uint32_t cap_prev = cap0;
+#pragma unroll 8
+        for (uint32_t i = i0; i < i1; i++) step_event_batch(own(i), tv, r, g, cnt, cap_prev);
+    }
+    const CombineCnt op;
+    const ChunkCnt zero = {0, 0, 0, 0, 0, 0, 0, 0};
+    const int lane = tid & 31, w = tid >> 5;
+    ChunkCnt x = cnt.c;
+#pragma unroll
+    for (int d = 1; d < 32; d <<= 1) {
+        const ChunkCnt y = shfl_up_any(x, d);
+        if (lane >= d) x = op(y, x);
+    }
+    ChunkCnt ex = shfl_up_any(x, 1);
+    if (lane == 0) ex = zero;
+    if (lane == 31) s_warp[w] = x;
+    __syncthreads();
+    if (tid == 0) {
+        ChunkCnt agg = zero;
+        for (int k = 0; k < LP_THREADS / 32; k++) {
+            const ChunkCnt t = s_warp[k];
+            s_warp[k] = agg;
+            agg = op(agg, t);
+        }
+        ChunkCnt pre = zero;
+        if (b > 0) {
+            lp.agg[b] = agg;
+            __threadfence();
+            lp.agg_tag[b] = lp.tag;
+            for (int64_t p = (int64_t)b - 1; p >= 0; p--) {
+                bool inc;
+                while (!(inc = lp.inc_tag[p] == lp.tag) && lp.agg_tag[p] != lp.tag) __nanosleep(32);
+                __threadfence();
+                pre = op(load_cnt_l2(inc ? lp.inc + p : lp.agg + p), pre);
+                if (inc) break;
+            }
+        }
+        lp.inc[b] = op(pre, agg);
+        __threadfence();
+        lp.inc_tag[b] = lp.tag;
+        s_pre = pre;
+    }
+    __syncthreads();
+    if (!has) return;
+    const ChunkCnt pc = op(s_pre, op(s_warp[w], ex));
+
     WriteSink sink;
     sink.sym = out.sym; sink.bits0 = out.bits0; sink.bits1 = out.bits1; sink.fr = out.fr; sink.fx = out.fx;
     sink.n_empty = out.n_empty; sink.a = out.a; sink.base0 = out.bits_in[0]; sink.base1 = out.bits_in[1];
@@ -478,15 +587,9 @@
     sink.isym = pc.nsym; sink.ib0 = pc.nbit0; sink.ib1 = pc.nbit1; sink.iem = resolved_records(pc, out.pending_in);
     sink.pend0 = (pc.has0 & 1) ? pc.tail0 : out.pending_in[0] + pc.tail0;
     sink.pend1 = (pc.has1 & 1) ? pc.tail1 : out.pending_in[1] + pc.tail1;
-    const uint32_t i0 = c * CHUNK, i1 = min(n_ev, i0 + CHUNK);
-    uint32_t cap_prev = tv.pitch ? batch_capture_before(tv, ev, (int64_t)i0) : 0u;
-    for (uint32_t i = i0; i < i1; i += 8) {
-        EventRec e[8];
-        load8(ev, i, e);
-#pragma unroll
-        for (int k = 0; k < 8; k++)
-            if (i + k < i1) step_event_batch(e[k], tv, rs, gs, sink, cap_prev);
-    }
+    uint32_t cap_prev = cap0;
+#pragma unroll 8
+    for (uint32_t i = i0; i < i1; i++) step_event_batch(own(i), tv, rs, gs, sink, cap_prev);
     if (c == n_chunks - 1) {
         DecCarry co;
         co.miller_state = rs & 15; co.started[1] = rs >> 4;
@@ -497,26 +600,23 @@
         out.bits_out[0] = sink.base0 + sink.ib0;
         out.bits_out[1] = sink.base1 + sink.ib1;
         *out.n_frames = sink.iem;
-    }
-}
+        const ChunkCnt t = op(pc, cnt.c);
+        const uint32_t tv8[8] = {t.nsym, t.nbit0, t.nbit1, t.nemit, t.has0, t.tail0, t.has1, t.tail1};
+        for (int k = 0; k < 8; k++) out.tot[k] = tv8[k];
+    }
+}
+
+int raise_dynamic_smem(const void *fn, size_t smem);
 
 uint32_t linecode_chunks(uint32_t n_ev) { return (n_ev + CHUNK - 1) / CHUNK; }
 size_t linecode_map_bytes() { return sizeof(ChunkMap); }
-size_t linecode_cnt_bytes() { return sizeof(ChunkCnt); }
 size_t linecode_emission_bytes() { return sizeof(FrameRec); }
-size_t linecode_scratch_bytes(uint32_t n_chunks) {
-    return scan_scratch_elems(n_chunks) * sizeof(ChunkMap) + scan_scratch_elems(n_chunks) * sizeof(ChunkCnt);
-}
-
-int launch_linecode_start(const EventRec *d_ev, const uint32_t *d_M, uint32_t cap_ev, const LineTables &lt, const DecCarry *d_carry_in,
-                          uint16_t *d_summary, uint16_t *d_start, uint32_t *d_flags, cudaStream_t stream) {
-    const uint32_t nc = std::max(1u, linecode_chunks(cap_ev));
-    const EvCount evc{d_M, cap_ev};
-    chunk_summary_kernel<<<(nc + 127) / 128, 128, 0, stream>>>(d_ev, evc, lt, d_summary);
-    NFC_CUDA_CHECK(cudaGetLastError());
-    chunk_start_kernel<<<(nc + 127) / 128, 128, 0, stream>>>(d_ev, evc, lt, d_carry_in, d_summary, d_start, d_flags);
-    NFC_CUDA_CHECK(cudaGetLastError());
-    return 0;
+size_t linecode_scratch_bytes(uint32_t n_chunks) { return scan_scratch_elems(n_chunks) * sizeof(ChunkMap); }
+
+static size_t line_pass_blocks(uint32_t cap_ev) { return (std::max(1u, linecode_chunks(cap_ev)) + LP_THREADS - 1) / LP_THREADS; }
+size_t line_pass_bytes(uint32_t cap_ev) {
+    const size_t nb = line_pass_blocks(cap_ev);
+    return 256 + ((nb * 3 * 4 + 15) / 16) * 16 + nb * 2 * sizeof(ChunkCnt) + nb * LP_THREADS * 2;
 }
 
 int launch_linecode_start_scan(const EventRec *d_ev, const uint32_t *d_M, uint32_t cap_ev, const LineTables &lt,
@@ -538,24 +638,23 @@
     return 0;
 }
 
-int launch_linecode_count(const EventRec *d_ev, const uint32_t *d_M, uint32_t cap_ev, const LineTables &lt, const uint16_t *d_start,
-                          void *d_cnts, void *d_cnt_prefix, void *d_scratch, void *d_total, cudaStream_t stream) {
-    const uint32_t nc = std::max(1u, linecode_chunks(cap_ev));
-    ChunkCnt *cnts = (ChunkCnt *)d_cnts, *cprefix = (ChunkCnt *)d_cnt_prefix;
-    const EvCount evc{d_M, cap_ev};
-    chunk_count_kernel<<<(nc + 127) / 128, 128, 0, stream>>>(d_ev, evc, lt, d_start, cnts, nc);
-    NFC_CUDA_CHECK(cudaGetLastError());
-    ChunkCnt zero = {0, 0, 0, 0, 0, 0, 0, 0};
-    return device_exclusive_scan<ChunkCnt, CombineCnt>(cnts, cprefix, nc, zero, CombineCnt(), (ChunkCnt *)d_scratch,
-                                                       (ChunkCnt *)d_total, stream);
-}
-
-int launch_linecode_write(const EventRec *d_ev, const uint32_t *d_M, uint32_t cap_ev, const LineTables &lt, const uint16_t *d_start,
-                          const void *d_cnt_prefix, SymbolRec *d_sym, uint32_t cap_sym, uint8_t *d_bits0, uint32_t cap_b0,
-                          uint8_t *d_bits1, uint32_t cap_b1, void *d_frames, void *d_findex, uint32_t cap_em, int64_t a,
-                          const void *d_bits_in, void *d_bits_out, uint32_t *d_n_empty, uint32_t *d_n_frames, const uint32_t *d_pending_in,
-                          const DecCarry *d_carry_in, DecCarry *d_carry_out, uint32_t *d_pending_out, cudaStream_t stream) {
-    const uint32_t nc = std::max(1u, linecode_chunks(cap_ev));
+int launch_line_pass(const EventRec *d_ev, const uint32_t *d_M, uint32_t cap_ev, const LineTables &lt, const DecCarry *d_carry_in,
+                     uint16_t *d_start, int starts_given, void *d_pass, uint32_t tag, uint32_t *d_flags, uint32_t *d_tot,
+                     SymbolRec *d_sym, uint32_t cap_sym, uint8_t *d_bits0, uint32_t cap_b0, uint8_t *d_bits1, uint32_t cap_b1,
+                     void *d_frames, void *d_findex, uint32_t cap_em, int64_t a, const void *d_bits_in, void *d_bits_out,
+                     uint32_t *d_n_empty, uint32_t *d_n_frames, const uint32_t *d_pending_in, DecCarry *d_carry_out,
+                     uint32_t *d_pending_out, cudaStream_t stream) {
+    const size_t nb = line_pass_blocks(cap_ev);
+    char *p = (char *)d_pass;
+    LinePass lp;
+    lp.ticket = (uint32_t *)p;
+    lp.sum_tag = (uint32_t *)(p + 256);
+    lp.agg_tag = lp.sum_tag + nb;
+    lp.inc_tag = lp.agg_tag + nb;
+    lp.agg = (ChunkCnt *)(p + 256 + ((nb * 3 * 4 + 15) / 16) * 16);
+    lp.inc = lp.agg + nb;
+    lp.summary = (uint16_t *)(lp.inc + nb);
+    lp.tag = tag;
     LineOut out;
     out.sym = d_sym; out.bits0 = d_bits0; out.bits1 = d_bits1; out.fr = (FrameRec *)d_frames; out.fx = (unsigned long long *)d_findex;
     out.cap_sym = cap_sym; out.cap_b0 = cap_b0; out.cap_b1 = cap_b1; out.cap_em = cap_em;
@@ -565,9 +664,11 @@
     out.bits_out = (unsigned long long *)d_bits_out;
     out.n_empty = d_n_empty;
     out.n_frames = d_n_frames;
+    out.tot = d_tot;
+    if (raise_dynamic_smem((const void *)line_pass_kernel, LP_SMEM)) return -1;
     const EvCount evc{d_M, cap_ev};
-    chunk_write_kernel<<<(nc + 127) / 128, 128, 0, stream>>>(d_ev, evc, lt, d_start, (const ChunkCnt *)d_cnt_prefix, out,
-                                                             d_carry_in, d_carry_out, d_pending_out);
+    line_pass_kernel<<<(unsigned)nb, LP_THREADS, LP_SMEM, stream>>>(d_ev, evc, lt, d_carry_in, d_start, starts_given, lp, d_flags,
+                                                                     out, d_carry_out, d_pending_out);
     NFC_CUDA_CHECK(cudaGetLastError());
     return 0;
 }
diff --git a/usrp_nfc_b200/csrc/slicer.cu b/usrp_nfc_b200/csrc/slicer.cu
--- a/usrp_nfc_b200/csrc/slicer.cu
+++ b/usrp_nfc_b200/csrc/slicer.cu
@@ -778,7 +778,7 @@
     return SLICER_NT;
 }
 
-static int raise_dynamic_smem(const void *fn, size_t smem);
+int raise_dynamic_smem(const void *fn, size_t smem);
 
 struct FastVariant {
     const void *fn;
@@ -864,7 +864,7 @@
 
 int slicer_streaming_tile(int L, int kind) { return fast_variant_of(L, kind).tile; }
 
-static int raise_dynamic_smem(const void *fn, size_t smem) {
+int raise_dynamic_smem(const void *fn, size_t smem) {
     static std::mutex mu;
     static std::map<std::pair<const void *, int>, size_t> have;
     int dev = 0;
diff --git a/usrp_nfc_b200/csrc/stream.cu b/usrp_nfc_b200/csrc/stream.cu
--- a/usrp_nfc_b200/csrc/stream.cu
+++ b/usrp_nfc_b200/csrc/stream.cu
@@ -42,21 +42,18 @@
                      RunCarry *d_carry_out, uint32_t *d_flags, cudaStream_t stream);
 uint32_t linecode_chunks(uint32_t n_ev);
 size_t linecode_map_bytes();
-size_t linecode_cnt_bytes();
 size_t linecode_emission_bytes();
 size_t linecode_scratch_bytes(uint32_t n_chunks);
-int launch_linecode_start(const EventRec *d_ev, const uint32_t *d_M, uint32_t cap_ev, const LineTables &lt, const DecCarry *d_carry_in,
-                          uint16_t *d_summary, uint16_t *d_start, uint32_t *d_flags, cudaStream_t stream);
+size_t line_pass_bytes(uint32_t cap_ev);
 int launch_linecode_start_scan(const EventRec *d_ev, const uint32_t *d_M, uint32_t cap_ev, const LineTables &lt,
                                const DecCarry *d_carry_in, void *d_maps, void *d_prefix, void *d_scratch, uint16_t *d_start,
                                cudaStream_t stream);
-int launch_linecode_count(const EventRec *d_ev, const uint32_t *d_M, uint32_t cap_ev, const LineTables &lt, const uint16_t *d_start,
-                          void *d_cnts, void *d_cnt_prefix, void *d_scratch, void *d_total, cudaStream_t stream);
-int launch_linecode_write(const EventRec *d_ev, const uint32_t *d_M, uint32_t cap_ev, const LineTables &lt, const uint16_t *d_start,
-                          const void *d_cnt_prefix, SymbolRec *d_sym, uint32_t cap_sym, uint8_t *d_bits0, uint32_t cap_b0,
-                          uint8_t *d_bits1, uint32_t cap_b1, void *d_frames, void *d_findex, uint32_t cap_em, int64_t a,
-                          const void *d_bits_in, void *d_bits_out, uint32_t *d_n_empty, uint32_t *d_n_frames, const uint32_t *d_pending_in,
-                          const DecCarry *d_carry_in, DecCarry *d_carry_out, uint32_t *d_pending_out, cudaStream_t stream);
+int launch_line_pass(const EventRec *d_ev, const uint32_t *d_M, uint32_t cap_ev, const LineTables &lt, const DecCarry *d_carry_in,
+                     uint16_t *d_start, int starts_given, void *d_pass, uint32_t tag, uint32_t *d_flags, uint32_t *d_tot,
+                     SymbolRec *d_sym, uint32_t cap_sym, uint8_t *d_bits0, uint32_t cap_b0, uint8_t *d_bits1, uint32_t cap_b1,
+                     void *d_frames, void *d_findex, uint32_t cap_em, int64_t a, const void *d_bits_in, void *d_bits_out,
+                     uint32_t *d_n_empty, uint32_t *d_n_frames, const uint32_t *d_pending_in, DecCarry *d_carry_out,
+                     uint32_t *d_pending_out, cudaStream_t stream);
 int slicer_tile(int L, int kind);
 int slicer_resident_ctas(int L, int kind);
 int slicer_tile_stats(unsigned long long *out4, bool reset);
@@ -215,9 +212,10 @@
     int force_serial = 0;
 
     DevBuf params_d, tab_d, staging, works_d, states_d, trans_seg, seg_counts, seg_status,
-        seam_ptrs, mismatch_d, run_counts, run_offsets, scan_scr, maps_d, prefix_d, cnts_d, cprefix_d,
+        seam_ptrs, mismatch_d, run_counts, run_offsets, scan_scr, maps_d, prefix_d,
         line_scr, serial_ring, start_d, ckpt_d, redo_states, redo_trans,
-        redo_counts, pieces_d, bitmap_d, ex_counts, ex_offsets, ex_scr, summ_d;
+        redo_counts, pieces_d, bitmap_d, ex_counts, ex_offsets, ex_scr, line_pass_d;
+    uint32_t line_pass_tag = 0;
     DevBuf events_d[2], sym_d[2], bits0_d[2], bits1_d[2], em_d[2], fx_d[2];
     DevBuf trans_dense[2];
     std::vector<DevBuf> kept_bufs;
@@ -435,10 +433,10 @@
 void Stream::destroy() {
     DevBuf *all[] = {&batch_states, &batch_stage, &params_d, &tab_d, &staging, &works_d, &states_d, &trans_seg, &trans_dense[0], &trans_dense[1], &seg_counts,
                      &seg_status, &seam_ptrs, &mismatch_d, &run_counts, &run_offsets, &scan_scr, &maps_d,
-                     &prefix_d, &cnts_d, &cprefix_d, &line_scr, &ctx_d, &events_d[0], &events_d[1], &sym_d[0], &sym_d[1], &bits0_d[0],
+                     &prefix_d, &line_scr, &ctx_d, &events_d[0], &events_d[1], &sym_d[0], &sym_d[1], &bits0_d[0],
                      &bits0_d[1], &bits1_d[0], &bits1_d[1], &em_d[0], &em_d[1], &fx_d[0], &fx_d[1],
                      &serial_ring, &start_d, &ckpt_d, &redo_states, &redo_trans, &redo_counts, &pieces_d, &state, &bitmap_d,
-                     &ex_counts, &ex_offsets, &ex_scr, &summ_d};
+                     &ex_counts, &ex_offsets, &ex_scr, &line_pass_d};
     finalize_all();
     if (marshal_thr.joinable()) marshal_thr.join();
     if (cs) cudaStreamSynchronize(cs);
@@ -1331,29 +1329,43 @@
     j.have_line = want_line;
     if (want_line) {
         const uint32_t nc = std::max(1u, linecode_chunks(j.cap_M));
-        if (start_d.ensure((size_t)nc * 2 + 64) || summ_d.ensure((size_t)nc * 2 + 64) || cnts_d.ensure((size_t)nc * linecode_cnt_bytes()) ||
-            cprefix_d.ensure((size_t)nc * linecode_cnt_bytes()) || line_scr.ensure(linecode_scratch_bytes(nc) + 256))
-            return -1;
+        if (start_d.ensure((size_t)nc * 2 + 64)) return -1;
+        if (line_pass_d.cap < line_pass_bytes(j.cap_M)) {
+            if (line_pass_d.ensure(line_pass_bytes(j.cap_M))) return -1;
+            NFC_CUDA_CHECK(cudaMemsetAsync(line_pass_d.p, 0, line_pass_d.cap, csL));
+        }
         const EventRec *ev = events_d[oi].as<EventRec>();
-        if (launch_linecode_start(ev, &cx->M, j.cap_M, lt, &cp->dc_out, summ_d.as<uint16_t>(), start_d.as<uint16_t>(), &cx->flags, csL)) return -1;
-        if (launch_linecode_count(ev, &cx->M, j.cap_M, lt, start_d.as<uint16_t>(), cnts_d.p, cprefix_d.p, line_scr.p, cx->tot, csL)) return -1;
-        stats.launches += 6;
+        auto line_pass = [&](int starts_given, bool write) -> int {
+            if (++line_pass_tag == 0) line_pass_tag = 1;
+            stats.launches++;
+            return launch_line_pass(ev, &cx->M, j.cap_M, lt, &cp->dc_out, start_d.as<uint16_t>(), starts_given, line_pass_d.p, line_pass_tag,
+                                    &cx->flags, cx->tot, write && want_sym ? sym_d[oi].as<SymbolRec>() : nullptr,
+                                    write && want_sym ? j.cap_sym : 0, write ? bits0_d[oi].as<uint8_t>() : nullptr, write ? j.cap_b0 : 0,
+                                    write ? bits1_d[oi].as<uint8_t>() : nullptr, write ? j.cap_b1 : 0, write ? em_d[oi].p : nullptr,
+                                    write ? fx_d[oi].p : nullptr, write ? j.cap_em : 0, a, cp->bits_out, cx->bits_out,
+                                    write ? &cx->n_empty : nullptr, &cx->n_frames, cp->pend_out, &cx->dc_out, cx->pend_out, csL);
+        };
+        int starts_given = 0;
         if (j.exact) {
+            if (line_pass(0, false)) return -1;
             PostCtx hx;
             NFC_CUDA_CHECK(cudaMemcpyAsync(&hx, cx, 64, cudaMemcpyDeviceToHost, csL));
             NFC_CUDA_CHECK(sync_on(csL));
             if (hx.flags & POST_UNRESOLVED) {
                 stats.linecode_scan_fallbacks++;
-                if (maps_d.ensure((size_t)nc * linecode_map_bytes()) || prefix_d.ensure((size_t)nc * linecode_map_bytes())) return -1;
+                if (maps_d.ensure((size_t)nc * linecode_map_bytes()) || prefix_d.ensure((size_t)nc * linecode_map_bytes()) ||
+                    line_scr.ensure(linecode_scratch_bytes(nc) + 256))
+                    return -1;
                 if (launch_linecode_start_scan(ev, &cx->M, j.cap_M, lt, &cp->dc_out, maps_d.p, prefix_d.p, line_scr.p, start_d.as<uint16_t>(), csL))
                     return -1;
-                if (launch_linecode_count(ev, &cx->M, j.cap_M, lt, start_d.as<uint16_t>(), cnts_d.p, cprefix_d.p, line_scr.p, cx->tot, csL)) return -1;
-                stats.launches += 9;
+                stats.launches += 5;
+                if (line_pass(1, false)) return -1;
                 NFC_CUDA_CHECK(cudaMemsetAsync(&cx->flags, 0, 4, csL));
                 NFC_CUDA_CHECK(cudaMemcpyAsync(&hx, cx, 64, cudaMemcpyDeviceToHost, csL));
                 NFC_CUDA_CHECK(sync_on(csL));
             }
             j.cap_sym = hx.tot[0]; j.cap_b0 = hx.tot[1]; j.cap_b1 = hx.tot[2]; j.cap_em = hx.tot[3];
+            starts_given = 1;
         } else {
             j.cap_sym = cap_of(rates.sym); j.cap_b0 = cap_of(rates.b0); j.cap_b1 = cap_of(rates.b1); j.cap_em = cap_of(rates.em);
         }
@@ -1361,12 +1373,7 @@
             bits1_d[oi].ensure((size_t)j.cap_b1 + 16) || em_d[oi].ensure(((size_t)j.cap_em + 16) * linecode_emission_bytes()) ||
             fx_d[oi].ensure(((size_t)j.cap_em + 16) * 8))
             return -1;
-        if (launch_linecode_write(ev, &cx->M, j.cap_M, lt, start_d.as<uint16_t>(), cprefix_d.p, want_sym ? sym_d[oi].as<SymbolRec>() : nullptr,
-                                  want_sym ? j.cap_sym : 0, bits0_d[oi].as<uint8_t>(), j.cap_b0, bits1_d[oi].as<uint8_t>(), j.cap_b1, em_d[oi].p,
-                                  fx_d[oi].p, j.cap_em, a, cp->bits_out, cx->bits_out, &cx->n_empty, &cx->n_frames, cp->pend_out, &cp->dc_out, &cx->dc_out,
-                                  cx->pend_out, csL))
-            return -1;
-        stats.launches++;
+        if (line_pass(starts_given, true)) return -1;
     } else {
         NFC_CUDA_CHECK(cudaMemcpyAsync(&cx->dc_out, &cp->dc_out, sizeof(DecCarry) + 8 + 8 + 16, cudaMemcpyDeviceToDevice, csL));
     }
```

After: 379,100, median of 6. -20.0%, worse.
